# ViskaWei/VIT

Hardware: AMD Instinct MI355X
Metric: images/sec ViT-B/16 224^2 bf16 train step (higher is better)
Workload: dtype bf16

## Files before the change

include/vit_amd.h:

```cpp
#ifndef VIT_AMD_H_
#define VIT_AMD_H_

#include <stddef.h>
#include <stdint.h>

#ifdef __cplusplus
extern "C" {
#endif

#define VIT_AMD_VERSION 100

typedef struct vit_ctx* vit_handle;
typedef void* vit_stream;

typedef enum { VIT_OK = 0, VIT_ERR_ARG = -1, VIT_ERR_HIP = -2, VIT_ERR_UNSUPPORTED = -3, VIT_ERR_WORKSPACE = -4 } vit_status;
typedef enum { VIT_F32 = 0, VIT_BF16 = 1 } vit_dtype;
typedef enum { VIT_ACT_NONE = 0, VIT_ACT_GELU = 1, VIT_ACT_DGELU = 2, VIT_ACT_GELU_GRAD = 3, VIT_ACT_MUL_AUX = 4 } vit_act;
typedef enum { VIT_LOSS_MSE = 0, VIT_LOSS_L1 = 1, VIT_LOSS_CE = 2 } vit_loss;

int vit_version(void);
const char* vit_last_error(void);

int vit_create(vit_handle* out, int device);
int vit_destroy(vit_handle h);
int vit_set_workspace(vit_handle h, void* ws, size_t bytes);
size_t vit_workspace_needed(void);
int vit_set_option(const char* name, int value);
int vit_handle_set_option(vit_handle h, const char* name, int value);

int vit_step_state_bind(vit_handle h, void* state);
int vit_step_advance(vit_handle h, uint64_t base_seed, float beta1, float beta2, vit_stream stream);
int vit_adamw_step_dyn(vit_handle h, float* p, const float* g, float* m, float* v, void* p_bf16, int64_t n, float beta1,
                       float beta2, float eps, float weight_decay, const float* sqnorm, float max_norm, vit_stream stream);

typedef struct vit_gemm_desc {
  int M, N, K;
  int a_trans, b_trans;
  int ab_dtype;
  const void* A; int64_t lda;
  const void* B; int64_t ldb;
  void* C; int64_t ldc; int c_dtype;
  float alpha;
  const float* bias;
  int act;
  void* aux_out;
  const void* aux_in;
  int64_t ldaux;
  float dropout_p; uint64_t seed; uint64_t site;
  const float* residual; int64_t ldres;
  int rows_per_batch, out_batch_rows, out_row_offset;
  int split_k;
  int accumulate;
  float* colsum_out;
  const float* rope_cos; const float* rope_sin;
  int rope_T, rope_dh, rope_cols;
  int drop_row_stride;
} vit_gemm_desc;
int vit_gemm(vit_handle h, const vit_gemm_desc* d, vit_stream stream);
const char* vit_last_gemm_kernel(void);

int vit_linear_fwd(vit_handle h, const void* x, const void* W, const float* bias, void* y, int y_dtype, int M, int N,
                   int K, int act, void* aux_out, float dropout_p, uint64_t seed, uint64_t site,
                   const float* residual, vit_stream stream);
int vit_linear_bwd_dx(vit_handle h, const void* dy, const void* W, void* dx, int dx_dtype, int M, int N, int K,
                      const void* dgelu_aux_in, vit_stream stream);
int vit_linear_bwd_dw(vit_handle h, const void* dy, const void* x, float* dW, int M, int N, int K, int accumulate,
                      vit_stream stream);

int vit_linear_bwd_dw_rows(vit_handle h, const void* dy, int64_t ldy, const void* x, int64_t ldx, int dtype, float* dW,
                           int rows, int N, int K, int64_t row_stride, int64_t full_rows, vit_stream stream);
int vit_colsum_rows(vit_handle h, const void* a, int a_dtype, int64_t lda, float* out, int rows, int cols, int64_t row_stride,
                    int64_t full_rows, vit_stream stream);

int vit_layernorm_fwd(vit_handle h, const float* x, const float* gamma, const float* beta, void* y, int y_dtype,
                      float* mean, float* rstd, int rows, int D, float eps, vit_stream stream);
int vit_layernorm_fwd_residual(vit_handle h, const float* x, const void* delta, int delta_dtype, float* xsum,
                               const float* gamma, const float* beta, void* y, int y_dtype, float* mean, float* rstd,
                               int rows, int D, float eps, vit_stream stream);
int vit_layernorm_fwd_residual_rows(vit_handle h, const float* x, int64_t x_row_stride, const void* delta, int delta_dtype,
                                    float* xsum, const float* gamma, const float* beta, void* y, int y_dtype, float* mean,
                                    float* rstd, int rows, int D, float eps, vit_stream stream);
int vit_layernorm_bwd(vit_handle h, const void* dy, int dy_dtype, const float* x, const float* gamma,
                      const float* mean, const float* rstd, const float* dres, float* dx, float* dgamma,
                      float* dbeta, int rows, int D, vit_stream stream);

int vit_layernorm_bwd_fused(vit_handle h, const void* dy, int dy_dtype, const float* x, const float* gamma,
                            const float* mean, const float* rstd, const float* dres, float* dx, float* dgamma,
                            float* dbeta, int rows, int D, void* dyn, int dyn_dtype, float* dbias, float dropout_p,
                            uint64_t seed, uint64_t site, vit_stream stream);

int vit_layernorm_bwd_rows(vit_handle h, const void* dy, int dy_dtype, const float* x, const float* gamma, const float* mean,
                           const float* rstd, const float* dres, int64_t dres_row_stride, float* dx, float* dgamma,
                           float* dbeta, int rows, int D, void* dyn, int dyn_dtype, float* dbias, float dropout_p,
                           uint64_t seed, uint64_t site, int64_t row_stride, vit_stream stream);

int vit_attention_fwd(vit_handle h, const void* qkv, void* ctx, void* ctx_lo, float* lse, int io_dtype, int B, int H, int T,
                      int dh, float scale, float dropout_p, uint64_t seed, uint64_t site, vit_stream stream);
int vit_attention_bwd(vit_handle h, const void* qkv, const void* ctx, const void* ctx_lo, const void* dctx, const float* lse,
                      float* delta, void* dqkv, int io_dtype, int B, int H, int T, int dh, float scale, float dropout_p,
                      uint64_t seed, uint64_t site, float* dqkv_colsum, vit_stream stream);
int vit_attention_probs(vit_handle h, const void* qkv, float* probs, int io_dtype, int B, int H, int T, int dh,
                        float scale, vit_stream stream);

int vit_unfold_cast(vit_handle h, const float* x, void* patches, int out_dtype, int B, int L, int P, int S, int N,
                    vit_stream stream);
int vit_fold_add(vit_handle h, const float* dpatches, float* dx, int B, int L, int P, int S, int N, vit_stream stream);

int vit_add_noise(vit_handle h, const float* flux, const float* error, float* out, long n, float noise_level,
                  uint64_t seed, vit_stream stream);

int vit_rope_qk(vit_handle h, void* qkv, int dtype, const float* cos_half, const float* sin_half, long rows, int T,
                int H, int dh, long ld, int inverse, vit_stream stream);

int vit_embed_finish(vit_handle h, float* tokens, const float* cls, const float* pos, int B, int T, int D,
                     float dropout_p, uint64_t seed, uint64_t site, vit_stream stream);
int vit_embed_finish_bwd(vit_handle h, const float* dtokens, void* dpatch_out, int dpatch_dtype, float* dcls, float* dpos,
                         int B, int T, int D, float dropout_p, uint64_t seed, uint64_t site, int accumulate,
                         vit_stream stream);

int vit_dropout_bwd_cast(vit_handle h, const float* dx, void* dy, int dy_dtype, int rows, int cols, float dropout_p,
                         uint64_t seed, uint64_t site, vit_stream stream);
int vit_colsum(vit_handle h, const void* a, int a_dtype, int64_t lda, float* out, int rows, int cols, int accumulate,
               vit_stream stream);
int vit_cast_f32_bf16(vit_handle h, const float* src, void* dst, int64_t n, vit_stream stream);
int vit_cast_bf16_f32(vit_handle h, const void* src, float* dst, int64_t n, float scale, vit_stream stream);

int vit_head_loss_fwd(vit_handle h, const float* last_hidden, const float* W, const float* b, const void* labels,
                      float* logits, float* loss_out, int B, int T, int D, int C, int loss_kind, vit_stream stream);
int vit_head_loss_bwd(vit_handle h, const float* last_hidden, const float* W, const float* logits, const void* labels,
                      const float* dloss, float* dlast_hidden, float* dW, float* db, int B, int T, int D, int C,
                      int loss_kind, int accumulate, vit_stream stream);

int vit_grad_sqnorm(vit_handle h, const float* g, int64_t n, float* out, vit_stream stream);
int vit_grad_sqnorm_acc(vit_handle h, const float* g, int64_t n, float* out, vit_stream stream);
int vit_adamw_step(vit_handle h, float* p, const float* g, float* m, float* v, void* p_bf16, int64_t n, float lr,
                   float beta1, float beta2, float eps, float weight_decay, int step, const float* sqnorm,
                   float max_norm, vit_stream stream);

#ifdef __cplusplus
}
#endif

#include "vit_amd_cov.h"

#endif
```

vit_amd/_cabi.py:

```python
from __future__ import annotations

import ctypes as C
import os
import re
import threading

_HERE = os.path.dirname(os.path.abspath(__file__))
LIB_PATH = os.environ.get("VIT_AMD_LIB") or os.path.join(_HERE, "lib", "libvit_amd.so")
HEADER_PATH = os.path.join(os.path.dirname(_HERE), "include", "vit_amd.h")

VIT_OK, VIT_ERR_WORKSPACE = 0, -4
VIT_F32, VIT_BF16 = 0, 1
ACT_NONE, ACT_GELU, ACT_DGELU, ACT_GELU_GRAD, ACT_MUL_AUX = 0, 1, 2, 3, 4
LOSS_MSE, LOSS_L1, LOSS_CE = 0, 1, 2


class VitError(RuntimeError):
    pass


class GemmDesc(C.Structure):
    _fields_ = [
        ("M", C.c_int), ("N", C.c_int), ("K", C.c_int),
        ("a_trans", C.c_int), ("b_trans", C.c_int),
        ("ab_dtype", C.c_int),
        ("A", C.c_void_p), ("lda", C.c_int64),
        ("B", C.c_void_p), ("ldb", C.c_int64),
        ("C", C.c_void_p), ("ldc", C.c_int64), ("c_dtype", C.c_int),
        ("alpha", C.c_float),
        ("bias", C.c_void_p),
        ("act", C.c_int),
        ("aux_out", C.c_void_p),
        ("aux_in", C.c_void_p),
        ("ldaux", C.c_int64),
        ("dropout_p", C.c_float), ("seed", C.c_uint64), ("site", C.c_uint64),
        ("residual", C.c_void_p), ("ldres", C.c_int64),
        ("rows_per_batch", C.c_int), ("out_batch_rows", C.c_int), ("out_row_offset", C.c_int),
        ("split_k", C.c_int),
        ("accumulate", C.c_int),
        ("colsum_out", C.c_void_p),
        ("rope_cos", C.c_void_p), ("rope_sin", C.c_void_p),
        ("rope_T", C.c_int), ("rope_dh", C.c_int), ("rope_cols", C.c_int),
        ("drop_row_stride", C.c_int),
    ]


_P, _I, _F, _U64, _I64, _SZ = C.c_void_p, C.c_int, C.c_float, C.c_uint64, C.c_int64, C.c_size_t

_PROTOS = {
    "vit_version": [],
    "vit_last_error": [],
    "vit_create": [C.POINTER(_P), _I],
    "vit_destroy": [_P],
    "vit_set_workspace": [_P, _P, _SZ],
    "vit_workspace_needed": [],
    "vit_set_option": [C.c_char_p, _I],
    "vit_handle_set_option": [_P, C.c_char_p, _I],
    "vit_step_state_bind": [_P, _P],
    "vit_step_advance": [_P, _U64, _F, _F, _P],
    "vit_adamw_step_dyn": [_P, _P, _P, _P, _P, _P, _I64, _F, _F, _F, _F, _P, _F, _P],
    "vit_gemm": [_P, C.POINTER(GemmDesc), _P],
    "vit_last_gemm_kernel": [],
    "vit_linear_fwd": [_P, _P, _P, _P, _P, _I, _I, _I, _I, _I, _P, _F, _U64, _U64, _P, _P],
    "vit_linear_bwd_dx": [_P, _P, _P, _P, _I, _I, _I, _I, _P, _P],
    "vit_linear_bwd_dw": [_P, _P, _P, _P, _I, _I, _I, _I, _P],
    "vit_layernorm_fwd": [_P, _P, _P, _P, _P, _I, _P, _P, _I, _I, _F, _P],
    "vit_layernorm_fwd_residual": [_P, _P, _P, _I, _P, _P, _P, _P, _I, _P, _P, _I, _I, _F, _P],
    "vit_linear_bwd_dw_rows": [_P, _P, _I64, _P, _I64, _I, _P, _I, _I, _I, _I64, _I64, _P],
    "vit_colsum_rows": [_P, _P, _I, _I64, _P, _I, _I, _I64, _I64, _P],
    "vit_layernorm_fwd_residual_rows": [_P, _P, _I64, _P, _I, _P, _P, _P, _P, _I, _P, _P, _I, _I, _F, _P],
    "vit_layernorm_bwd_rows": [_P, _P, _I, _P, _P, _P, _P, _P, _I64, _P, _P, _P, _I, _I, _P, _I, _P, _F, _U64, _U64, _I64, _P],
    "vit_layernorm_bwd": [_P, _P, _I, _P, _P, _P, _P, _P, _P, _P, _P, _I, _I, _P],
    "vit_layernorm_bwd_fused": [_P, _P, _I, _P, _P, _P, _P, _P, _P, _P, _P, _I, _I, _P, _I, _P, _F, _U64, _U64, _P],
    "vit_attention_fwd": [_P, _P, _P, _P, _P, _I, _I, _I, _I, _I, _F, _F, _U64, _U64, _P],
    "vit_attention_bwd": [_P, _P, _P, _P, _P, _P, _P, _P, _I, _I, _I, _I, _I, _F, _F, _U64, _U64, _P, _P],
    "vit_attention_probs": [_P, _P, _P, _I, _I, _I, _I, _I, _F, _P],
    "vit_unfold_cast": [_P, _P, _P, _I, _I, _I, _I, _I, _I, _P],
    "vit_fold_add": [_P, _P, _P, _I, _I, _I, _I, _I, _P],
    "vit_add_noise": [_P, _P, _P, _P, C.c_long, _F, _U64, _P],
    "vit_rope_qk": [_P, _P, _I, _P, _P, C.c_long, _I, _I, _I, C.c_long, _I, _P],
    "vit_embed_finish": [_P, _P, _P, _P, _I, _I, _I, _F, _U64, _U64, _P],
    "vit_embed_finish_bwd": [_P, _P, _P, _I, _P, _P, _I, _I, _I, _F, _U64, _U64, _I, _P],
    "vit_dropout_bwd_cast": [_P, _P, _P, _I, _I, _I, _F, _U64, _U64, _P],
    "vit_colsum": [_P, _P, _I, _I64, _P, _I, _I, _I, _P],
    "vit_cov_accumulate": [_P, _P, _I64, _P, _P, _I, _I, _P],
    "vit_cov_finish": [_P, _P, _P, _I, _I64, _P],
    "vit_cov_mean_finish": [_P, _P, _I, _I64, _P],
    "vit_cast_f32_bf16": [_P, _P, _P, _I64, _P],
    "vit_cast_bf16_f32": [_P, _P, _P, _I64, _F, _P],
    "vit_head_loss_fwd": [_P, _P, _P, _P, _P, _P, _P, _I, _I, _I, _I, _I, _P],
    "vit_head_loss_bwd": [_P, _P, _P, _P, _P, _P, _P, _P, _P, _I, _I, _I, _I, _I, _I, _P],
    "vit_grad_sqnorm": [_P, _P, _I64, _P, _P],
    "vit_grad_sqnorm_acc": [_P, _P, _I64, _P, _P],
    "vit_adamw_step": [_P, _P, _P, _P, _P, _P, _I64, _F, _F, _F, _F, _F, _I, _P, _F, _P],
}
_RESTYPES = {"vit_last_error": C.c_char_p, "vit_last_gemm_kernel": C.c_char_p, "vit_workspace_needed": C.c_size_t}

_lib = None
_lock = threading.Lock()


def declared_symbols(header_path: str = HEADER_PATH):
    seen, names, todo = set(), set(), [os.path.abspath(header_path)]
    while todo:
        path = todo.pop()
        if path in seen:
            continue
        seen.add(path)
        text = re.sub(r"/\*.*?\*/", "", open(path).read(), flags=re.S)
        names.update(re.findall(r"\b(vit_[a-z0-9_]+)\s*\(", text))
        for inc in re.findall(r'#include\s+"([^"]+)"', text):
            sub = os.path.join(os.path.dirname(path), inc)
            if os.path.exists(sub):
                todo.append(sub)
    return sorted(names)


def load():
    global _lib
    if _lib is not None:
        return _lib
    with _lock:
        if _lib is not None:
            return _lib
        import torch

        if not os.path.exists(LIB_PATH):
            raise VitError(
                f"{LIB_PATH} is missing: run `python -m vit_amd.build` (or __graft_entry__.build()). "
                "vit_amd has no fallback path; the HIP library is required.")
        lib = C.CDLL(LIB_PATH)
        for name, argtypes in _PROTOS.items():
            fn = getattr(lib, name)
            fn.argtypes = argtypes
            fn.restype = _RESTYPES.get(name, C.c_int)
        _lib = lib
        for item in filter(None, os.environ.get("VIT_OPTIONS", "").split(",")):
            name, _, value = item.partition("=")
            rc = lib.vit_set_option(name.strip().encode(), int(value))
            if rc != VIT_OK:
                raise VitError(f"VIT_OPTIONS: vit_set_option({name!r}, {value}) failed: {lib.vit_last_error().decode()}")
        return lib


def set_option(name: str, value: int):
    check(load().vit_set_option(name.encode(), int(value)), f"vit_set_option({name})")


def check(rc: int, what: str = ""):
    if rc != VIT_OK:
        msg = load().vit_last_error()
        raise VitError(f"{what or 'vit call'} failed (status {rc}): {msg.decode() if msg else ''}")


class Handle:

    def __init__(self, device_index: int, workspace_bytes: int = 256 << 20):
        import torch

        self.lib = load()
        self.device_index = device_index
        h = C.c_void_p()
        check(self.lib.vit_create(C.byref(h), device_index), "vit_create")
        self.h = h
        self._ws = None
        self.set_workspace(workspace_bytes)

    def set_workspace(self, nbytes: int):
        import torch

        self._ws = torch.empty(nbytes, dtype=torch.uint8, device=f"cuda:{self.device_index}")
        check(self.lib.vit_set_workspace(self.h, self._ws.data_ptr(), nbytes), "vit_set_workspace")
        self.workspace_bytes = nbytes

    def set_option(self, name: str, value: int):
        check(self.lib.vit_handle_set_option(self.h, name.encode(), int(value)), f"vit_handle_set_option({name})")

    def ensure_workspace(self, nbytes: int):
        if nbytes > self.workspace_bytes:
            self.set_workspace(int(nbytes * 1.25))

    def call(self, name: str, *args):
        fn = getattr(self.lib, name)
        rc = fn(self.h, *args)
        if rc == VIT_ERR_WORKSPACE:
            self.ensure_workspace(self.lib.vit_workspace_needed())
            rc = fn(self.h, *args)
        check(rc, name)

    def __del__(self):
        try:
            if getattr(self, "h", None):
                self.lib.vit_destroy(self.h)
                self.h = None
        except Exception:
            pass


_handles = {}


def handle_for(device) -> Handle:
    import torch

    idx = device.index if device.index is not None else torch.cuda.current_device()
    if idx not in _handles:
        _handles[idx] = Handle(idx)
    return _handles[idx]
```

vit_amd/build.py:

```python
from __future__ import annotations

import hashlib
import os
import subprocess
import sys
from concurrent.futures import ThreadPoolExecutor

HERE = os.path.dirname(os.path.abspath(__file__))
ROOT = os.path.dirname(HERE)
CSRC = os.path.join(HERE, "csrc")
OBJ = os.path.join(CSRC, "_build")
LIBDIR = os.path.join(HERE, "lib")
LIB = os.path.join(LIBDIR, "libvit_amd.so")
ARCH = "gfx950"
SOURCES = ["api.hip", "gemm.hip", "gemm2.hip", "layernorm.hip", "attention.hip", "attention_tiled.hip", "attention_resident.hip",
           "attention_pipe.hip", "attention_f32.hip", "elementwise.hip", "covariance.hip"]
HEADERS = [os.path.join(CSRC, "common.h"), os.path.join(CSRC, "attention.h"), os.path.join(ROOT, "include", "vit_amd.h"),
           os.path.join(ROOT, "include", "vit_amd_cov.h")]


def _hipcc() -> str:
    for c in (os.environ.get("HIPCC"), "/opt/rocm/bin/hipcc", "hipcc"):
        if c and (os.path.isabs(c) and os.path.exists(c) or not os.path.isabs(c)):
            return c
    raise RuntimeError("hipcc not found")


def _stamp(paths) -> str:
    h = hashlib.sha256()
    for p in paths:
        with open(p, "rb") as f:
            h.update(f.read())
    return h.hexdigest()


def source_stamp() -> str:
    return _stamp([os.path.join(CSRC, s) for s in SOURCES] + HEADERS + [os.path.abspath(__file__)])


def _torch_libdir() -> str:
    import torch

    return os.path.join(os.path.dirname(torch.__file__), "lib")


def build(force: bool = False, verbose: bool = True) -> str:
    os.makedirs(OBJ, exist_ok=True)
    os.makedirs(LIBDIR, exist_ok=True)
    srcs = [os.path.join(CSRC, s) for s in SOURCES]
    stamp_file = os.path.join(OBJ, "stamp.txt")
    stamp = source_stamp()
    if not force and os.path.exists(LIB) and os.path.exists(stamp_file) and open(stamp_file).read() == stamp:
        return LIB
    hipcc = _hipcc()
    flags = [f"--offload-arch={ARCH}", "-O3", "-fPIC", "-std=c++17", "-Wno-comment", "-Wno-inline-asm", "-DNDEBUG"]

    def cc(src):
        obj = os.path.join(OBJ, os.path.basename(src).replace(".hip", ".o"))
        cmd = [hipcc, *flags, "-c", src, "-o", obj]
        r = subprocess.run(cmd, capture_output=True, text=True)
        if r.returncode != 0:
            raise RuntimeError(f"hipcc failed on {src}:\n{r.stdout}\n{r.stderr}")
        return obj

    with ThreadPoolExecutor(max_workers=min(len(srcs), os.cpu_count() or 4)) as ex:
        objs = list(ex.map(cc, srcs))
    tl = _torch_libdir()
    link = ["g++", "-shared", "-o", LIB, *objs, f"-L{tl}", "-lamdhip64", "-Wl,--no-undefined", "-lstdc++", "-lm",
            "-Wl,-rpath," + tl, "-Wl,-rpath,/opt/rocm/lib"]
    r = subprocess.run(link, capture_output=True, text=True)
    if r.returncode != 0:
        raise RuntimeError(f"link failed:\n{r.stdout}\n{r.stderr}")
    with open(stamp_file, "w") as f:
        f.write(stamp)
    if verbose:
        print(f"[vit_amd.build] built {LIB}")
    return LIB


if __name__ == "__main__":
    build(force="--force" in sys.argv)
```

vit_amd/csrc/common.h:

```cpp
#pragma once
#include <hip/hip_runtime.h>
#include <stdint.h>

#include "../../include/vit_amd.h"

namespace vit {

typedef __attribute__((ext_vector_type(8))) short bf16x8;
typedef __attribute__((ext_vector_type(4))) short bf16x4;
typedef __attribute__((ext_vector_type(4))) float f32x4;
typedef __attribute__((ext_vector_type(4))) int i32x4;
typedef __attribute__((ext_vector_type(2))) int i32x2;
typedef __attribute__((ext_vector_type(4))) unsigned u32x4;
typedef __attribute__((ext_vector_type(2))) unsigned u32x2;

#define LDS_AS __attribute__((address_space(3)))

void set_error(const char* fmt, ...);
extern thread_local char g_last_gemm[96];
#define VIT_CHECK(cond, code, ...)            \
  do {                                         \
    if (!(cond)) {                             \
      ::vit::set_error(__VA_ARGS__);           \
      return (code);                           \
    }                                          \
  } while (0)
#define VIT_HIP(expr)                                                                  \
  do {                                                                                 \
    hipError_t e_ = (expr);                                                            \
    if (e_ != hipSuccess) {                                                            \
      ::vit::set_error("%s failed: %s (%s:%d)", #expr, hipGetErrorString(e_), __FILE__, __LINE__); \
      return VIT_ERR_HIP;                                                              \
    }                                                                                  \
  } while (0)
#define VIT_LAUNCH_CHECK() VIT_HIP(hipGetLastError())

__device__ __forceinline__ float bf2f(short h) {
  return __builtin_bit_cast(float, ((unsigned)(unsigned short)h) << 16);
}
__device__ __forceinline__ short f2bf(float f) {
  return __builtin_bit_cast(short, (__bf16)f);
}
__device__ __forceinline__ unsigned pack2bf(float lo, float hi) {
  typedef __attribute__((ext_vector_type(2))) __bf16 bf2;
  typedef __attribute__((ext_vector_type(2))) float f2;
  f2 v = {lo, hi};
  bf2 r = __builtin_convertvector(v, bf2);
  return __builtin_bit_cast(unsigned, r);
}

__device__ __forceinline__ unsigned drop_hash(unsigned k0, unsigned k1, unsigned long long idx) {
  unsigned x = (unsigned)idx ^ k0 ^ ((unsigned)(idx >> 32) * 0x9E3779B9u);
  x ^= x >> 16; x *= 0x7feb352du; x += k1; x ^= x >> 15; x *= 0x846ca68bu; x ^= x >> 16;
  return x;
}
__device__ __forceinline__ unsigned drop_bits(unsigned rowkey, unsigned colpair) {
  unsigned x = (colpair ^ rowkey) * 0x2C1B3C6Du;
  x ^= x >> 15; x *= 0x297A2D39u; x ^= x >> 16;
  return x;
}
struct DropCfg {
  unsigned thr;
  float scale;
  unsigned k0, k1;
  const unsigned* dyn;
};
__device__ __forceinline__ void resolve_drop(DropCfg& d) {
  if (d.thr && d.dyn) {
    d.k0 ^= d.dyn[0];
    d.k1 ^= d.dyn[1];
  }
}
__host__ __device__ inline DropCfg make_drop(float p, uint64_t seed, uint64_t site) {
  DropCfg d;
  unsigned thr = (p <= 0.f) ? 0u : (unsigned)(p * 65536.0f + 0.5f);
  if (thr > 65535u) thr = 65535u;
  d.thr = thr;
  d.scale = 65536.0f / (float)(65536u - thr);
  uint64_t z = seed + 0x9E3779B97F4A7C15ull * (site + 1);
  z = (z ^ (z >> 30)) * 0xBF58476D1CE4E5B9ull;
  z = (z ^ (z >> 27)) * 0x94D049BB133111EBull;
  z ^= z >> 31;
  d.k0 = (unsigned)z;
  d.k1 = (unsigned)(z >> 32);
  d.dyn = nullptr;
  return d;
}
__device__ __forceinline__ unsigned drop_rowkey(const DropCfg& d, unsigned long long row) { return drop_hash(d.k0, d.k1, row); }
__device__ __forceinline__ void drop_pair(const DropCfg& d, unsigned long long row, unsigned col, float& m0, float& m1) {
  const unsigned h = drop_bits(drop_rowkey(d, row), col >> 1);
  m0 = ((h & 0xFFFFu) >= d.thr) ? d.scale : 0.f;
  m1 = ((h >> 16) >= d.thr) ? d.scale : 0.f;
}

__device__ __forceinline__ void phi_parts(float x, float& cdf, float& ex) {
  const float t = __builtin_amdgcn_rcpf(fmaf(0.3275911f * 0.70710678118654752440f, fabsf(x), 1.0f));
  ex = __builtin_amdgcn_exp2f(x * x * -0.72134752044448170368f);
  float poly = fmaf(0.5f * 1.061405429f, t, 0.5f * -1.453152027f);
  poly = fmaf(poly, t, 0.5f * 1.421413741f);
  poly = fmaf(poly, t, 0.5f * -0.284496736f);
  poly = fmaf(poly, t, 0.5f * 0.254829592f);
  const float half_erfc = poly * t * ex;
  cdf = x >= 0.f ? 1.0f - half_erfc : half_erfc;
}
__device__ __forceinline__ float gelu_erf(float x) {
  float cdf, ex;
  phi_parts(x, cdf, ex);
  return x * cdf;
}
__device__ __forceinline__ void gelu_both(float x, float& g, float& dg) {
  float cdf, ex;
  phi_parts(x, cdf, ex);
  g = x * cdf;
  dg = fmaf(x * 0.39894228040143267794f, ex, cdf);
}
typedef __attribute__((ext_vector_type(2))) float f32x2;
__device__ __forceinline__ void gelu_both2(f32x2 x, f32x2& g, f32x2& dg) {
  const f32x2 ax = {fabsf(x[0]), fabsf(x[1])};
  const f32x2 den = ax * (0.3275911f * 0.70710678118654752440f) + 1.0f;
  const f32x2 t = {__builtin_amdgcn_rcpf(den[0]), __builtin_amdgcn_rcpf(den[1])};
  const f32x2 e2 = (x * x) * -0.72134752044448170368f;
  const f32x2 ex = {__builtin_amdgcn_exp2f(e2[0]), __builtin_amdgcn_exp2f(e2[1])};
  f32x2 poly = t * (0.5f * 1.061405429f) + (0.5f * -1.453152027f);
  poly = poly * t + (0.5f * 1.421413741f);
  poly = poly * t + (0.5f * -0.284496736f);
  poly = poly * t + (0.5f * 0.254829592f);
  const f32x2 h = (poly * t) * ex;
  const f32x2 d = 0.5f - h;
  const f32x2 cdf = {0.5f + __builtin_copysignf(d[0], x[0]), 0.5f + __builtin_copysignf(d[1], x[1])};
  g = x * cdf;
  dg = (x * 0.39894228040143267794f) * ex + cdf;
}
__device__ __forceinline__ f32x2 gelu_erf2(f32x2 x) {
  f32x2 g, dg;
  gelu_both2(x, g, dg);
  return g;
}
__device__ __forceinline__ float dgelu_erf(float x) {
  float cdf, ex;
  phi_parts(x, cdf, ex);
  return fmaf(x * 0.39894228040143267794f, ex, cdf);
}

__device__ __forceinline__ float wave_sum(float v) {
#pragma unroll
  for (int o = 32; o > 0; o >>= 1) v += __shfl_xor(v, o, 64);
  return v;
}
__device__ __forceinline__ float wave_max(float v) {
#pragma unroll
  for (int o = 32; o > 0; o >>= 1) v = fmaxf(v, __shfl_xor(v, o, 64));
  return v;
}

__device__ __forceinline__ float dpp_add(float v, int ctrl_sel) {
  int m;
  const int iv = __builtin_bit_cast(int, v);
  switch (ctrl_sel) {
    case 0: m = __builtin_amdgcn_update_dpp(0, iv, 0x128, 0xF, 0xF, false); break;
    case 1: m = __builtin_amdgcn_update_dpp(0, iv, 0x124, 0xF, 0xF, false); break;
    case 2: m = __builtin_amdgcn_update_dpp(0, iv, 0x4E, 0xF, 0xF, false); break;
    default: m = __builtin_amdgcn_update_dpp(0, iv, 0xB1, 0xF, 0xF, false); break;
  }
  return v + __builtin_bit_cast(float, m);
}
template <int CPR>
__device__ __forceinline__ float sum_lanes_cpr(float x) {
  x = dpp_add(x, 3);
  x = dpp_add(x, 2);
  if (CPR == 8) {
    const int m = __builtin_amdgcn_update_dpp(0, __builtin_bit_cast(int, x), 0x141, 0xF, 0xF, false);
    x += __builtin_bit_cast(float, m);
  }
  return x;
}
__device__ __forceinline__ f32x4 rows16_sum(f32x4 v) {
#pragma unroll
  for (int c = 0; c < 4; ++c) {
    float x = v[c];
    x = dpp_add(x, 0); x = dpp_add(x, 1); x = dpp_add(x, 2); x = dpp_add(x, 3);
    v[c] = x;
  }
  return v;
}
__device__ __forceinline__ f32x4 bf_round4(u32x2 pk) {
  return (f32x4){__builtin_bit_cast(float, pk[0] << 16), __builtin_bit_cast(float, pk[0] & 0xFFFF0000u),
                 __builtin_bit_cast(float, pk[1] << 16), __builtin_bit_cast(float, pk[1] & 0xFFFF0000u)};
}

__device__ __forceinline__ int widen_pair(u32x2& a, u32x2& b, int lg) {
  auto r0 = __builtin_amdgcn_permlane16_swap(a[0], b[0], false, false);
  auto r1 = __builtin_amdgcn_permlane16_swap(a[1], b[1], false, false);
  a[0] = r0[0]; b[0] = r0[1];
  a[1] = r1[0]; b[1] = r1[1];
  return (lg & 1) ? 16 + 4 * (lg - 1) : 4 * lg;
}

__device__ __forceinline__ float grp4_max(float x) {
  x = fmaxf(x, __shfl_xor(x, 16, 64));
  return fmaxf(x, __shfl_xor(x, 32, 64));
}
__device__ __forceinline__ float grp4_sum(float x) {
  x += __shfl_xor(x, 16, 64);
  return x + __shfl_xor(x, 32, 64);
}
__device__ __forceinline__ float fast_exp2(float x) { return __builtin_amdgcn_exp2f(x); }

__device__ __forceinline__ __amdgpu_buffer_rsrc_t make_rsrc(const void* base, unsigned long long bytes) {
  unsigned n = bytes > 0x7FFFFFF0ull ? 0x7FFFFFF0u : (unsigned)bytes;
  return __builtin_amdgcn_make_buffer_rsrc(const_cast<void*>(base), 0, n, 0x00020000);
}
constexpr unsigned OOB = 0x80000000u;

__device__ __forceinline__ void lds_dma16(const void* gsrc, void* lds_dst ) {
  const unsigned a = __builtin_amdgcn_readfirstlane((unsigned)(uintptr_t)(__attribute__((address_space(3))) char*)lds_dst);
  asm volatile("s_mov_b32 m0, %1\n\ts_nop 0\n\tglobal_load_lds_dwordx4 %0, off" ::"v"(gsrc), "s"(a) : "memory", "m0");
}
__device__ __forceinline__ void lds_dma4(const void* gsrc, void* lds_dst ) {
  const unsigned a = __builtin_amdgcn_readfirstlane((unsigned)(uintptr_t)(__attribute__((address_space(3))) char*)lds_dst);
  asm volatile("s_mov_b32 m0, %1\n\ts_nop 0\n\tglobal_load_lds_dword %0, off" ::"v"(gsrc), "s"(a) : "memory", "m0");
}
__device__ __forceinline__ unsigned lds_addr_of(const void* p) { return (unsigned)(uintptr_t)(__attribute__((address_space(3))) const char*)p; }
__device__ __forceinline__ void lds_dma16_s(const void* sbase , unsigned voff, unsigned lds_addr ) {
  const unsigned a = __builtin_amdgcn_readfirstlane(lds_addr);
  asm volatile("s_mov_b32 m0, %2\n\ts_nop 0\n\tglobal_load_lds_dwordx4 %0, %1" ::"v"(voff), "s"(sbase), "s"(a) : "memory", "m0");
}
__device__ __forceinline__ void lds_dma4_s(const void* sbase , unsigned voff, unsigned lds_addr ) {
  const unsigned a = __builtin_amdgcn_readfirstlane(lds_addr);
  asm volatile("s_mov_b32 m0, %2\n\ts_nop 0\n\tglobal_load_lds_dword %0, %1" ::"v"(voff), "s"(sbase), "s"(a) : "memory", "m0");
}

struct StepState { unsigned key0, key1; float lr, bc1, rsqrt_bc2; unsigned step; };
const StepState* ctx_step_state(vit_handle h);
int ctx_num_cus(vit_handle h);
int ctx_grad_accumulate(vit_handle h);
void* ctx_claim(vit_handle h, size_t need_bytes, const char* who);
size_t colsum_ws_bytes(int rows, int cols);
static inline DropCfg make_drop_h(vit_handle h, float p, uint64_t seed, uint64_t site) {
  DropCfg d = make_drop(p, seed, site);
  const StepState* s = h ? ctx_step_state(h) : nullptr;
  d.dyn = s ? &s->key0 : nullptr;
  return d;
}

static inline int cdiv(long a, long b) { return (int)((a + b - 1) / b); }

int launch_reduce_partials(const float* part, int nblk, int width, float* out0, int split, float* out1, int accumulate,
                           hipStream_t st, int stride = 0 , int split2 = 0,
                           float* out2 = nullptr);

}
```

vit_amd/csrc/gemm.hip:

```cpp
#include <algorithm>
#include <stdio.h>

#include "common.h"

namespace vit {

constexpr int BM = 128, BN = 128, BK = 64, NTHR = 256;
constexpr int STAGE_BYTES = (BM * BK + BN * BK) * 2;
constexpr int A_BYTES = BM * BK * 2;

struct GemmArgs {
  const char* A; const char* B; char* C;
  long lda, ldb, ldc;
  long a_bs, b_bs, c_bs;
  int M, N, K;
  int tiles_m, tiles_n;
  int splits, k_per_split;
  float* slab;
  const float* bias;
  const short* aux_in; short* aux_out; long ldaux;
  const float* residual; long ldres;
  float alpha;
  int act, c_dtype;
  DropCfg drop;
  int rpb, orb, roff;
  int drs;
  int krs, krs_rows;
};

__device__ __forceinline__ int tr_swz(int k) { return ((k & 3) | (((k >> 3) & 1) << 2)) << 2; }

template <int AUX_F32>
__device__ __forceinline__ void generic_epilogue(f32x4 (&acc)[4][4], const GemmArgs& p, int m0, int n0, int wm, int wn,
                                                 int l15, int lg, int z, int batch) {
  if (p.splits > 1) {
    float* slab = p.slab + (long)z * p.M * p.N;
#pragma unroll
    for (int i = 0; i < 4; ++i) {
      const int m = m0 + wm * 64 + i * 16 + l15;
      if (m >= p.M) continue;
#pragma unroll
      for (int j = 0; j < 4; ++j) {
        const int n = n0 + wn * 64 + j * 16 + lg * 4;
        if (n < p.N) *(f32x4*)(slab + (long)m * p.N + n) = acc[i][j];
      }
    }
    return;
  }
  char* Cb = p.C + (long)batch * p.c_bs * (p.c_dtype == VIT_BF16 ? 2 : 4);
  const int N = p.N;
#pragma unroll
  for (int i = 0; i < 4; ++i) {
    const int m = m0 + wm * 64 + i * 16 + l15;
    if (m >= p.M) continue;
    long orow = m;
    if (p.rpb > 0) {
      const int b = m / p.rpb;
      orow = (long)b * p.orb + (m - b * p.rpb) + p.roff;
    }
#pragma unroll
    for (int j = 0; j < 4; ++j) {
      const int n = n0 + wn * 64 + j * 16 + lg * 4;
      if (n >= N) continue;
      f32x4 v = acc[i][j] * p.alpha;
      if (p.bias) v += *(const f32x4*)(p.bias + n);
      if (p.act == VIT_ACT_GELU || p.act == VIT_ACT_GELU_GRAD) {
        f32x4 sv = v;
        if (p.act == VIT_ACT_GELU_GRAD) {
#pragma unroll
          for (int r = 0; r < 4; ++r) {
            float g_, d_;
            gelu_both(v[r], g_, d_);
            v[r] = g_;
            sv[r] = d_;
          }
        } else {
#pragma unroll
          for (int r = 0; r < 4; ++r) v[r] = gelu_erf(v[r]);
        }
        if (p.aux_out) {
          if (AUX_F32) {
            *(f32x4*)((float*)p.aux_out + orow * p.ldaux + n) = sv;
          } else {
            u32x2 pk = {pack2bf(sv[0], sv[1]), pack2bf(sv[2], sv[3])};
            *(u32x2*)(p.aux_out + orow * p.ldaux + n) = pk;
          }
        }
      } else if (p.act == VIT_ACT_DGELU || p.act == VIT_ACT_MUL_AUX) {
        f32x4 u;
        if (AUX_F32) {
          u = *(const f32x4*)((const float*)p.aux_in + orow * p.ldaux + n);
        } else {
          const bf16x4 ub = *(const bf16x4*)(p.aux_in + orow * p.ldaux + n);
          u = (f32x4){bf2f(ub[0]), bf2f(ub[1]), bf2f(ub[2]), bf2f(ub[3])};
        }
        if (p.act == VIT_ACT_DGELU) {
#pragma unroll
          for (int r = 0; r < 4; ++r) u[r] = dgelu_erf(u[r]);
        }
        v *= u;
      }
      if (p.drop.thr) {
        float k0, k1, k2, k3;
        const unsigned long long krow = (unsigned long long)orow * (unsigned)p.drs;
        drop_pair(p.drop, krow, (unsigned)n, k0, k1);
        drop_pair(p.drop, krow, (unsigned)n + 2, k2, k3);
        v[0] *= k0; v[1] *= k1; v[2] *= k2; v[3] *= k3;
      }
      if (p.residual) v += *(const f32x4*)(p.residual + orow * p.ldres + n);
      if (p.c_dtype == VIT_BF16) {
        u32x2 pk = {pack2bf(v[0], v[1]), pack2bf(v[2], v[3])};
        *(u32x2*)(Cb + (orow * p.ldc + n) * 2) = pk;
      } else {
        *(f32x4*)(Cb + (orow * p.ldc + n) * 4) = v;
      }
    }
  }
}

template <int TRANS>
struct Loader {
  unsigned voff[4];
  unsigned lds_off[4];
  bool col_ok[4];
  int kchunk[4];
  __device__ __forceinline__ void init(int tid, long ld, int rows_total_minus_r0, int kdummy) {
#pragma unroll
    for (int i = 0; i < 4; ++i) {
      int q = tid + NTHR * i;
      if (TRANS == 0) {
        int r = q >> 3, c = q & 7;
        voff[i] = (unsigned)(r * ld * 2 + c * 16);
        lds_off[i] = r * 128 + ((c ^ ((r >> 1) & 7)) << 4);
        kchunk[i] = c * 8;
        col_ok[i] = true;
      } else {
        int kr = q >> 4, c16 = q & 15;
        voff[i] = (unsigned)(kr * ld * 2 + c16 * 16);
        lds_off[i] = kr * 256 + (((2 * c16) ^ tr_swz(kr)) << 3);
        kchunk[i] = 0;
        col_ok[i] = (c16 * 8) < rows_total_minus_r0;
      }
    }
  }
};

template <int A_T, int B_T>
__global__ __launch_bounds__(NTHR, 2) void gemm_bf16_kernel(GemmArgs p) {
  resolve_drop(p.drop);
  __shared__ __attribute__((aligned(16))) char smem[2 * STAGE_BYTES];
  const int tid = threadIdx.x, lane = tid & 63, wave = tid >> 6;
  const int wm = wave >> 1, wn = wave & 1;
  const int l15 = lane & 15, lg = lane >> 4;

  const int ntile = p.tiles_m * p.tiles_n;
  int bid = blockIdx.x;
  {
    const int q = ntile >> 3, r = ntile & 7, xcd = bid & 7, within = bid >> 3;
    bid = (xcd < r ? xcd * (q + 1) : r * (q + 1) + (xcd - r) * q) + within;
  }
  const int tm = bid / p.tiles_n, tn = bid - tm * p.tiles_n;
  const int m0 = tm * BM, n0 = tn * BN;
  const int z = blockIdx.y;
  const int batch = z / p.splits, split = z - batch * p.splits;
  const int k_begin = split * p.k_per_split;
  const int k_end = min(p.K, k_begin + p.k_per_split);
  const int nk = (k_end - k_begin + BK - 1) / BK;

  const char* Ab;
  const char* Bb;
  unsigned long long a_bytes, b_bytes;
  if (A_T == 0) {
    Ab = p.A + ((long)batch * p.a_bs + (long)m0 * p.lda + k_begin) * 2;
    a_bytes = (unsigned long long)(p.M - m0) * p.lda * 2;
  } else {
    Ab = p.A + ((long)batch * p.a_bs + (long)k_begin * p.lda + m0) * 2;
    a_bytes = (unsigned long long)(k_end - k_begin) * p.lda * 2;
  }
  if (B_T == 0) {
    Bb = p.B + ((long)batch * p.b_bs + (long)n0 * p.ldb + k_begin) * 2;
    b_bytes = (unsigned long long)(p.N - n0) * p.ldb * 2;
  } else {
    Bb = p.B + ((long)batch * p.b_bs + (long)k_begin * p.ldb + n0) * 2;
    b_bytes = (unsigned long long)(k_end - k_begin) * p.ldb * 2;
  }
  const __amdgpu_buffer_rsrc_t ra = make_rsrc(Ab, a_bytes);
  const __amdgpu_buffer_rsrc_t rb = make_rsrc(Bb, b_bytes);

  Loader<A_T> la;
  Loader<B_T> lb;
  la.init(tid, p.lda, p.M - m0, 0);
  lb.init(tid, p.ldb, p.N - n0, 0);
  const unsigned a_step = (A_T == 0) ? BK * 2 : (unsigned)(BK * p.lda * 2);
  const unsigned b_step = (B_T == 0) ? BK * 2 : (unsigned)(BK * p.ldb * 2);
  const int klen = k_end - k_begin;

  i32x4 sa[4], sb[4];
  auto issue = [&](int kt) {
#pragma unroll
    for (int i = 0; i < 4; ++i) {
      bool ok = (A_T == 0) ? (kt * BK + la.kchunk[i] < klen) : la.col_ok[i];
      unsigned vo = ok ? la.voff[i] + (unsigned)kt * a_step : OOB;
      sa[i] = __builtin_amdgcn_raw_buffer_load_b128(ra, vo, 0, 0);
    }
#pragma unroll
    for (int i = 0; i < 4; ++i) {
      bool ok = (B_T == 0) ? (kt * BK + lb.kchunk[i] < klen) : lb.col_ok[i];
      unsigned vo = ok ? lb.voff[i] + (unsigned)kt * b_step : OOB;
      sb[i] = __builtin_amdgcn_raw_buffer_load_b128(rb, vo, 0, 0);
    }
  };
  auto commit = [&](int stage) {
    char* As = smem + stage * STAGE_BYTES;
    char* Bs = As + A_BYTES;
#pragma unroll
    for (int i = 0; i < 4; ++i) *(i32x4*)(As + la.lds_off[i]) = sa[i];
#pragma unroll
    for (int i = 0; i < 4; ++i) *(i32x4*)(Bs + lb.lds_off[i]) = sb[i];
  };

  const int kc_row = l15 * 128;
  const int kc_c0 = ((lg ^ (l15 >> 1)) << 4);
  const int kc_c1 = (((4 + lg) ^ (l15 >> 1)) << 4);
  const int tq = l15 >> 2, tp = l15 & 3;
  const int tr_f = (tq | ((lg & 1) << 2)) << 2;
  const int tr_k0 = (lg * 8 + tq) * 256;

  f32x4 acc[4][4];
#pragma unroll
  for (int i = 0; i < 4; ++i)
#pragma unroll
    for (int j = 0; j < 4; ++j) acc[i][j] = (f32x4){0.f, 0.f, 0.f, 0.f};

  auto read_frag = [&](const char* img, int trans, int base16, int s) -> bf16x8 {
    if (!trans) {
      const char* pa = img + (base16 * 128 + kc_row) + (s ? kc_c1 : kc_c0);
      return *(const bf16x8*)pa;
    } else {
      const int ch = (((base16 >> 2) + tp) ^ tr_f) << 3;
      const char* pa = img + tr_k0 + s * (32 * 256) + ch;
      bf16x4 lo = __builtin_amdgcn_ds_read_tr16_b64_v4i16((LDS_AS bf16x4*)pa);
      bf16x4 hi = __builtin_amdgcn_ds_read_tr16_b64_v4i16((LDS_AS bf16x4*)(pa + 4 * 256));
      return (bf16x8){lo[0], lo[1], lo[2], lo[3], hi[0], hi[1], hi[2], hi[3]};
    }
  };

  if (nk > 0) {
    issue(0);
    commit(0);
  }
  __syncthreads();
  for (int kt = 0; kt < nk; ++kt) {
    const int cur = kt & 1;
    if (kt + 1 < nk) issue(kt + 1);
    const char* As = smem + cur * STAGE_BYTES;
    const char* Bs = As + A_BYTES;
#pragma unroll
    for (int s = 0; s < 2; ++s) {
      bf16x8 af[4], bf[4];
#pragma unroll
      for (int i = 0; i < 4; ++i) af[i] = read_frag(As, A_T, wm * 64 + i * 16, s);
#pragma unroll
      for (int j = 0; j < 4; ++j) bf[j] = read_frag(Bs, B_T, wn * 64 + j * 16, s);
#pragma unroll
      for (int i = 0; i < 4; ++i)
#pragma unroll
        for (int j = 0; j < 4; ++j)
          acc[i][j] = __builtin_amdgcn_mfma_f32_16x16x32_bf16(bf[j], af[i], acc[i][j], 0, 0, 0);
    }
    if (kt + 1 < nk) commit(cur ^ 1);
    __syncthreads();
  }

  generic_epilogue<0>(acc, p, m0, n0, wm, wn, l15, lg, z, batch);
}

constexpr int XBK = 32;
constexpr int XIMG = 128 * XBK * 2;
constexpr int XSTAGE = 4 * XIMG;

__device__ __forceinline__ void split8(const i32x4& v0, const i32x4& v1, i32x4& out_hi, i32x4& out_lo) {
  const f32x4 a = __builtin_bit_cast(f32x4, v0), b = __builtin_bit_cast(f32x4, v1);
  const unsigned h0 = pack2bf(a[0], a[1]), h1 = pack2bf(a[2], a[3]), h2 = pack2bf(b[0], b[1]), h3 = pack2bf(b[2], b[3]);
  const f32x4 ra = {a[0] - __builtin_bit_cast(float, h0 << 16), a[1] - __builtin_bit_cast(float, h0 & 0xFFFF0000u),
                    a[2] - __builtin_bit_cast(float, h1 << 16), a[3] - __builtin_bit_cast(float, h1 & 0xFFFF0000u)};
  const f32x4 rb = {b[0] - __builtin_bit_cast(float, h2 << 16), b[1] - __builtin_bit_cast(float, h2 & 0xFFFF0000u),
                    b[2] - __builtin_bit_cast(float, h3 << 16), b[3] - __builtin_bit_cast(float, h3 & 0xFFFF0000u)};
  out_hi = (i32x4){(int)h0, (int)h1, (int)h2, (int)h3};
  out_lo = (i32x4){(int)pack2bf(ra[0], ra[1]), (int)pack2bf(ra[2], ra[3]), (int)pack2bf(rb[0], rb[1]),
                   (int)pack2bf(rb[2], rb[3])};
}

template <int A_T, int B_T>
__global__ __launch_bounds__(NTHR, 2) void gemm_f32x3_kernel(GemmArgs p) {
  resolve_drop(p.drop);
  __shared__ __attribute__((aligned(16))) char smem[2 * XSTAGE];
  const int tid = threadIdx.x, lane = tid & 63, wave = tid >> 6;
  const int wm = wave >> 1, wn = wave & 1;
  const int l15 = lane & 15, lg = lane >> 4;
  const int tm = blockIdx.x / p.tiles_n, tn = blockIdx.x - tm * p.tiles_n;
  const int m0 = tm * BM, n0 = tn * BN;
  const int z = blockIdx.y;
  const int batch = z / p.splits, split = z - batch * p.splits;
  const int k_begin = split * p.k_per_split;
  const int k_end = min(p.K, k_begin + p.k_per_split);
  const int klen = k_end - k_begin;
  const int nk = (klen + XBK - 1) / XBK;

  const char* Ab;
  const char* Bb;
  unsigned long long a_bytes, b_bytes;
  const bool strided = A_T == 1 && B_T == 1 && p.krs > 1;
  if (A_T == 0) { Ab = p.A + ((long)batch * p.a_bs + (long)m0 * p.lda + k_begin) * 4; a_bytes = (unsigned long long)(p.M - m0) * p.lda * 4; }
  else if (strided) { Ab = p.A; a_bytes = (unsigned long long)p.krs_rows * p.lda * 4; }
  else { Ab = p.A + ((long)batch * p.a_bs + (long)k_begin * p.lda + m0) * 4; a_bytes = (unsigned long long)klen * p.lda * 4; }
  if (B_T == 0) { Bb = p.B + ((long)batch * p.b_bs + (long)n0 * p.ldb + k_begin) * 4; b_bytes = (unsigned long long)(p.N - n0) * p.ldb * 4; }
  else if (strided) { Bb = p.B; b_bytes = (unsigned long long)p.krs_rows * p.ldb * 4; }
  else { Bb = p.B + ((long)batch * p.b_bs + (long)k_begin * p.ldb + n0) * 4; b_bytes = (unsigned long long)klen * p.ldb * 4; }
  const __amdgpu_buffer_rsrc_t ra = make_rsrc(Ab, a_bytes);
  const __amdgpu_buffer_rsrc_t rb = make_rsrc(Bb, b_bytes);

  unsigned voffA[2], voffB[2], ldsA[2], ldsB[2];
  bool okA[2], okB[2];
  int kcA[2], kcB[2];
#pragma unroll
  for (int i = 0; i < 2; ++i) {
    const int q = tid + NTHR * i;
    if (A_T == 0) { const int r = q >> 2, c = q & 3; voffA[i] = (unsigned)(r * p.lda * 4 + c * 32); ldsA[i] = r * 64 + ((c ^ ((-(r >> 2)) & 3)) << 4); kcA[i] = c * 8; okA[i] = true; }
    else { const int kr = q >> 4, c16 = q & 15; voffA[i] = (unsigned)(kr * p.lda * 4 + c16 * 32); ldsA[i] = kr * 256 + (((2 * c16) ^ tr_swz(kr)) << 3); kcA[i] = 0; okA[i] = (c16 * 8) < (p.M - m0); }
    if (B_T == 0) { const int r = q >> 2, c = q & 3; voffB[i] = (unsigned)(r * p.ldb * 4 + c * 32); ldsB[i] = r * 64 + ((c ^ ((-(r >> 2)) & 3)) << 4); kcB[i] = c * 8; okB[i] = true; }
    else { const int kr = q >> 4, c16 = q & 15; voffB[i] = (unsigned)(kr * p.ldb * 4 + c16 * 32); ldsB[i] = kr * 256 + (((2 * c16) ^ tr_swz(kr)) << 3); kcB[i] = 0; okB[i] = (c16 * 8) < (p.N - n0); }
  }
  const unsigned a_step = (A_T == 0) ? XBK * 4 : (unsigned)(XBK * p.lda * 4);
  const unsigned b_step = (B_T == 0) ? XBK * 4 : (unsigned)(XBK * p.ldb * 4);

  i32x4 sa[2][2], sb[2][2];
  auto issue = [&](int kt) {
#pragma unroll
    for (int i = 0; i < 2; ++i) {
      bool ok = (A_T == 0) ? (kt * XBK + kcA[i] < klen) : okA[i];
      unsigned vo = ok ? voffA[i] + (unsigned)kt * a_step : OOB;
      bool okb = (B_T == 0) ? (kt * XBK + kcB[i] < klen) : okB[i];
      unsigned vb = okb ? voffB[i] + (unsigned)kt * b_step : OOB;
      if (strided) {
        const int q = tid + NTHR * i, c16 = q & 15;
        const int k = k_begin + kt * XBK + (q >> 4);
        const int ph = k / p.krs;
        const bool here = k < k_end && ph * p.krs == k && ph < p.krs_rows;
        ok = ok && here;
        okb = okb && here;
        vo = ok ? (unsigned)ph * (unsigned)(p.lda * 4) + (unsigned)((m0 + c16 * 8) * 4) : OOB;
        vb = okb ? (unsigned)ph * (unsigned)(p.ldb * 4) + (unsigned)((n0 + c16 * 8) * 4) : OOB;
      }
      sa[i][0] = __builtin_amdgcn_raw_buffer_load_b128(ra, vo, 0, 0);
      sa[i][1] = __builtin_amdgcn_raw_buffer_load_b128(ra, ok ? vo + 16 : OOB, 0, 0);
      sb[i][0] = __builtin_amdgcn_raw_buffer_load_b128(rb, vb, 0, 0);
      sb[i][1] = __builtin_amdgcn_raw_buffer_load_b128(rb, okb ? vb + 16 : OOB, 0, 0);
    }
  };
  auto commit = [&](int stage) {
    char* st = smem + stage * XSTAGE;
#pragma unroll
    for (int i = 0; i < 2; ++i) {
      i32x4 h, l;
      split8(sa[i][0], sa[i][1], h, l);
      *(i32x4*)(st + ldsA[i]) = h;
      *(i32x4*)(st + XIMG + ldsA[i]) = l;
      split8(sb[i][0], sb[i][1], h, l);
      *(i32x4*)(st + 2 * XIMG + ldsB[i]) = h;
      *(i32x4*)(st + 3 * XIMG + ldsB[i]) = l;
    }
  };

  const int kc_off = l15 * 64 + ((lg ^ ((-(l15 >> 2)) & 3)) << 4);
  const int tq = l15 >> 2, tp = l15 & 3;
  const int tr_f = (tq | ((lg & 1) << 2)) << 2;
  auto read_frag = [&](const char* img, int trans, int base16) -> bf16x8 {
    if (!trans) {
      return *(const bf16x8*)(img + base16 * 64 + kc_off);
    } else {
      const char* pa = img + (lg * 8 + tq) * 256 + ((((base16 >> 2) + tp) ^ tr_f) << 3);
      bf16x4 lo = __builtin_amdgcn_ds_read_tr16_b64_v4i16((LDS_AS bf16x4*)pa);
      bf16x4 hi = __builtin_amdgcn_ds_read_tr16_b64_v4i16((LDS_AS bf16x4*)(pa + 4 * 256));
      return (bf16x8){lo[0], lo[1], lo[2], lo[3], hi[0], hi[1], hi[2], hi[3]};
    }
  };

  f32x4 acc[4][4];
#pragma unroll
  for (int i = 0; i < 4; ++i)
#pragma unroll
    for (int j = 0; j < 4; ++j) acc[i][j] = (f32x4){0.f, 0.f, 0.f, 0.f};

  if (nk > 0) {
    issue(0);
    commit(0);
  }
  __syncthreads();
  for (int kt = 0; kt < nk; ++kt) {
    const int cur = kt & 1;
    if (kt + 1 < nk) issue(kt + 1);
    const char* st = smem + cur * XSTAGE;
    bf16x8 ah[4], al[4];
#pragma unroll
    for (int i = 0; i < 4; ++i) {
      ah[i] = read_frag(st, A_T, wm * 64 + i * 16);
      al[i] = read_frag(st + XIMG, A_T, wm * 64 + i * 16);
    }
#pragma unroll
    for (int j = 0; j < 4; ++j) {
      const bf16x8 bh = read_frag(st + 2 * XIMG, B_T, wn * 64 + j * 16);
      const bf16x8 bl = read_frag(st + 3 * XIMG, B_T, wn * 64 + j * 16);
#pragma unroll
      for (int i = 0; i < 4; ++i) {
        acc[i][j] = __builtin_amdgcn_mfma_f32_16x16x32_bf16(bl, ah[i], acc[i][j], 0, 0, 0);
        acc[i][j] = __builtin_amdgcn_mfma_f32_16x16x32_bf16(bh, al[i], acc[i][j], 0, 0, 0);
        acc[i][j] = __builtin_amdgcn_mfma_f32_16x16x32_bf16(bh, ah[i], acc[i][j], 0, 0, 0);
      }
    }
    if (kt + 1 < nk) commit(cur ^ 1);
    __syncthreads();
  }
  generic_epilogue<1>(acc, p, m0, n0, wm, wn, l15, lg, z, batch);
}

__global__ void splitk_reduce_kernel(const float* __restrict__ slab, float* __restrict__ C, long ldc, int M, int N,
                                     int splits, float alpha, int accumulate) {
  const long nvec = (long)M * (N >> 2);
  const long stride = (long)M * N;
  for (long i = blockIdx.x * (long)blockDim.x + threadIdx.x; i < nvec; i += (long)gridDim.x * blockDim.x) {
    const long m = i / (N >> 2);
    const int n = (int)(i - m * (N >> 2)) << 2;
    const float* s = slab + m * N + n;
    f32x4 a = *(const f32x4*)s;
    for (int k = 1; k < splits; ++k) a += *(const f32x4*)(s + k * stride);
    a *= alpha;
    float* c = C + m * ldc + n;
    if (accumulate) a += *(const f32x4*)c;
    *(f32x4*)c = a;
  }
}

__global__ void add_into_kernel(float* __restrict__ C, long ldc, const float* __restrict__ src, int M, int N) {
  const long nvec = (long)M * (N >> 2);
  for (long i = blockIdx.x * (long)blockDim.x + threadIdx.x; i < nvec; i += (long)gridDim.x * blockDim.x) {
    const long m = i / (N >> 2);
    const int n = (int)(i - m * (N >> 2)) << 2;
    float* c = C + m * ldc + n;
    *(f32x4*)c = *(const f32x4*)c + *(const f32x4*)(src + m * N + n);
  }
}

void* ctx_reserve_tail(vit_handle h, size_t bytes);
void ctx_release_tail(vit_handle h);
int gemm2_try_launch(vit_handle h, const vit_gemm_desc* d, hipStream_t st, int* rc);
bool gemm2_ws_bytes(vit_handle h, const vit_gemm_desc* d, size_t* bytes);

int launch_splitk_reduce(const float* slab, float* C, long ldc, int M, int N, int splits, float alpha, int accumulate,
                         hipStream_t st) {
  const long nvec = (long)M * (N / 4);
  const int blocks = (int)std::min<long>((nvec + 255) / 256, 2048);
  hipLaunchKernelGGL(splitk_reduce_kernel, dim3(blocks), dim3(256), 0, st, slab, C, ldc, M, N, splits, alpha, accumulate);
  VIT_LAUNCH_CHECK();
  return VIT_OK;
}

static bool al16(const void* p) { return ((uintptr_t)p & 15) == 0; }

thread_local int g_colsum_fused = 0;
thread_local int g_rope_fused = 0;
struct KRows { int stride, rows; };
int gemm_launch(vit_handle h, const vit_gemm_desc* d, hipStream_t st, int k_row_stride = 0, int k_rows = 0);
static int gemm_launch_core(vit_handle h, const vit_gemm_desc* d, hipStream_t st, KRows kr = {0, 0});

static size_t round256(size_t bytes) { return (bytes + 255) & ~(size_t)255; }

static size_t accum_scratch_bytes(const vit_gemm_desc* d) { return round256((size_t)d->M * d->N * sizeof(float)); }
static int gemm_accumulate_with_colsum(vit_handle h, const vit_gemm_desc* d, hipStream_t st) {
  float* scr = (float*)ctx_reserve_tail(h, accum_scratch_bytes(d));
  VIT_CHECK(scr, VIT_ERR_WORKSPACE, "vit_gemm: the workspace's tail is already lent out");
  vit_gemm_desc t = *d;
  t.C = scr; t.ldc = d->N; t.accumulate = 0; t.colsum_out = nullptr;
  int rc = gemm_launch_core(h, &t, st);
  if (rc == VIT_OK) rc = vit_colsum(h, scr, VIT_F32, d->N, d->colsum_out, d->M, d->N, 1, (vit_stream)st);
  ctx_release_tail(h);
  if (rc != VIT_OK) return rc;
  const long nvec = (long)d->M * (d->N / 4);
  hipLaunchKernelGGL(add_into_kernel, dim3((int)std::min<long>((nvec + 255) / 256, 2048)), dim3(256), 0, st, (float*)d->C,
                     (long)d->ldc, scr, d->M, d->N);
  VIT_LAUNCH_CHECK();
  return VIT_OK;
}

static void split_plan(const vit_gemm_desc* d, int bk, int* splits_out, int* kps_out) {
  const int ktiles = cdiv(d->K, bk);
  int splits = d->split_k;
  if (splits < 0) {
    const int tiles = cdiv(d->M, BM) * cdiv(d->N, BN);
    splits = 1;
    if (tiles < 256) splits = std::min(std::max(1, 512 / tiles), std::max(1, ktiles / 4));
  }
  if (splits < 1) splits = 1;
  if (splits > ktiles) splits = ktiles;
  const int kps = cdiv(ktiles, splits) * bk;
  *splits_out = cdiv(d->K, kps);
  *kps_out = kps;
}

static size_t gemm_ws_bytes(vit_handle h, const vit_gemm_desc* d) {
  size_t need = 0;
  const bool f32in = d->ab_dtype == VIT_F32;
  if (f32in || !gemm2_ws_bytes(h, d, &need)) {
    int splits, kps;
    split_plan(d, f32in ? XBK : BK, &splits, &kps);
    if (splits > 1) need = (size_t)splits * d->M * d->N * sizeof(float);
  }
  if (d->colsum_out) need = std::max(need, colsum_ws_bytes(d->M, d->N));
  return need;
}

static int gemm_check_args(const vit_gemm_desc* d, KRows kr) {
  VIT_CHECK(d && d->A && d->B && d->C, VIT_ERR_ARG, "vit_gemm: null operand");
  VIT_CHECK(d->M > 0 && d->N > 0 && d->K > 0, VIT_ERR_ARG, "vit_gemm: empty problem M=%d N=%d K=%d", d->M, d->N, d->K);
  VIT_CHECK(d->ab_dtype == VIT_BF16 || d->ab_dtype == VIT_F32, VIT_ERR_ARG, "vit_gemm: bad ab_dtype");
  const bool f32in = d->ab_dtype == VIT_F32;
  VIT_CHECK(d->c_dtype == VIT_BF16 || d->c_dtype == VIT_F32, VIT_ERR_ARG, "vit_gemm: bad c_dtype");
  VIT_CHECK((d->lda % 8) == 0 && (d->ldb % 8) == 0 && (d->ldc % 4) == 0 && (d->N % 4) == 0, VIT_ERR_ARG,
            "vit_gemm: lda, ldb must be multiples of 8, ldc and N of 4 (N=%d lda=%ld ldb=%ld ldc=%ld)", d->N,
            (long)d->lda, (long)d->ldb, (long)d->ldc);
  VIT_CHECK(d->a_trans ? (d->M % 8) == 0 : (d->K % 8) == 0, VIT_ERR_ARG,
            "vit_gemm: A needs %s %% 8 == 0 (M=%d K=%d)", d->a_trans ? "M" : "K", d->M, d->K);
  VIT_CHECK(d->b_trans ? (d->N % 8) == 0 : (d->K % 8) == 0, VIT_ERR_ARG,
            "vit_gemm: B needs %s %% 8 == 0 (N=%d K=%d)", d->b_trans ? "N" : "K", d->N, d->K);
  VIT_CHECK(al16(d->A) && al16(d->B) && al16(d->C), VIT_ERR_ARG, "vit_gemm: operands must be 16-byte aligned");
  VIT_CHECK(d->lda >= (d->a_trans ? d->M : d->K) && d->ldb >= (d->b_trans ? d->N : d->K) && d->ldc >= d->N,
            VIT_ERR_ARG, "vit_gemm: leading dimension smaller than the row length");
  if (d->bias) VIT_CHECK(al16(d->bias), VIT_ERR_ARG, "vit_gemm: bias must be 16-byte aligned");
  if (d->residual) VIT_CHECK(al16(d->residual) && (d->ldres % 4) == 0, VIT_ERR_ARG, "vit_gemm: residual alignment");
  VIT_CHECK(d->act >= VIT_ACT_NONE && d->act <= VIT_ACT_MUL_AUX, VIT_ERR_ARG, "vit_gemm: bad act %d", d->act);
  if (d->act == VIT_ACT_DGELU || d->act == VIT_ACT_MUL_AUX)
    VIT_CHECK(d->aux_in && (d->ldaux % 4) == 0, VIT_ERR_ARG, "vit_gemm: ACT_DGELU / ACT_MUL_AUX need aux_in");
  if (d->act == VIT_ACT_GELU_GRAD) VIT_CHECK(d->aux_out, VIT_ERR_ARG, "vit_gemm: ACT_GELU_GRAD needs aux_out");
  if (d->aux_out) VIT_CHECK((d->ldaux % 4) == 0 && d->ldaux >= d->N, VIT_ERR_ARG, "vit_gemm: bad ldaux");
  VIT_CHECK(d->dropout_p >= 0.f && d->dropout_p < 1.f, VIT_ERR_ARG, "vit_gemm: dropout_p out of [0,1)");
  VIT_CHECK(d->drop_row_stride >= 0, VIT_ERR_ARG, "vit_gemm: drop_row_stride=%d", d->drop_row_stride);

  if (d->dropout_p > 0.f) VIT_CHECK((d->N % 2) == 0, VIT_ERR_ARG, "vit_gemm: dropout needs an even N");
  if (kr.stride > 1)
    VIT_CHECK(f32in && d->a_trans && d->b_trans && kr.rows > 0 &&
                  (unsigned long long)kr.rows * (unsigned long long)std::max(d->lda, d->ldb) * 4 < 0x7FFFFFF0ull,
              VIT_ERR_ARG, "vit_gemm: compact K rows need f32 operands, both transposed, below 2 GiB");
  return VIT_OK;
}

int gemm_launch(vit_handle h, const vit_gemm_desc* d, hipStream_t st, int k_row_stride, int k_rows) {
  g_colsum_fused = 0;
  g_rope_fused = 0;
  const KRows kr = {k_row_stride, k_rows};
  int rc = gemm_check_args(d, kr);
  if (rc != VIT_OK) return rc;
  const int accum = ctx_grad_accumulate(h);
  vit_gemm_desc dd;
  if (accum && d->a_trans && d->c_dtype == VIT_F32 && !d->accumulate) {
    dd = *d;
    dd.accumulate = 1;
    d = &dd;
  }
  const bool scratch = accum && d->accumulate && d->colsum_out;
  if (scratch)
    VIT_CHECK(d->c_dtype == VIT_F32 && d->rows_per_batch == 0 && !d->rope_cos && !d->residual, VIT_ERR_ARG,
              "vit_gemm: accumulate with colsum_out needs an f32 C and no row map, rope or residual");
  if (d->colsum_out) VIT_CHECK(d->rows_per_batch == 0, VIT_ERR_ARG, "vit_gemm: colsum_out with a row map is not supported");
  if (d->rope_cos) {
    VIT_CHECK(d->rope_sin && d->rope_T > 0 && d->rope_dh >= 8 && (d->rope_dh % 8) == 0 && d->rope_cols > 0 &&
                  (d->rope_cols % (2 * d->rope_dh)) == 0 && d->rope_cols <= d->N && d->rows_per_batch == 0 && !d->colsum_out &&
                  d->act == VIT_ACT_NONE && !d->residual && d->split_k <= 1 && d->dropout_p == 0.f,
              VIT_ERR_ARG, "vit_gemm: rope needs sin, T > 0, head_dim %% 8 == 0, rope_cols = 2 x heads x head_dim <= N, and a "
                           "projection (a bias is fine) without dropout, row map, column sums, residual or split-K: the pass "
                           "behind a dropped-out product would rotate AFTER the dropout, which is not the reference's order");
  }
  size_t need = gemm_ws_bytes(h, d);
  if (scratch) need = round256(need) + accum_scratch_bytes(d);
  if (need && !ctx_claim(h, need, "vit_gemm")) return VIT_ERR_WORKSPACE;
  if (scratch) return gemm_accumulate_with_colsum(h, d, st);
  rc = gemm_launch_core(h, d, st, kr);
  if (rc == VIT_OK && d->rope_cos && !g_rope_fused)
    rc = vit_rope_qk(h, d->C, d->c_dtype, d->rope_cos, d->rope_sin, d->M, d->rope_T, d->rope_cols / (2 * d->rope_dh), d->rope_dh,
                     d->ldc, 0, (vit_stream)st);
  if (rc != VIT_OK || !d->colsum_out || g_colsum_fused) return rc;
  return vit_colsum(h, d->C, d->c_dtype, d->ldc, d->colsum_out, d->M, d->N, accum, (vit_stream)st);
}

static int gemm_launch_core(vit_handle h, const vit_gemm_desc* d, hipStream_t st, KRows kr) {
  const bool f32in = d->ab_dtype == VIT_F32;
  if (!f32in) {
    int rc2 = VIT_OK;
    if (gemm2_try_launch(h, d, st, &rc2)) return rc2;
  }

  GemmArgs a;
  a.A = (const char*)d->A; a.B = (const char*)d->B; a.C = (char*)d->C;
  a.lda = d->lda; a.ldb = d->ldb; a.ldc = d->ldc;
  a.a_bs = a.b_bs = a.c_bs = 0;
  a.M = d->M; a.N = d->N; a.K = d->K;
  a.tiles_m = cdiv(d->M, BM); a.tiles_n = cdiv(d->N, BN);
  int splits, kps;
  split_plan(d, f32in ? XBK : BK, &splits, &kps);
  a.splits = splits; a.k_per_split = kps;
  a.slab = nullptr;
  if (splits > 1) {
    VIT_CHECK(d->c_dtype == VIT_F32 && !d->bias && d->act == VIT_ACT_NONE && d->dropout_p == 0.f && !d->residual &&
                  d->rows_per_batch == 0,
              VIT_ERR_ARG, "vit_gemm: split_k supports only alpha and an f32 C");
    if (!(a.slab = (float*)ctx_claim(h, (size_t)splits * d->M * d->N * sizeof(float), "vit_gemm: split-K"))) return VIT_ERR_WORKSPACE;
  }
  a.bias = d->bias;
  a.aux_in = (const short*)d->aux_in; a.aux_out = (short*)d->aux_out; a.ldaux = d->ldaux;
  a.residual = d->residual; a.ldres = d->ldres;
  if (d->accumulate && splits == 1) {
    VIT_CHECK(d->c_dtype == VIT_F32 && !d->residual && d->rows_per_batch == 0, VIT_ERR_ARG,
              "vit_gemm: accumulate needs an f32 C and no residual");
    a.residual = (const float*)d->C; a.ldres = d->ldc;
  }
  a.alpha = d->alpha;
  a.act = d->act; a.c_dtype = d->c_dtype;
  a.drop = make_drop_h(h, d->dropout_p, d->seed, d->site);
  a.rpb = d->rows_per_batch; a.orb = d->out_batch_rows; a.roff = d->out_row_offset;
  a.drs = (a.drop.thr && d->drop_row_stride > 1) ? d->drop_row_stride : 1;
  a.krs = a.krs_rows = 0;
  if (kr.stride > 1) {
    a.krs = kr.stride;
    a.krs_rows = kr.rows;
  }

  dim3 grid(a.tiles_m * a.tiles_n, splits), block(NTHR);
  const int v = d->a_trans * 2 + d->b_trans;
  snprintf(g_last_gemm, sizeof(g_last_gemm), "%s<%d, %d>", f32in ? "gemm_f32x3_kernel" : "gemm_bf16_kernel", d->a_trans,
           d->b_trans);
  if (f32in) {
    switch (v) {
      case 0: hipLaunchKernelGGL((gemm_f32x3_kernel<0, 0>), grid, block, 0, st, a); break;
      case 1: hipLaunchKernelGGL((gemm_f32x3_kernel<0, 1>), grid, block, 0, st, a); break;
      case 2: hipLaunchKernelGGL((gemm_f32x3_kernel<1, 0>), grid, block, 0, st, a); break;
      default: hipLaunchKernelGGL((gemm_f32x3_kernel<1, 1>), grid, block, 0, st, a); break;
    }
  } else
  switch (v) {
    case 0: hipLaunchKernelGGL((gemm_bf16_kernel<0, 0>), grid, block, 0, st, a); break;
    case 1: hipLaunchKernelGGL((gemm_bf16_kernel<0, 1>), grid, block, 0, st, a); break;
    case 2: hipLaunchKernelGGL((gemm_bf16_kernel<1, 0>), grid, block, 0, st, a); break;
    default: hipLaunchKernelGGL((gemm_bf16_kernel<1, 1>), grid, block, 0, st, a); break;
  }
  VIT_LAUNCH_CHECK();
  if (splits > 1)
    return launch_splitk_reduce(a.slab, (float*)d->C, (long)d->ldc, d->M, d->N, splits, d->alpha, d->accumulate, st);
  return VIT_OK;
}

}

extern "C" {

int vit_gemm(vit_handle h, const vit_gemm_desc* d, vit_stream stream) {
  return vit::gemm_launch(h, d, (hipStream_t)stream);
}

int vit_linear_fwd(vit_handle h, const void* x, const void* W, const float* bias, void* y, int y_dtype, int M, int N,
                   int K, int act, void* aux_out, float dropout_p, uint64_t seed, uint64_t site,
                   const float* residual, vit_stream stream) {
  vit_gemm_desc d = {};
  d.M = M; d.N = N; d.K = K; d.ab_dtype = VIT_BF16;
  d.A = x; d.lda = K; d.B = W; d.ldb = K; d.C = y; d.ldc = N; d.c_dtype = y_dtype;
  d.alpha = 1.f; d.bias = bias; d.act = act; d.aux_out = aux_out; d.ldaux = N;
  d.dropout_p = dropout_p; d.seed = seed; d.site = site; d.residual = residual; d.ldres = N;
  return vit::gemm_launch(h, &d, (hipStream_t)stream);
}

int vit_linear_bwd_dx(vit_handle h, const void* dy, const void* W, void* dx, int dx_dtype, int M, int N, int K,
                      const void* dgelu_aux_in, vit_stream stream) {
  vit_gemm_desc d = {};
  d.M = M; d.N = K; d.K = N; d.ab_dtype = VIT_BF16;
  d.A = dy; d.lda = N; d.B = W; d.ldb = K; d.b_trans = 1; d.C = dx; d.ldc = K; d.c_dtype = dx_dtype;
  d.alpha = 1.f;
  if (dgelu_aux_in) { d.act = VIT_ACT_DGELU; d.aux_in = dgelu_aux_in; d.ldaux = K; }
  return vit::gemm_launch(h, &d, (hipStream_t)stream);
}

int vit_linear_bwd_dw(vit_handle h, const void* dy, const void* x, float* dW, int M, int N, int K, int accumulate,
                      vit_stream stream) {
  vit_gemm_desc d = {};
  d.M = N; d.N = K; d.K = M; d.ab_dtype = VIT_BF16;
  d.A = dy; d.lda = N; d.a_trans = 1; d.B = x; d.ldb = K; d.b_trans = 1; d.C = dW; d.ldc = K; d.c_dtype = VIT_F32;
  d.alpha = 1.f; d.split_k = -1; d.accumulate = accumulate;
  return vit::gemm_launch(h, &d, (hipStream_t)stream);
}

}
```

vit_amd/csrc/gemm2.hip:

```cpp
#include <algorithm>
#include <stdio.h>

#include "common.h"

namespace vit {

#define GLB_AS __attribute__((address_space(1)))

struct Gemm2Args {
  const char* A; const char* B; char* C;
  long lda, ldb, ldc;
  int M, N, K;
  int tiles_m, tiles_n, nblk;
  int splits, k_per_split;
  float* slab;
  const float* bias;
  const short* aux_in; short* aux_out; long ldaux;
  const float* residual; long ldres;
  float alpha;
  int act, c_dtype;
  DropCfg drop;
  int rpb, orb, roff;
  int drs;
  int lin_split;
  float* colsum_part;
  int grp2;
  const float* rope_cos; const float* rope_sin;
  int rope_T, rope_dh, rope_cols;
};

__device__ __forceinline__ int tr_swz2(int k) { return ((k & 3) | (((k >> 3) & 1) << 2)) << 2; }

template <int WM, int WN, int CW, int EPI>
__device__ __forceinline__ void tile_epilogue(f32x4 (&acc)[WM][WN], char* scr, const Gemm2Args& p, int m0, int n0,
                                              int split, int lane) {
  const int l15 = lane & 15, lg = lane >> 4;
  constexpr int CPR = CW / 4;
  constexpr int RPI = 64 / CPR;
  float* slab = p.splits > 1 ? p.slab + (long)split * p.M * p.N : nullptr;
#pragma unroll
  for (int i = 0; i < WM; ++i) {
#pragma unroll
    for (int jc = 0; jc < (WN * 16) / CW; ++jc) {
#pragma unroll
      for (int jj = 0; jj < CW / 16; ++jj) {
        const int c16 = jj * 4 + lg;
        *(f32x4*)(scr + l15 * (CW * 4) + ((c16 ^ (l15 & (CPR - 1))) << 4)) = acc[i][jc * (CW / 16) + jj];
        acc[i][jc * (CW / 16) + jj] = (f32x4){0.f, 0.f, 0.f, 0.f};
      }
#pragma unroll
      for (int rr = 0; rr < 16 / RPI; ++rr) {
        const int row = rr * RPI + lane / CPR, c16 = lane % CPR;
        f32x4 v = *(const f32x4*)(scr + row * (CW * 4) + ((c16 ^ (row & (CPR - 1))) << 4));
        const int m = m0 + i * 16 + row, n = n0 + jc * CW + c16 * 4;
        if (slab) {
          *(f32x4*)(slab + (long)m * p.N + n) = v;
          continue;
        }
        long orow = m;
        if (p.rpb > 0) {
          const int b = m / p.rpb;
          orow = (long)b * p.orb + (m - b * p.rpb) + p.roff;
        }
        v *= p.alpha;
        if (p.bias) v += *(const f32x4*)(p.bias + n);
        if (EPI == 1) {
          f32x4 sv = v;
          if (p.act == VIT_ACT_GELU_GRAD) {
#pragma unroll
            for (int r = 0; r < 4; ++r) {
              float g_, d_;
              gelu_both(v[r], g_, d_);
              v[r] = g_;
              sv[r] = d_;
            }
          } else {
#pragma unroll
            for (int r = 0; r < 4; ++r) v[r] = gelu_erf(v[r]);
          }
          if (p.aux_out) {
            u32x2 pk = {pack2bf(sv[0], sv[1]), pack2bf(sv[2], sv[3])};
            *(u32x2*)(p.aux_out + orow * p.ldaux + n) = pk;
          }
        } else if (EPI == 2) {
          bf16x4 u = *(const bf16x4*)(p.aux_in + orow * p.ldaux + n);
          if (p.act == VIT_ACT_MUL_AUX) {
#pragma unroll
            for (int r = 0; r < 4; ++r) v[r] *= bf2f(u[r]);
          } else {
#pragma unroll
            for (int r = 0; r < 4; ++r) v[r] *= dgelu_erf(bf2f(u[r]));
          }
        }
        if (p.drop.thr) {
          float k0, k1, k2, k3;
          const unsigned long long krow = (unsigned long long)orow * (unsigned)p.drs;
          drop_pair(p.drop, krow, (unsigned)n, k0, k1);
          drop_pair(p.drop, krow, (unsigned)n + 2, k2, k3);
          v[0] *= k0; v[1] *= k1; v[2] *= k2; v[3] *= k3;
        }
        if (p.residual) v += *(const f32x4*)(p.residual + orow * p.ldres + n);
        if (p.c_dtype == VIT_BF16) {
          u32x2 pk = {pack2bf(v[0], v[1]), pack2bf(v[2], v[3])};
          *(u32x2*)(p.C + (orow * p.ldc + n) * 2) = pk;
        } else {
          *(f32x4*)(p.C + (orow * p.ldc + n) * 4) = v;
        }
      }
    }
  }
}

int launch_splitk_reduce(const float* slab, float* C, long ldc, int M, int N, int splits, float alpha, int accumulate,
                         hipStream_t st);

template <int FAST, int NI>
__device__ __forceinline__ void pp_epilogue(f32x4 (&acc)[NI][4], char* scr, const Gemm2Args& p, int m0, int n0, int split,
                                            int lane) {
  const int l15 = lane & 15, lg = lane >> 4;
  if (FAST == 7) {
    float* cf = p.splits > 1 ? p.slab + (long)split * p.M * p.N : (float*)p.C;
    const long ldc = p.splits > 1 ? (long)p.N : p.ldc;
    const int n = n0 + l15 * 4;
#pragma unroll
    for (int i = 0; i < NI; ++i) {
#pragma unroll
      for (int j = 0; j < 4; ++j) {
        *(f32x4*)(scr + l15 * 256 + (((j * 4 + lg) ^ l15) << 4)) = acc[i][j];
        acc[i][j] = (f32x4){0.f, 0.f, 0.f, 0.f};
      }
#pragma unroll
      for (int rr = 0; rr < 4; ++rr) {
        const int row = rr * 4 + lg;
        *(f32x4*)(cf + (long)(m0 + i * 16 + row) * ldc + n) = *(const f32x4*)(scr + row * 256 + ((l15 ^ row) << 4));
      }
    }
    return;
  }
  const int cg = lane & 7, rsub = lane >> 3;
  const int n = n0 + cg * 8;
  const __amdgpu_buffer_rsrc_t rc_ = make_rsrc(p.C, (unsigned long long)p.M * p.ldc * 2);
  const __amdgpu_buffer_rsrc_t ra_ = make_rsrc(p.aux_out ? (const void*)p.aux_out : (const void*)p.C, (unsigned long long)p.M * p.ldaux * 2);
#define EPI_STORE_C(M_, PK) __builtin_amdgcn_raw_buffer_store_b128(PK, rc_, (unsigned)(((M_) * p.ldc + n) * 2), 0, 16)
#define EPI_STORE_AUX(M_, PK) __builtin_amdgcn_raw_buffer_store_b128(PK, ra_, (unsigned)(((M_) * p.ldaux + n) * 2), 0, 16)
  f32x4 bv0 = (f32x4){0.f, 0.f, 0.f, 0.f}, bv1 = bv0;
  if ((FAST == 3 || FAST == 4 || FAST == 8) && p.bias) {
    bv0 = *(const f32x4*)(p.bias + n);
    bv1 = *(const f32x4*)(p.bias + n + 4);
  }
  float cs[8] = {0.f, 0.f, 0.f, 0.f, 0.f, 0.f, 0.f, 0.f};
  const bool want_cs = p.colsum_part != nullptr;
  u32x4 au[4][2];
  f32x4 rc0, rc1, rs0, rs1, k8c0, k8c1, k8s0, k8s1;
  int rt = 0;
  const int rope_peer = (lane ^ (p.rope_dh >> 4)) << 2;
  if (FAST == 8 && n0 < p.rope_cols) {
    const int hl_ = p.rope_dh >> 4, hd = p.rope_dh >> 1, io = (cg & (hl_ - 1)) * 8;
    rt = (m0 + rsub) % p.rope_T;
    const long to = (long)rt * hd + io, t8 = 8L * hd + io;
    rc0 = *(const f32x4*)(p.rope_cos + to); rc1 = *(const f32x4*)(p.rope_cos + to + 4);
    rs0 = *(const f32x4*)(p.rope_sin + to); rs1 = *(const f32x4*)(p.rope_sin + to + 4);
    k8c0 = *(const f32x4*)(p.rope_cos + t8); k8c1 = *(const f32x4*)(p.rope_cos + t8 + 4);
    k8s0 = *(const f32x4*)(p.rope_sin + t8); k8s1 = *(const f32x4*)(p.rope_sin + t8 + 4);
  }
  const __amdgpu_buffer_rsrc_t rx_ = make_rsrc(p.aux_in ? (const void*)p.aux_in : (const void*)p.C, (unsigned long long)p.M * p.ldaux * 2);
#pragma unroll
  for (int i = 0; i < NI; ++i) {
    if (FAST == 5 && (i & 3) == 0) {
#pragma unroll
      for (int ii = 0; ii < 4; ++ii)
#pragma unroll
        for (int rr = 0; rr < 2; ++rr)
          au[ii][rr] = __builtin_amdgcn_raw_buffer_load_b128(rx_, (unsigned)(((long)(m0 + (i + ii) * 16 + rr * 8 + rsub) * p.ldaux + n) * 2), 0, 18);
    }
    f32x4 v[2][2];
#pragma unroll
    for (int j = 0; j < 4; ++j) {
      *(f32x4*)(scr + l15 * 256 + (((j * 4 + lg) ^ l15) << 4)) = acc[i][j];
      acc[i][j] = (f32x4){0.f, 0.f, 0.f, 0.f};
    }
#pragma unroll
    for (int rr = 0; rr < 2; ++rr) {
      const int row = rr * 8 + rsub;
      v[rr][0] = *(const f32x4*)(scr + row * 256 + (((2 * cg) ^ row) << 4));
      v[rr][1] = *(const f32x4*)(scr + row * 256 + (((2 * cg + 1) ^ row) << 4));
    }
#pragma unroll
    for (int rr = 0; rr < 2; ++rr) {
      const long m = m0 + i * 16 + rr * 8 + rsub;
      float o[8];
#pragma unroll
      for (int r = 0; r < 4; ++r) {
        o[r] = v[rr][0][r] + bv0[r];
        o[4 + r] = v[rr][1][r] + bv1[r];
      }
      if (FAST == 4) {
        float sv[8];
        if (p.act == VIT_ACT_GELU_GRAD) {
#pragma unroll
          for (int r = 0; r < 8; r += 2) {
            f32x2 g_, d_;
            gelu_both2((f32x2){o[r], o[r + 1]}, g_, d_);
            o[r] = g_[0]; o[r + 1] = g_[1];
            sv[r] = d_[0]; sv[r + 1] = d_[1];
          }
        } else {
#pragma unroll
          for (int r = 0; r < 8; r += 2) {
            sv[r] = o[r]; sv[r + 1] = o[r + 1];
            const f32x2 g_ = gelu_erf2((f32x2){o[r], o[r + 1]});
            o[r] = g_[0]; o[r + 1] = g_[1];
          }
        }
        if (p.aux_out) {
          u32x4 pk = {pack2bf(sv[0], sv[1]), pack2bf(sv[2], sv[3]), pack2bf(sv[4], sv[5]), pack2bf(sv[6], sv[7])};
          EPI_STORE_AUX(m, pk);
        }
      }
      if (FAST == 5) {
        const u32x4 u = au[i & 3][rr];
        if (p.act == VIT_ACT_MUL_AUX) {
#pragma unroll
          for (int r = 0; r < 4; ++r) {
            o[2 * r] *= __builtin_bit_cast(float, u[r] << 16);
            o[2 * r + 1] *= __builtin_bit_cast(float, u[r] & 0xFFFF0000u);
          }
        } else {
#pragma unroll
          for (int r = 0; r < 4; ++r) {
            o[2 * r] *= dgelu_erf(__builtin_bit_cast(float, u[r] << 16));
            o[2 * r + 1] *= dgelu_erf(__builtin_bit_cast(float, u[r] & 0xFFFF0000u));
          }
        }
      }
      if (FAST == 8 && n0 < p.rope_cols) {
        const int hl = p.rope_dh >> 4;
        const float sg = (cg & hl) ? 1.f : -1.f;
        const f32x4 c0 = rc0, c1 = rc1, s0 = rs0, s1 = rs1;
        float px[8];
#pragma unroll
        for (int r = 0; r < 8; ++r)
          px[r] = __builtin_bit_cast(float, __builtin_amdgcn_ds_bpermute(rope_peer, __builtin_bit_cast(int, o[r])));
#pragma unroll
        for (int r = 0; r < 4; ++r) {
          o[r] = fmaf(o[r], c0[r], sg * px[r] * s0[r]);
          o[4 + r] = fmaf(o[4 + r], c1[r], sg * px[4 + r] * s1[r]);
        }
        rt += 8;
        const bool wrapped = rt >= p.rope_T;
        if (wrapped) rt -= p.rope_T;
        {
          const f32x4 nc0 = rc0 * k8c0 - rs0 * k8s0, ns0 = rs0 * k8c0 + rc0 * k8s0;
          const f32x4 nc1 = rc1 * k8c1 - rs1 * k8s1, ns1 = rs1 * k8c1 + rc1 * k8s1;
          rc0 = nc0; rs0 = ns0; rc1 = nc1; rs1 = ns1;
        }
        if (__builtin_amdgcn_ballot_w64(wrapped)) {
          const long to = (long)rt * (p.rope_dh >> 1) + (cg & (hl - 1)) * 8;
          rc0 = *(const f32x4*)(p.rope_cos + to); rc1 = *(const f32x4*)(p.rope_cos + to + 4);
          rs0 = *(const f32x4*)(p.rope_sin + to); rs1 = *(const f32x4*)(p.rope_sin + to + 4);
        }
      }
      if (FAST == 3 && p.drop.thr) {
#pragma unroll
        for (int r = 0; r < 4; ++r) {
          float k0, k1;
          drop_pair(p.drop, (unsigned long long)m, (unsigned)n + 2 * r, k0, k1);
          o[2 * r] *= k0;
          o[2 * r + 1] *= k1;
        }
      }
      u32x4 pk = {pack2bf(o[0], o[1]), pack2bf(o[2], o[3]), pack2bf(o[4], o[5]), pack2bf(o[6], o[7])};
      EPI_STORE_C(m, pk);
      if (want_cs) {
#pragma unroll
        for (int r = 0; r < 4; ++r) {
          cs[2 * r] += __builtin_bit_cast(float, pk[r] << 16);
          cs[2 * r + 1] += __builtin_bit_cast(float, pk[r] & 0xFFFF0000u);
        }
      }
    }
  }
  if (p.colsum_part) {
#pragma unroll
    for (int r = 0; r < 8; ++r) {
      float v = cs[r];
      v += __shfl_xor(v, 8, 64);
      v += __shfl_xor(v, 16, 64);
      v += __shfl_xor(v, 32, 64);
      cs[r] = v;
    }
    if (lane < 8) {
      float* dst = p.colsum_part + (long)(m0 >> 7) * p.N + n;
      *(f32x4*)dst = (f32x4){cs[0], cs[1], cs[2], cs[3]};
      *(f32x4*)(dst + 4) = (f32x4){cs[4], cs[5], cs[6], cs[7]};
    }
  }
#undef EPI_STORE_C
#undef EPI_STORE_AUX
}

template <int A_T, int B_T, int EPI, int NSLOT>
__global__ __launch_bounds__(512, 2) void gemm3_kernel(Gemm2Args p) {
  resolve_drop(p.drop);
  constexpr int BM = 256, BN = 256, BK = 64;
  constexpr int HALF = 128 * BK * 2;
  static_assert(NSLOT == 8, "the ring arithmetic below is for 8 slots (two K-tiles of four half-tiles)");
  constexpr int DEPTH = NSLOT - 3, INFL = 2 * (DEPTH - 1);
  constexpr int SCR = 4096, CW = 64;
  constexpr int XA0 = 0, XB0 = 1, XB1 = 2, XA1 = 3;
  constexpr int RELAX = INFL + (((EPI >= 3 && EPI <= 6) || EPI == 8) ? 16 : 32);
  extern __shared__ __attribute__((aligned(16))) char smem[];

  const int tid = threadIdx.x, lane = tid & 63;
  const int wave = __builtin_amdgcn_readfirstlane(tid >> 6);
  const int wr = wave >> 2, wc = wave & 3, grp = wr;
  const int l15 = lane & 15, lg = lane >> 4;

  const int ntile = p.tiles_m * p.tiles_n;
  int split = blockIdx.y, bx = blockIdx.x;
  if (p.lin_split) {
    const int total = ntile * p.splits, lin = blockIdx.x;
    const int q = total >> 3, r = total & 7, xcd = lin & 7, within = lin >> 3;
    const int pos = (xcd < r ? xcd * (q + 1) : r * (q + 1) + (xcd - r) * q) + within;
    split = pos / ntile;
    bx = pos - split * ntile;
  }
  const int k_begin = split * p.k_per_split;
  const int k_end = min(p.K, k_begin + p.k_per_split);
  const int nk = (k_end - k_begin) / BK;
  const int nblk = p.nblk;
  const int my_tiles = (ntile - bx + nblk - 1) / nblk;
  const int T = my_tiles * nk;

  int offA[2], offB[2];
#pragma unroll
  for (int i = 0; i < 2; ++i) {
    if (A_T == 0) {
      const int rimg = i * 64 + wave * 8 + (lane >> 3);
      offA[i] = (i * 128 + wave * 8 + (lane >> 3)) * (int)p.lda + (((lane & 7) ^ ((rimg >> 1) & 7)) << 3);
    } else {
      const int k = i * 32 + wave * 4 + (lane >> 4);
      const int c16 = (lane & 15) ^ (tr_swz2(k) >> 1);
      offA[i] = k * (int)p.lda + (c16 >> 3) * 128 + ((c16 & 7) << 3);
    }
    if (B_T == 0) {
      const int rimg = i * 64 + wave * 8 + (lane >> 3);
      offB[i] = ((rimg >> 5) * 64 + (rimg & 31)) * (int)p.ldb + (((lane & 7) ^ ((rimg >> 1) & 7)) << 3);
    } else {
      const int k = i * 32 + wave * 4 + (lane >> 4);
      const int c16 = (lane & 15) ^ (tr_swz2(k) >> 1);
      offB[i] = k * (int)p.ldb + (c16 >> 2) * 64 + ((c16 & 3) << 3);
    }
  }
  const long halfA = (A_T == 0) ? 64 * p.lda : 64, halfB = (B_T == 0) ? 32 * p.ldb : 32;

  auto tile_coords = [&](int j, int& tm, int& tn) {
    const int round0 = j * nblk;
    const int n_here = min(nblk, ntile - round0);
    const int q = n_here >> 3, r = n_here & 7, xcd = bx & 7, within = bx >> 3;
    const int pos = (xcd < r ? xcd * (q + 1) : r * (q + 1) + (xcd - r) * q) + within;
    if (p.grp2) {
      const int hgrp = n_here >> 1, hn = p.tiles_n >> 1;
      const int g = pos >= hgrp;
      const int u = (round0 >> 1) + (g ? pos - hgrp : pos);
      tm = u / hn;
      tn = g * hn + (u - tm * hn);
      return;
    }
    const int t = p.lin_split ? bx : round0 + pos;
    tm = t / p.tiles_n;
    tn = t - tm * p.tiles_n;
  };
  const long dA = (A_T == 0) ? (long)BK * 2 : (long)BK * p.lda * 2;
  const long dB = (B_T == 0) ? (long)BK * 2 : (long)BK * p.ldb * 2;
  int cj = 0, ckt = 0;
  const char *ca, *cb;
  auto tile_bases = [&](int j) {
    int tm, tn;
    tile_coords(j, tm, tn);
    ca = (A_T == 0) ? p.A + ((long)tm * BM * p.lda + k_begin) * 2 : p.A + ((long)k_begin * p.lda + (long)tm * BM) * 2;
    cb = (B_T == 0) ? p.B + ((long)tn * BN * p.ldb + k_begin) * 2 : p.B + ((long)k_begin * p.ldb + (long)tn * BN) * 2;
  };
  tile_bases(0);
  auto cursor_next = [&](const char*& ab, const char*& bb) {
    ab = ca;
    bb = cb;
    if (++ckt == nk) {
      if (cj + 1 < my_tiles) {
        ++cj;
        ckt = 0;
        tile_bases(cj);
      } else {
        ckt = nk - 1;
      }
    } else {
      ca += dA;
      cb += dB;
    }
  };
  unsigned dofs = 0;
  const unsigned smem_a = lds_addr_of(smem) + wave * 1024;
  auto issue_half = [&](const char* base, long half_off, const int (&off)[2]) {
    const unsigned dst = smem_a + dofs;
    dofs = (dofs + HALF) & (NSLOT * HALF - 1);
    const char* sb = base + half_off * 2;
    lds_dma16_s(sb, (unsigned)off[0] * 2u, dst);
    lds_dma16_s(sb, (unsigned)off[1] * 2u, dst + 8192);
  };

  const int tq = l15 >> 2, tp = l15 & 3;
  const int tr_f = (tq | ((lg & 1) << 2)) << 2;
  int kc_off[2];
#pragma unroll
  for (int s = 0; s < 2; ++s) kc_off[s] = l15 * 128 + (((s * 4 + lg) ^ (l15 >> 1)) << 4);
  auto read_frag = [&](const char* img, int trans, int base16, int s) -> bf16x8 {
    if (!trans) {
      return *(const bf16x8*)(img + base16 * (BK * 2) + kc_off[s]);
    } else {
      const char* pa = img + (s * 32 + lg * 8 + tq) * 256 + ((((base16 >> 2) + tp) ^ tr_f) << 3);
      bf16x4 lo = __builtin_amdgcn_ds_read_tr16_b64_v4i16((LDS_AS bf16x4*)pa);
      bf16x4 hi = __builtin_amdgcn_ds_read_tr16_b64_v4i16((LDS_AS bf16x4*)(pa + 4 * 256));
      return (bf16x8){lo[0], lo[1], lo[2], lo[3], hi[0], hi[1], hi[2], hi[3]};
    }
  };

  f32x4 acc[8][4];
#pragma unroll
  for (int i = 0; i < 8; ++i)
#pragma unroll
    for (int j = 0; j < 4; ++j) acc[i][j] = (f32x4){0.f, 0.f, 0.f, 0.f};
  bf16x8 af[4][2], b0[2][2], b1[2][2];

#define PP_READ_A(IMG)                                                                           \
  _Pragma("unroll") for (int i_ = 0; i_ < 4; ++i_) _Pragma("unroll") for (int s_ = 0; s_ < 2; ++s_) \
      af[i_][s_] = read_frag(IMG, A_T, wr * 64 + i_ * 16, s_);
#define PP_READ_B(BF, IMG)                                                                       \
  _Pragma("unroll") for (int j_ = 0; j_ < 2; ++j_) _Pragma("unroll") for (int s_ = 0; s_ < 2; ++s_) \
      BF[j_][s_] = read_frag(IMG, B_T, wc * 32 + j_ * 16, s_);
#define PP_MFMA(HA, HB, BF)                                                                      \
  __builtin_amdgcn_sched_barrier(0);                                                             \
  __builtin_amdgcn_s_barrier();                                                                  \
  asm volatile("s_waitcnt lgkmcnt(0)" ::: "memory");                                             \
  __builtin_amdgcn_sched_barrier(0);                                                             \
  __builtin_amdgcn_s_setprio(1);                                                                 \
  _Pragma("unroll") for (int s_ = 0; s_ < 2; ++s_) _Pragma("unroll") for (int i_ = 0; i_ < 4; ++i_) \
      _Pragma("unroll") for (int j_ = 0; j_ < 2; ++j_)                                            \
          acc[HA * 4 + i_][HB * 2 + j_] =                                                        \
              __builtin_amdgcn_mfma_f32_16x16x32_bf16(BF[j_][s_], af[i_][s_], acc[HA * 4 + i_][HB * 2 + j_], 0, 0, 0); \
  __builtin_amdgcn_s_setprio(0);                                                                 \
  __builtin_amdgcn_sched_barrier(0);                                                             \
  __builtin_amdgcn_s_barrier();
#define PP_STAGE(BASE, HOFF, OFF)                                                                \
  {                                                                                              \
  issue_half(BASE, HOFF, OFF);                                                                   \
  asm volatile("s_cmp_lg_u32 %0, 0\n\t"                                                          \
               "s_cbranch_scc1 .Lpp_relaxed_%=\n\t"                                              \
               "s_waitcnt vmcnt(%1)\n\t"                                                         \
               "s_branch .Lpp_waited_%=\n"                                                       \
               ".Lpp_relaxed_%=:\n\t"                                                            \
               "s_waitcnt vmcnt(%2)\n"                                                           \
               ".Lpp_waited_%=:" ::"s"(relaxed), "n"(INFL), "n"(RELAX) : "scc", "memory");        \
  }
#define PP_KTILE4                                                                                \
  PP_READ_B(b0, sp + XB0 * HALF)                                                                 \
  PP_READ_A(sp + XA0 * HALF)                                                                     \
  PP_STAGE(bb1, halfB, offB)                                                                     \
  PP_MFMA(0, 0, b0)                                                                              \
  PP_READ_B(b1, sp + XB1 * HALF)                                                                 \
  PP_STAGE(a1, halfA, offA)                                                                      \
  PP_MFMA(0, 1, b1)                                                                              \
  PP_READ_A(sp + XA1 * HALF)                                                                     \
  PP_STAGE(a2, 0, offA)                                                                          \
  PP_MFMA(1, 1, b1)                                                                              \
  PP_STAGE(bb2, 0, offB)                                                                         \
  PP_MFMA(1, 0, b0)
#define PP_LOADED(RX)                                                                            \
  asm volatile("s_cmp_lg_u32 %0, 0\n\t"                                                          \
               "s_cbranch_scc1 .Lpp_relaxed_%=\n\t"                                              \
               "s_waitcnt vmcnt(%1)\n\t"                                                         \
               "s_branch .Lpp_waited_%=\n"                                                       \
               ".Lpp_relaxed_%=:\n\t"                                                            \
               "s_waitcnt vmcnt(%2)\n"                                                           \
               ".Lpp_waited_%=:\n\t"                                                             \
               "s_waitcnt lgkmcnt(0)" ::"s"(relaxed), "n"(INFL), "n"(RX) : "scc", "memory");
#define PP_MFMA2(HA, BFA, HBA, BFB, HBB)                                                         \
  __builtin_amdgcn_sched_barrier(0);                                                             \
  __builtin_amdgcn_s_barrier();                                                                  \
  __builtin_amdgcn_sched_barrier(0);                                                             \
  __builtin_amdgcn_s_setprio(1);                                                                 \
  _Pragma("unroll") for (int s_ = 0; s_ < 2; ++s_) _Pragma("unroll") for (int i_ = 0; i_ < 4; ++i_) \
      _Pragma("unroll") for (int j_ = 0; j_ < 2; ++j_)                                            \
          acc[HA * 4 + i_][HBA * 2 + j_] =                                                       \
              __builtin_amdgcn_mfma_f32_16x16x32_bf16(BFA[j_][s_], af[i_][s_], acc[HA * 4 + i_][HBA * 2 + j_], 0, 0, 0); \
  _Pragma("unroll") for (int s_ = 0; s_ < 2; ++s_) _Pragma("unroll") for (int i_ = 0; i_ < 4; ++i_) \
      _Pragma("unroll") for (int j_ = 0; j_ < 2; ++j_)                                            \
          acc[HA * 4 + i_][HBB * 2 + j_] =                                                       \
              __builtin_amdgcn_mfma_f32_16x16x32_bf16(BFB[j_][s_], af[i_][s_], acc[HA * 4 + i_][HBB * 2 + j_], 0, 0, 0); \
  __builtin_amdgcn_s_setprio(0);                                                                 \
  __builtin_amdgcn_sched_barrier(0);                                                             \
  __builtin_amdgcn_s_barrier();
#define PP_KTILE2                                                                                \
  PP_READ_B(b0, sp + XB0 * HALF)                                                                 \
  PP_READ_A(sp + XA0 * HALF)                                                                     \
  PP_READ_B(b1, sp + XB1 * HALF)                                                                 \
  issue_half(a1, halfA, offA);                                                                   \
  PP_LOADED(RELAX)                                                                               \
  PP_MFMA2(0, b0, 0, b1, 1)                                                                      \
  PP_READ_A(sp + XA1 * HALF)                                                                     \
  issue_half(a2, 0, offA);                                                                       \
  issue_half(bb2, 0, offB);                                                                      \
  issue_half(bb2, halfB, offB);                                                                  \
  PP_LOADED(RELAX)                                                                               \
  PP_MFMA2(1, b1, 1, b0, 0)
  constexpr bool MERGED = A_T || B_T;

  static_assert(DEPTH == 5, "stage schedule written out for the 8-slot ring");
  const char *a1, *bb1, *a2, *bb2;
  {
    const char *a0, *bb0;
    cursor_next(a0, bb0);
    issue_half(a0, 0, offA);
    issue_half(bb0, 0, offB);
    issue_half(bb0, halfB, offB);
    issue_half(a0, halfA, offA);
    cursor_next(a1, bb1);
    issue_half(a1, 0, offA);
    issue_half(bb1, 0, offB);
    if constexpr (MERGED) issue_half(bb1, halfB, offB);
    asm volatile("s_waitcnt vmcnt(%0)" ::"n"(INFL) : "memory");
    cursor_next(a2, bb2);
  }
  __builtin_amdgcn_s_barrier();
  if (grp == 1) __builtin_amdgcn_s_barrier();

  unsigned kb = 0;
  int relaxed = 0;
  for (int jt = 0; jt < my_tiles; ++jt) {
    for (int kt = 0; kt < nk; ++kt) {
      const char* sp = smem + kb;
      if constexpr (MERGED) {
        PP_KTILE2
      } else {
        PP_KTILE4
      }
      relaxed = 0;
      a1 = a2;
      bb1 = bb2;
      cursor_next(a2, bb2);
      kb ^= 4 * HALF;
    }
    {
      int tm, tn;
      tile_coords(jt, tm, tn);
      if (grp == 0) __builtin_amdgcn_s_barrier();
      char* scr = smem + 8 * HALF + wave * SCR;
      if constexpr (EPI >= 3) pp_epilogue<EPI, 8>(acc, scr, p, tm * BM + wr * 128, tn * BN + wc * 64, split, lane);
      else tile_epilogue<8, 4, CW, EPI>(acc, scr, p, tm * BM + wr * 128, tn * BN + wc * 64, split, lane);
      if (grp == 1) __builtin_amdgcn_s_barrier();
      relaxed = 1;
    }
  }
  if (grp == 0) __builtin_amdgcn_s_barrier();
#undef PP_READ_A
#undef PP_READ_B
#undef PP_MFMA
#undef PP_STAGE
#undef PP_KTILE2
#undef PP_KTILE4
#undef PP_LOADED
#undef PP_MFMA2
  asm volatile("s_waitcnt vmcnt(0)" ::: "memory");
}

template <int AT, int BT, int EPI>
static int launch_stag(const Gemm2Args& a, dim3 grid, hipStream_t st) {
  constexpr int smem = 160 * 1024;
  static bool attr_done = false;
  auto fn = gemm3_kernel<AT, BT, EPI, 8>;
  if (!attr_done) {
    VIT_HIP(hipFuncSetAttribute((const void*)fn, hipFuncAttributeMaxDynamicSharedMemorySize, smem));
    attr_done = true;
  }
  hipLaunchKernelGGL(fn, grid, dim3(512), smem, st, a);
  VIT_LAUNCH_CHECK();
  return VIT_OK;
}
static int launch_stag_cfg(const Gemm2Args& a, int at, int bt, int epi, dim3 grid, hipStream_t st) {
  if (epi == 1) return launch_stag<0, 0, 1>(a, grid, st);
  if (epi == 2) return launch_stag<0, 1, 2>(a, grid, st);
  if (epi == 3) return launch_stag<0, 0, 3>(a, grid, st);
  if (epi == 4) return launch_stag<0, 0, 4>(a, grid, st);
  if (epi == 5) return launch_stag<0, 1, 5>(a, grid, st);
  if (epi == 6) return launch_stag<0, 1, 6>(a, grid, st);
  if (epi == 8) return launch_stag<0, 0, 8>(a, grid, st);
  if (epi == 7) return launch_stag<1, 1, 7>(a, grid, st);
  if (!at && !bt) return launch_stag<0, 0, 0>(a, grid, st);
  if (!at && bt) return launch_stag<0, 1, 0>(a, grid, st);
  if (at && !bt) return launch_stag<1, 0, 0>(a, grid, st);
  return launch_stag<1, 1, 0>(a, grid, st);
}

extern thread_local int g_colsum_fused, g_rope_fused;
int g_gemm2_mode = 1;

static void pp_split_plan(int slots, int ntile, int K, int split_k, int* splits_out, int* kps_out) {
  const int ktiles = K / 64;
  int splits = split_k;
  if (splits < 0) {
    splits = 1;
    if (ntile < slots) splits = std::min(std::max(1, slots / ntile), std::max(1, ktiles / 8));
  }
  if (splits < 1) splits = 1;
  if (splits > ktiles) splits = ktiles;
  const int kps = cdiv(ktiles, splits) * 64;
  *splits_out = cdiv(K, kps);
  *kps_out = kps;
}

static bool pp_shape_ok(long M, long N, long K, long lda, long ldb) {
  if (g_gemm2_mode == 0) return false;
  if (M % 256 || N % 256 || K % 64) return false;
  if (lda * 256 >= (1L << 30) || ldb * 256 >= (1L << 30)) return false;
  return true;
}

static bool pp_plan(vit_handle h, const vit_gemm_desc* d, int* epi_out, int* splits_out, int* kps_out) {
  if (!pp_shape_ok(d->M, d->N, d->K, d->lda, d->ldb)) return false;
  int epi = 0;
  if (d->act == VIT_ACT_GELU || d->act == VIT_ACT_GELU_GRAD) {
    if (d->a_trans || d->b_trans) return false;
    epi = 1;
  } else if (d->act == VIT_ACT_DGELU || d->act == VIT_ACT_MUL_AUX) {
    if (d->a_trans || !d->b_trans) return false;
    epi = 2;
  }
  int splits, kps;
  pp_split_plan(ctx_num_cus(h), (d->M / 256) * (d->N / 256), d->K, d->split_k, &splits, &kps);
  if (splits > 1 && !(d->c_dtype == VIT_F32 && !d->bias && d->act == VIT_ACT_NONE && d->dropout_p == 0.f && !d->residual &&
                      d->rows_per_batch == 0)) return false;
  if (d->accumulate && splits == 1 && !(d->c_dtype == VIT_F32 && !d->residual && d->rows_per_batch == 0)) return false;
  *epi_out = epi; *splits_out = splits; *kps_out = kps;
  return true;
}
static size_t pp_colsum_bytes(const vit_gemm_desc* d) { return (size_t)(d->M / 256) * 2 * d->N * sizeof(float); }

bool gemm2_ws_bytes(vit_handle h, const vit_gemm_desc* d, size_t* bytes) {
  int epi, splits, kps;
  if (!pp_plan(h, d, &epi, &splits, &kps)) return false;
  *bytes = splits > 1 ? (size_t)splits * d->M * d->N * sizeof(float) : 0;
  if (d->colsum_out) *bytes = std::max(*bytes, pp_colsum_bytes(d));
  return true;
}

int gemm2_try_launch(vit_handle h, const vit_gemm_desc* d, hipStream_t st, int* rc) {
  int epi, splits, kps;
  if (!pp_plan(h, d, &epi, &splits, &kps)) return 0;
  const int slots = ctx_num_cus(h);

  Gemm2Args a;
  a.A = (const char*)d->A; a.B = (const char*)d->B; a.C = (char*)d->C;
  a.lda = d->lda; a.ldb = d->ldb; a.ldc = d->ldc;
  a.M = d->M; a.N = d->N; a.K = d->K;
  a.tiles_m = d->M / 256; a.tiles_n = d->N / 256;
  const int ntile = a.tiles_m * a.tiles_n;
  a.splits = splits; a.k_per_split = kps;
  a.slab = nullptr;
  *rc = VIT_ERR_WORKSPACE;
  if (splits > 1 && !(a.slab = (float*)ctx_claim(h, (size_t)splits * d->M * d->N * sizeof(float), "vit_gemm: split-K"))) return 1;
  a.nblk = std::min(ntile, slots);
  a.bias = d->bias;
  a.aux_in = (const short*)d->aux_in; a.aux_out = (short*)d->aux_out; a.ldaux = d->ldaux;
  a.residual = d->residual; a.ldres = d->ldres;
  if (d->accumulate && splits == 1) { a.residual = (const float*)d->C; a.ldres = d->ldc; }
  a.alpha = d->alpha;
  a.rope_cos = d->rope_cos; a.rope_sin = d->rope_sin; a.rope_T = d->rope_T; a.rope_dh = d->rope_dh; a.rope_cols = d->rope_cols;
  a.act = d->act; a.c_dtype = d->c_dtype;
  a.drop = make_drop_h(h, d->dropout_p, d->seed, d->site);
  a.rpb = d->rows_per_batch; a.orb = d->out_batch_rows; a.roff = d->out_row_offset;
  a.drs = (a.drop.thr && d->drop_row_stride > 1) ? d->drop_row_stride : 1;

  dim3 grid(a.nblk, splits);
  a.lin_split = 0;
  a.colsum_part = nullptr;
  if (splits > 1 && a.nblk == ntile) {
    a.lin_split = 1;
    grid = dim3(ntile * splits, 1);
  }
  int epi5 = epi;
  const bool plain = !a.residual && a.rpb == 0 && a.drs == 1 && d->alpha == 1.0f;
  if (epi == 1 && plain && a.bias && d->c_dtype == VIT_BF16 && !a.drop.thr && splits == 1) epi5 = 4;
  else if (epi == 2 && plain && !a.bias && d->c_dtype == VIT_BF16 && !a.drop.thr && splits == 1) epi5 = 5;
  else if (epi == 0 && plain && d->c_dtype == VIT_BF16 && !d->a_trans && !d->b_trans && splits == 1) epi5 = 3;
  else if (epi == 0 && plain && !a.bias && !a.drop.thr && d->c_dtype == VIT_BF16 && !d->a_trans && d->b_trans &&
           splits == 1) epi5 = 6;
  else if (epi == 0 && plain && !a.bias && !a.drop.thr && d->c_dtype == VIT_F32 && d->a_trans && d->b_trans) epi5 = 7;
  if (d->rope_cos) {
    if (epi5 == 3 && !a.drop.thr && (d->rope_dh == 16 || d->rope_dh == 32 || d->rope_dh == 64) && (d->rope_cols % 64) == 0 &&
        d->rope_T >= 9)
      epi5 = 8;
  }
  if (((epi5 >= 3 && epi5 <= 6) || epi5 == 8) &&
      ((unsigned long long)d->M * d->ldc * 2 >= 0x7FFFFFF0ull ||
       ((d->aux_out || d->aux_in) && (unsigned long long)d->M * d->ldaux * 2 >= 0x7FFFFFF0ull)))
    epi5 = epi;
  if (splits == 1 && ntile > slots) {
    a.nblk = cdiv(ntile, cdiv(ntile, slots));
    grid = dim3(a.nblk, splits);
  }
  a.grp2 = 0;
  if (splits == 1 && (a.tiles_n % 2) == 0 && (size_t)d->N * d->K * 2 > (size_t)4 << 20 && ntile > slots && (ntile % 2) == 0) {
    a.grp2 = 1;
    if (a.nblk & 1) {
      a.nblk += 1;
      grid = dim3(a.nblk, splits);
    }
  }
  if (d->colsum_out && (epi5 == 3 || epi5 == 5 || epi5 == 6) &&
      !(a.colsum_part = (float*)ctx_claim(h, pp_colsum_bytes(d), "vit_gemm: column sums"))) return 1;
  {
    const int at = epi ? 0 : d->a_trans, bt = epi == 1 ? 0 : (epi == 2 ? 1 : d->b_trans);
    snprintf(g_last_gemm, sizeof(g_last_gemm), "gemm3_kernel<%d, %d, %d, %d>", at, bt, epi5, 8);
  }
  if (epi5 == 8) g_rope_fused = 1;
  int r = launch_stag_cfg(a, d->a_trans, d->b_trans, epi5, grid, st);
  if (r == VIT_OK && a.colsum_part) {
    r = launch_reduce_partials(a.colsum_part, a.tiles_m * 2, d->N, d->colsum_out, d->N, d->colsum_out, ctx_grad_accumulate(h), st);
    g_colsum_fused = 1;
  }
  if (r == VIT_OK && splits > 1)
    r = launch_splitk_reduce(a.slab, (float*)d->C, (long)d->ldc, d->M, d->N, splits, d->alpha, d->accumulate, st);
  *rc = r;
  return 1;
}


__global__ __launch_bounds__(256) void dw_rows_kernel(const short* __restrict__ dy, long ldy, const short* __restrict__ x,
                                                      long ldx, float* __restrict__ dW, long ldw, int B, int s, int kps,
                                                      int splits, int accumulate) {
  constexpr int R = 128;
  __shared__ __attribute__((aligned(16))) short ys[R][64];
  __shared__ __attribute__((aligned(16))) short xs[R][64];
  const int t = threadIdx.x, lane = t & 63, wave = t >> 6, l15 = lane & 15, lg = lane >> 4;
  const int wn = (wave >> 1) * 32, wk = (wave & 1) * 32;
  const int n0 = blockIdx.x * 64, k0 = blockIdx.y * 64;
  f32x4 acc[2][2], tot[2][2];
#pragma unroll
  for (int i = 0; i < 2; ++i)
#pragma unroll
    for (int j = 0; j < 2; ++j) acc[i][j] = tot[i][j] = (f32x4){0.f, 0.f, 0.f, 0.f};
  int sp = 0;
  int bend = (int)min((long)B, ((long)(sp + 1) * kps + s - 1) / s);
  auto flush = [&]() {
#pragma unroll
    for (int i = 0; i < 2; ++i)
#pragma unroll
      for (int j = 0; j < 2; ++j) {
        tot[i][j] = sp == 0 ? acc[i][j] : tot[i][j] + acc[i][j];
        acc[i][j] = (f32x4){0.f, 0.f, 0.f, 0.f};
      }
    ++sp;
    bend = sp >= splits - 1 ? B : (int)min((long)B, ((long)(sp + 1) * kps + s - 1) / s);
  };
  if (splits == 1) bend = B;
  const int lr = t >> 3, lc = (t & 7) * 8;
  for (int b0 = 0; b0 < B; b0 += R) {
    __syncthreads();
    {
      u32x4 vy[R / 32], vx[R / 32];
#pragma unroll
      for (int q = 0; q < R / 32; ++q) {
        const int b = b0 + lr + 32 * q;
        vy[q] = vx[q] = (u32x4){0u, 0u, 0u, 0u};
        if (b < B) {
          vy[q] = *(const u32x4*)(dy + (long)b * ldy + n0 + lc);
          vx[q] = *(const u32x4*)(x + (long)b * ldx + k0 + lc);
        }
      }
#pragma unroll
      for (int q = 0; q < R / 32; ++q) {
        *(u32x4*)&ys[lr + 32 * q][lc] = vy[q];
        *(u32x4*)&xs[lr + 32 * q][lc] = vx[q];
      }
    }
    __syncthreads();
    const int nb = min(R, B - b0);
    int bb = 0;
    while (bb < nb) {
      while (b0 + bb >= bend) flush();
      const int seg = min(nb, bend - b0);
#pragma unroll 4
      for (; bb < seg; ++bb) {
        bf16x8 yf[2], xf[2];
#pragma unroll
        for (int i = 0; i < 2; ++i) {
          yf[i] = (bf16x8){0, 0, 0, 0, 0, 0, 0, 0};
          xf[i] = (bf16x8){0, 0, 0, 0, 0, 0, 0, 0};
          if (lg == 0) {
            yf[i][0] = ys[bb][wn + i * 16 + l15];
            xf[i][0] = xs[bb][wk + i * 16 + l15];
          }
        }
#pragma unroll
        for (int i = 0; i < 2; ++i)
#pragma unroll
          for (int j = 0; j < 2; ++j) acc[i][j] = __builtin_amdgcn_mfma_f32_16x16x32_bf16(yf[i], xf[j], acc[i][j], 0, 0, 0);
      }
    }
  }
  while (sp < splits) flush();
#pragma unroll
  for (int i = 0; i < 2; ++i)
#pragma unroll
    for (int j = 0; j < 2; ++j)
#pragma unroll
      for (int r = 0; r < 4; ++r) {
        float* o = dW + (long)(n0 + wn + i * 16 + 4 * lg + r) * ldw + k0 + wk + j * 16 + l15;
        *o = accumulate ? *o + tot[i][j][r] : tot[i][j][r];
      }
}

__global__ void colsum_rows_part_kernel(const short* __restrict__ a, long lda, float* __restrict__ part, int nblk, int N,
                                        int B, int s) {
  const long i = blockIdx.x * (long)blockDim.x + threadIdx.x;
  if (i >= (long)nblk * N) return;
  const int p = (int)(i / N), n = (int)(i - (long)p * N);
  const int b0 = (int)(((long)p * 128 + s - 1) / s), b1 = (int)min((long)B, ((long)(p + 1) * 128 + s - 1) / s);
  float v = 0.f;
  for (int b = b0; b < b1; ++b) v += bf2f(a[(long)b * lda + n]);
  part[i] = v;
}

int gemm_launch(vit_handle h, const vit_gemm_desc* d, hipStream_t st, int k_row_stride = 0, int k_rows = 0);
int colsum_strided(vit_handle h, const void* a, int a_dtype, int64_t lda, float* out, int rows, int cols, int64_t row_stride,
                   int held, int accumulate, hipStream_t st);

}

extern "C" {

int vit_linear_bwd_dw_rows(vit_handle h, const void* dy, int64_t ldy, const void* x, int64_t ldx, int dtype, float* dW,
                           int rows, int N, int K, int64_t row_stride, int64_t full_rows, vit_stream stream) {
  using namespace vit;
  VIT_CHECK(dy && x && dW, VIT_ERR_ARG, "vit_linear_bwd_dw_rows: null pointer");
  VIT_CHECK(rows > 0 && N > 0 && K > 0 && row_stride >= 1 && full_rows >= (int64_t)(rows - 1) * row_stride + 1 &&
                full_rows <= 0x7FFFFFFF && ldy >= N && ldx >= K,
            VIT_ERR_ARG, "vit_linear_bwd_dw_rows: rows=%d N=%d K=%d row_stride=%lld full_rows=%lld", rows, N, K,
            (long long)row_stride, (long long)full_rows);
  hipStream_t st = (hipStream_t)stream;
  if (dtype == VIT_BF16 && pp_shape_ok(N, K, full_rows, N, K) && (ldy % 8) == 0 && (ldx % 8) == 0 &&
      ((uintptr_t)dy % 16) == 0 && ((uintptr_t)x % 16) == 0 && ((uintptr_t)dW % 16) == 0) {
    int splits, kps;
    pp_split_plan(ctx_num_cus(h), (N / 256) * (K / 256), (int)full_rows, -1, &splits, &kps);
    hipLaunchKernelGGL(dw_rows_kernel, dim3(N / 64, K / 64), dim3(256), 0, st, (const short*)dy, (long)ldy, (const short*)x,
                       (long)ldx, dW, (long)K, rows, (int)row_stride, kps, splits, ctx_grad_accumulate(h));
    VIT_LAUNCH_CHECK();
    return VIT_OK;
  }
  if (dtype == VIT_F32 && row_stride > 1 &&
      (unsigned long long)rows * (unsigned long long)std::max(ldy, ldx) * 4 < 0x7FFFFFF0ull) {
    vit_gemm_desc d = {};
    d.M = N; d.N = K; d.K = (int)full_rows; d.ab_dtype = VIT_F32; d.a_trans = 1; d.b_trans = 1;
    d.A = dy; d.lda = ldy; d.B = x; d.ldb = ldx; d.C = dW; d.ldc = K; d.c_dtype = VIT_F32; d.alpha = 1.f; d.split_k = -1;
    return gemm_launch(h, &d, st, (int)row_stride, rows);
  }
  vit_gemm_desc d = {};
  d.M = N; d.N = K; d.K = rows; d.ab_dtype = dtype; d.a_trans = 1; d.b_trans = 1;
  d.A = dy; d.lda = ldy; d.B = x; d.ldb = ldx; d.C = dW; d.ldc = K; d.c_dtype = VIT_F32; d.alpha = 1.f; d.split_k = 1;
  return gemm_launch(h, &d, st);
}

int vit_colsum_rows(vit_handle h, const void* a, int a_dtype, int64_t lda, float* out, int rows, int cols, int64_t row_stride,
                    int64_t full_rows, vit_stream stream) {
  using namespace vit;
  VIT_CHECK(a && out, VIT_ERR_ARG, "vit_colsum_rows: null pointer");
  VIT_CHECK(rows > 0 && cols > 0 && lda >= cols && row_stride >= 1 && full_rows >= (int64_t)(rows - 1) * row_stride + 1 &&
                full_rows <= 0x7FFFFFFF,
            VIT_ERR_ARG, "vit_colsum_rows: rows=%d cols=%d row_stride=%lld full_rows=%lld", rows, cols, (long long)row_stride,
            (long long)full_rows);
  hipStream_t st = (hipStream_t)stream;
  if (a_dtype == VIT_BF16 && pp_shape_ok(full_rows, cols, 64, 64, 64)) {
    const int nblk = (int)(full_rows / 128);
    float* part = (float*)ctx_claim(h, (size_t)nblk * cols * sizeof(float), "vit_colsum_rows");
    if (!part) return VIT_ERR_WORKSPACE;
    hipLaunchKernelGGL(colsum_rows_part_kernel, dim3((unsigned)cdiv((long)nblk * cols, 256)), dim3(256), 0, st,
                       (const short*)a, (long)lda, part, nblk, cols, rows, (int)row_stride);
    VIT_LAUNCH_CHECK();
    return launch_reduce_partials(part, nblk, cols, out, cols, out, ctx_grad_accumulate(h), st);
  }
  if (a_dtype == VIT_F32 && row_stride > 1)
    return colsum_strided(h, a, a_dtype, lda, out, (int)full_rows, cols, row_stride, rows, ctx_grad_accumulate(h), st);
  return vit_colsum(h, a, a_dtype, lda, out, rows, cols, ctx_grad_accumulate(h), stream);
}

}
```

vit_amd/engine.py:

```python
from __future__ import annotations

import math
import os
from typing import Callable, Dict, List, Optional, Tuple

import torch

from . import functional as vf
from ._cabi import ACT_GELU, LOSS_CE, LOSS_L1, LOSS_MSE, VitError
from .config import ViTConfig

ALIGN = 8


def resolved_loss(task_type: str, loss_name: str) -> Tuple[str, int]:
    if task_type == "cls":
        return "ce", LOSS_CE
    if task_type == "reg":
        ln = loss_name or "l2"
        return ln, (LOSS_L1 if "l1" in ln.lower() else LOSS_MSE)
    raise ValueError(f"Unsupported task_type '{task_type}'")


class ParamLayout:

    def __init__(self, cfg: ViTConfig):
        D, P, Fd, T = cfg.hidden_size, cfg.patch_size, cfg.intermediate_size, cfg.seq_len
        self.entries: Dict[str, Tuple[int, Tuple[int, ...]]] = {}
        self.layer_ranges: List[Tuple[int, int]] = []
        off = 0

        def add(name, shape):
            nonlocal off
            n = 1
            for s in shape:
                n *= s
            self.entries[name] = (off, tuple(shape))
            off += (n + ALIGN - 1) // ALIGN * ALIGN

        e = "vit.embeddings."
        self.embed_start = off
        add(e + "cls_token", (1, 1, D))
        if cfg.pos_encoding_type == "learned":
            add(e + "position_embeddings", (1, T, D))
        add(e + "patch_embeddings.projection.weight", (D, P) if cfg.proj_fn == "SW" else (D, 1, P))
        add(e + "patch_embeddings.projection.bias", (D,))
        self.embed_end = off
        for i in range(cfg.num_hidden_layers):
            p = f"vit.encoder.layer.{i}."
            start = off
            for n in ("query", "key", "value"):
                add(p + f"attention.attention.{n}.weight", (D, D))
            for n in ("query", "key", "value"):
                add(p + f"attention.attention.{n}.bias", (D,))
            add(p + "attention.output.dense.weight", (D, D))
            add(p + "attention.output.dense.bias", (D,))
            add(p + "intermediate.dense.weight", (Fd, D))
            add(p + "intermediate.dense.bias", (Fd,))
            add(p + "output.dense.weight", (D, Fd))
            add(p + "output.dense.bias", (D,))
            add(p + "layernorm_before.weight", (D,))
            add(p + "layernorm_before.bias", (D,))
            add(p + "layernorm_after.weight", (D,))
            add(p + "layernorm_after.bias", (D,))
            self.layer_ranges.append((start, off))
        self.tail_start = off
        add("vit.layernorm.weight", (D,))
        add("vit.layernorm.bias", (D,))
        head = "classifier" if cfg.task_type == "cls" else "regressor"
        self.head = head
        add(head + ".weight", (cfg.num_labels, D))
        add(head + ".bias", (cfg.num_labels,))
        self.n_trainable = off
        add("vit.pooler.dense.weight", (D, D))
        add("vit.pooler.dense.bias", (D,))
        self.n_total = off
        order = [e + "cls_token"]
        if cfg.pos_encoding_type == "learned":
            order.append(e + "position_embeddings")
        order += [e + "patch_embeddings.projection.weight", e + "patch_embeddings.projection.bias"]
        for i in range(cfg.num_hidden_layers):
            p = f"vit.encoder.layer.{i}."
            for n in ("query", "key", "value"):
                order += [p + f"attention.attention.{n}.weight", p + f"attention.attention.{n}.bias"]
            for n in ("attention.output.dense", "intermediate.dense", "output.dense", "layernorm_before", "layernorm_after"):
                order += [p + n + ".weight", p + n + ".bias"]
        order += ["vit.layernorm.weight", "vit.layernorm.bias", "vit.pooler.dense.weight", "vit.pooler.dense.bias",
                  head + ".weight", head + ".bias"]
        assert sorted(order) == sorted(self.entries)
        self.state_order = order

    def view(self, flat: torch.Tensor, name: str) -> torch.Tensor:
        off, shape = self.entries[name]
        n = 1
        for s in shape:
            n *= s
        return flat[off:off + n].view(shape)

    def numel(self, name: str) -> int:
        n = 1
        for s in self.entries[name][1]:
            n *= s
        return n

    def buckets(self) -> List[Tuple[int, int]]:
        return [(self.tail_start, self.n_trainable)] + list(reversed(self.layer_ranges)) + \
               [(self.embed_start, self.embed_end)]


class ViTEngine:
    def __init__(self, cfg: ViTConfig, loss_name: str = ""):
        if cfg.pos_encoding_type == "rope" and (cfg.head_dim % 8) != 0:
            raise ValueError(f"pos_encoding_type='rope' needs head_dim % 8 == 0 here (got {cfg.head_dim}); "
                             f"the reference needs it even (rope.py:28-29)")
        if cfg.pos_encoding_type not in (None, "none", "learned", "rope"):
            raise ValueError(f"Unsupported pos_encoding_type '{cfg.pos_encoding_type}'. "
                             f"Choose from: 'rope', 'learned', 'none', or None")
        if cfg.proj_fn not in ("SW", "C1D", "CNN"):
            raise ValueError(f"Unsupported proj_fn '{cfg.proj_fn}'")
        if cfg.hidden_size % cfg.num_attention_heads:
            raise ValueError(f"The hidden size {cfg.hidden_size} is not a multiple of the number of attention heads "
                             f"{cfg.num_attention_heads}.")
        if cfg.head_dim % 4 or cfg.head_dim > 128 or cfg.hidden_size % 8 or cfg.patch_size % 8:
            raise ValueError(f"vit_amd kernels need head_dim % 4 == 0 and <= 128, hidden_size % 8 == 0, patch_size % 8 == 0 "
                             f"(got head_dim {cfg.head_dim}, hidden_size {cfg.hidden_size}, patch_size {cfg.patch_size})")
        self.cfg = cfg
        self.loss_name, self.loss_kind = resolved_loss(cfg.task_type, loss_name)
        self.layout = ParamLayout(cfg)
        self.flat = torch.zeros(self.layout.n_total, dtype=torch.float32)
        self.shadow: Optional[torch.Tensor] = None
        self.grads: Optional[torch.Tensor] = None
        self._shadow_version = -1
        self._arena_key = None
        self._arenas: Dict[bool, tuple] = {}
        self.act: Dict[str, object] = {}
        self.tmp: Dict[str, torch.Tensor] = {}
        self.precision = "f32"
        self.base_seed = int(torch.initial_seed()) & 0x7FFFFFFFFFFFFFFF
        self.step_counter = 0
        self._last = None
        self.side_stream: Optional[torch.cuda.Stream] = None
        self._side_handle = None
        self._main_handle = None
        self.reserve_cus = -1
        self._side_reads: Dict[str, object] = {}
        self.overlap_dw = "auto"
        self.cls_tail = os.environ.get("VIT_CLS_TAIL", "1") != "0"
        self._accum = False
        self._gen = 0
        self.grad_ready_cb: Optional[Callable[[int, int], None]] = None
        self.version_fn: Callable[[], int] = lambda: self.flat._version

    def set_precision(self, precision) -> str:
        ps = str(precision).lower()
        if ps in ("32", "32-true", "fp32", "f32", "float32"):
            mode = "f32"
        elif ps in ("bf16-mixed", "bf16", "bf16-true", "bfloat16"):
            mode = "bf16"
        elif ps in ("16-mixed", "16", "16-true", "fp16"):
            raise ValueError(f"precision '{precision}': fp16 arithmetic is not implemented on this path (it would need loss "
                             f"scaling); use '32' or 'bf16-mixed'")
        else:
            raise ValueError(f"Unsupported precision '{precision}'")
        if mode == "f32" and self.cfg.seq_len > 4096:
            raise ValueError(f"precision '{precision}': the fp32 attention kernels keep a score row in the LDS and take at most "
                             f"4096 tokens (this model has {self.cfg.seq_len}); use 'bf16-mixed'")
        if mode != self.precision:
            self.precision = mode
            self._drop_arenas()
        return mode

    @property
    def adt(self):
        return torch.bfloat16 if self.precision == "bf16" else torch.float32

    @property
    def device(self):
        return self.flat.device

    def rebind(self, new_flat: torch.Tensor):
        if new_flat.dtype != torch.float32:
            raise VitError("vit_amd keeps master parameters in fp32 (precision '32' / 'bf16-mixed' semantics); "
                           "casting the module to another dtype is not supported")
        self.flat = new_flat.contiguous()
        self.shadow = None
        self.grads = None
        self._shadow_version = -1
        self._drop_arenas()

    def p(self, name: str) -> torch.Tensor:
        return self.layout.view(self.flat, name)

    def _ensure_device_state(self):
        if not self.flat.is_cuda:
            raise VitError("vit_amd runs on an MI355X only: move the model to the GPU first (model.to('cuda')); "
                           "there is no CPU fallback path")
        if self.grads is None:
            self.grads = torch.zeros(self.layout.n_total, dtype=torch.float32, device=self.flat.device)
        if self.precision != "bf16":
            return
        if self.shadow is None:
            self.shadow = torch.empty(self.layout.n_total, dtype=torch.bfloat16, device=self.flat.device)
            self._shadow_version = -1
        ver = self.version_fn()
        if self._shadow_version != ver:
            vf.cast_f32_bf16(self.flat, self.shadow)
            self._shadow_version = ver

    def handle(self):
        from . import _cabi

        dev = self.flat.device
        if self._main_handle is None or self._main_handle.device_index != (dev.index if dev.index is not None else torch.cuda.current_device()):
            self._main_handle = _cabi.Handle(dev.index if dev.index is not None else torch.cuda.current_device())
            self._main_handle.set_option("reserve_cus", self.reserve_cus)
        return self._main_handle

    def set_reserve_cus(self, n: int):
        self.reserve_cus = int(n)
        for h in (self._main_handle, self._side_handle):
            if h is not None:
                h.set_option("reserve_cus", self.reserve_cus)

    def mark_shadow_fresh(self):
        self._shadow_version = self.version_fn()

    def w16(self, name: str) -> torch.Tensor:
        return self.layout.view(self.shadow if self.precision == "bf16" else self.flat, name)

    def g(self, name: str) -> torch.Tensor:
        return self.layout.view(self.grads, name)

    def _qkv16(self, i: int):
        off, _ = self.layout.entries[f"vit.encoder.layer.{i}.attention.attention.query.weight"]
        D = self.cfg.hidden_size
        src = self.shadow if self.precision == "bf16" else self.flat
        return src[off:off + 3 * D * D].view(3 * D, D)

    def _qkv_bias(self, i: int, buf: torch.Tensor):
        off, _ = self.layout.entries[f"vit.encoder.layer.{i}.attention.attention.query.bias"]
        D = self.cfg.hidden_size
        return buf[off:off + 3 * D]

    def _qkv_wgrad(self, i: int):
        off, _ = self.layout.entries[f"vit.encoder.layer.{i}.attention.attention.query.weight"]
        D = self.cfg.hidden_size
        return self.grads[off:off + 3 * D * D].view(3 * D, D)

    def _ensure_arena(self, B: int, train: bool):
        key = (B, train, self.precision)
        if self._arena_key == key:
            return
        slot = self._arenas.get(train)
        if slot is not None and slot[0] == key:
            self._arena_key, self.act, self.tmp, self._Mp = key, slot[1], slot[2], slot[3]
            return
        self.act, self.tmp = {}, {}
        self._arenas.pop(train, None)
        c = self.cfg
        dev = self.flat.device
        T, D, Fd, H, L, N, P = c.seq_len, c.hidden_size, c.intermediate_size, c.num_attention_heads, \
            c.num_hidden_layers, c.num_patches, c.patch_size
        M = B * T
        Mp = -(-M // 256) * 256 if (D % 256 == 0 and Fd % 256 == 0) else M
        self._Mp = Mp
        nl = L if train else 1
        f32, b16 = torch.float32, self.adt

        def E(shape, dt):
            return torch.empty(shape, dtype=dt, device=dev)

        def G(cols, dt):
            return torch.zeros((Mp, cols), dtype=dt, device=dev)[:M]

        self.act = dict(
            patches=E((B * N, P), b16),
            x=[E((B, T, D), f32) for _ in range(L + 1)],
            h1=[G(D, b16) for _ in range(nl)], qkv=[G(3 * D, b16) for _ in range(nl)],
            ctx=[G(D, b16) for _ in range(nl)], lse=[E((B * H, T), f32) for _ in range(nl)],
            ctx_lo=[E((M, D), b16) if (train and self.precision == "bf16") else None for _ in range(nl)],
            x1=[E((M, D), f32) for _ in range(nl)], h2=[G(D, b16) for _ in range(nl)],
            u=[G(Fd, b16) for _ in range(nl)], g=[G(Fd, b16) for _ in range(nl)],
            mean1=[E((M,), f32) for _ in range(nl)], rstd1=[E((M,), f32) for _ in range(nl)],
            mean2=[E((M,), f32) for _ in range(nl)], rstd2=[E((M,), f32) for _ in range(nl)],
            last=E((B, T, D), f32), meanF=E((M,), f32), rstdF=E((M,), f32),
            y=G(D, b16),
            c_y=E((B, D), b16), c_x1=E((B, D), f32), c_h2=E((B, D), b16), c_u=E((B, Fd), b16), c_g=E((B, Fd), b16),
            c_mean2=E((B,), f32), c_rstd2=E((B,), f32), c_xL=E((B, D), f32), c_last=E((B, 1, D), f32),
            c_meanF=E((B,), f32), c_rstdF=E((B,), f32),
        )
        self.tmp = {}
        if train:
            self.tmp = dict(
                dxa=E((M, D), f32), dxb=E((M, D), f32), dy=G(D, b16), dy2=G(D, b16), dU=G(Fd, b16), dh=G(D, b16),
                dqkv=G(3 * D, b16), dctx=G(D, b16), delta=E((B * H, T), f32), dpatch=E((B * N, D), b16),
                dlast=E((B, T, D), f32),
                c_dxa=E((B, D), f32), c_dxb=E((B, D), f32), c_dy=E((B, D), b16), c_dy2=E((B, D), b16), c_dU=E((B, Fd), b16),
                c_dh=E((B, D), b16), c_dlast=E((B, 1, D), f32),
                dctx_cls=G(D, b16),
            )
        self._arena_key = key
        self._arenas[train] = (key, self.act, self.tmp, Mp)

    def _drop_arenas(self):
        self._arena_key = None
        self._arenas = {}
        self.act, self.tmp = {}, {}

    def _rope_tables(self, T: int):
        c = self.cfg
        key = (T, c.head_dim, float(c.rope_base), self.flat.device)
        if getattr(self, "_rope_key", None) != key:
            dim = c.head_dim
            inv_freq = 1.0 / (c.rope_base ** (torch.arange(0, dim, 2).float() / dim))
            freqs = torch.outer(torch.arange(T).type_as(inv_freq), inv_freq)
            self._rope = (freqs.cos().contiguous().to(self.flat.device), freqs.sin().contiguous().to(self.flat.device))
            self._rope_key = key
        return self._rope

    def _site(self, layer: int, which: int) -> int:
        return 1 + 4 * layer + which

    def forward(self, x: torch.Tensor, labels: Optional[torch.Tensor], training: bool, need_grad: bool,
                output_hidden_states: bool = False, output_attentions: bool = False, capture_ctx: Optional[list] = None):
        self._ensure_device_state()
        with vf.use_handle(self.handle()):
            return self._forward(x, labels, training, need_grad, output_hidden_states, output_attentions, capture_ctx)

    def _forward(self, x, labels, training, need_grad, output_hidden_states, output_attentions, capture_ctx):
        c = self.cfg
        if x.dim() != 2 or x.shape[1] != c.image_size:
            raise ValueError(f"pixel_values must be [batch, {c.image_size}], got {tuple(x.shape)}")
        if not x.is_cuda:
            raise VitError("pixel_values must live on the GPU")
        if self.precision == "f32" and c.seq_len > 4096:
            raise ValueError(f"precision '32': the fp32 attention kernels take at most 4096 tokens (this model has "
                             f"{c.seq_len}); use train.precision 'bf16-mixed'")
        x = x.contiguous().to(torch.float32)
        B = x.shape[0]
        self._gen += 1
        T, D, Fd, H, L, N, P, S = c.seq_len, c.hidden_size, c.intermediate_size, c.num_attention_heads, \
            c.num_hidden_layers, c.num_patches, c.patch_size, c.stride
        dh, M = c.head_dim, B * T
        self._ensure_arena(B, need_grad)
        Mp = self._Mp
        a = self.act
        ph = c.hidden_dropout_prob if training else 0.0
        pa = c.attention_probs_dropout_prob if training else 0.0
        if training:
            self.step_counter += 1
        seed = (self.base_seed + 0x9E3779B97F4A7C15 * self.step_counter) & 0xFFFFFFFFFFFFFFFF
        scale = dh ** -0.5
        eps = c.layer_norm_eps
        e = "vit.embeddings."

        vf.unfold_cast(x, P, S, N, out=a["patches"])
        wp = self.w16(e + "patch_embeddings.projection.weight").view(D, P)
        x0 = a["x"][0]
        vf.gemm(a["patches"], wp, M=B * N, N=D, K=P, out=x0.view(M, D), bias=self.p(e + "patch_embeddings.projection.bias"),
                row_map=(N, T, 1))
        pos = self.p(e + "position_embeddings").view(T, D) if c.pos_encoding_type == "learned" else None
        vf.embed_finish(x0, self.p(e + "cls_token").view(D), pos, dropout=(ph, seed, 0))

        atts = [] if output_attentions else None
        rope = self._rope_tables(T) if c.pos_encoding_type == "rope" else None
        y = a["y"]
        tail = bool(self.cls_tail) and L > 0 and not output_hidden_states
        for i in range(L):
            j = i if need_grad else 0
            pre = f"vit.encoder.layer.{i}."
            xin = a["x"][i].view(M, D)
            if i == 0:
                self._ln(xin, pre + "layernorm_before", a["h1"][j], a["mean1"][j], a["rstd1"][j])
            else:
                self._ln_res(a["x1"][jprev], y, xin, pre + "layernorm_before", a["h1"][j], a["mean1"][j], a["rstd1"][j])
            vf.gemm(a["h1"][j], self._qkv16(i), M=Mp, N=3 * D, K=D, out=a["qkv"][j], bias=self._qkv_bias(i, self.flat),
                    rope=None if rope is None else (rope[0], rope[1], T, dh, 2 * D))
            vf.attention_fwd(a["qkv"][j], B, H, T, dh, scale, dropout=(pa, seed, self._site(i, 0)), ctx=a["ctx"][j],
                             lse=a["lse"][j], ctx_lo=a["ctx_lo"][j])
            if output_attentions:
                atts.append(vf.attention_probs(a["qkv"][j], B, H, T, dh, scale))
            if capture_ctx is not None:
                capture_ctx.append(a["ctx"][j].view(B, T, D).clone())
            if tail and i == L - 1:
                break
            vf.gemm(a["ctx"][j], self.w16(pre + "attention.output.dense.weight"), M=Mp, N=D, K=D, out=y,
                    bias=self.p(pre + "attention.output.dense.bias"), dropout=(ph, seed, self._site(i, 1)))
            self._ln_res(xin, y, a["x1"][j], pre + "layernorm_after", a["h2"][j], a["mean2"][j], a["rstd2"][j])
            vf.gemm(a["h2"][j], self.w16(pre + "intermediate.dense.weight"), M=Mp, N=Fd, K=D, out=a["g"][j],
                    bias=self.p(pre + "intermediate.dense.bias"), act=vf.ACT_GELU_GRAD if need_grad else ACT_GELU,
                    aux_out=a["u"][j] if need_grad else None)
            vf.gemm(a["g"][j], self.w16(pre + "output.dense.weight"), M=Mp, N=D, K=Fd, out=y,
                    bias=self.p(pre + "output.dense.bias"), dropout=(ph, seed, self._site(i, 2)))
            jprev = j
        last = a["last"]
        if tail:
            i, pre = L - 1, f"vit.encoder.layer.{L - 1}."
            j = i if need_grad else 0
            cy, last = a["c_y"], a["c_last"]
            vf.gemm(a["ctx"][j], self.w16(pre + "attention.output.dense.weight"), M=B, N=D, K=D, lda=T * D, out=cy,
                    bias=self.p(pre + "attention.output.dense.bias"), dropout=(ph, seed, self._site(i, 1)), drop_row_stride=T)
            self._ln_res(a["x"][i].view(M, D), cy, a["c_x1"], pre + "layernorm_after", a["c_h2"], a["c_mean2"], a["c_rstd2"],
                         x_row_stride=T)
            vf.gemm(a["c_h2"], self.w16(pre + "intermediate.dense.weight"), M=B, N=Fd, K=D, out=a["c_g"],
                    bias=self.p(pre + "intermediate.dense.bias"), act=vf.ACT_GELU_GRAD if need_grad else ACT_GELU,
                    aux_out=a["c_u"] if need_grad else None)
            vf.gemm(a["c_g"], self.w16(pre + "output.dense.weight"), M=B, N=D, K=Fd, out=cy,
                    bias=self.p(pre + "output.dense.bias"), dropout=(ph, seed, self._site(i, 2)), drop_row_stride=T)
            self._ln_res(a["c_x1"], cy, a["c_xL"], "vit.layernorm", last.view(B, D), a["c_meanF"], a["c_rstdF"])
        elif L > 0:
            self._ln_res(a["x1"][jprev], y, a["x"][L].view(M, D), "vit.layernorm", a["last"].view(M, D), a["meanF"],
                         a["rstdF"])
        else:
            self._ln(a["x"][L].view(M, D), "vit.layernorm", a["last"].view(M, D), a["meanF"], a["rstdF"])
        hn = self.layout.head
        if labels is not None:
            labels = labels.to(self.flat.device)
            labels = labels.contiguous().to(torch.int64 if self.loss_kind == LOSS_CE else torch.float32)
            n_expected = B if self.loss_kind == LOSS_CE else B * c.num_labels
            if labels.numel() != n_expected:
                raise ValueError(f"labels has {labels.numel()} elements, expected {n_expected}")
        logits, loss = vf.head_loss_fwd(last, self.p(hn + ".weight"), self.p(hn + ".bias"), labels, self.loss_kind)
        self._last = dict(B=B, seed=seed, ph=ph, pa=pa, labels=labels, logits=logits, gen=self._gen, grad=need_grad,
                          tail=tail)
        hs = [t.clone() for t in a["x"]] if output_hidden_states else None
        return loss, logits, hs, atts

    def saved_attentions(self):
        st, c = self._last, self.cfg
        if st is None or not st["grad"] or st["gen"] != self._gen:
            raise VitError("saved_attentions(): the last forward did not keep per-layer activations")
        with vf.use_handle(self.handle()):
            return [vf.attention_probs(self.act["qkv"][i], st["B"], c.num_attention_heads, c.seq_len, c.head_dim,
                                       c.head_dim ** -0.5) for i in range(c.num_hidden_layers)]

    def _ln(self, x, name, out, mean, rstd):
        vf.layernorm_fwd(x, self.p(name + ".weight"), self.p(name + ".bias"), self.cfg.layer_norm_eps, out=out,
                         mean=mean, rstd=rstd)

    def _ln_res(self, x, delta, xsum, name, out, mean, rstd, x_row_stride=1):
        vf.layernorm_fwd_residual(x, delta, xsum, self.p(name + ".weight"), self.p(name + ".bias"),
                                  self.cfg.layer_norm_eps, out=out, mean=mean, rstd=rstd, x_row_stride=x_row_stride)

    def _dw(self, *args, reads=(), **kw):
        if self.side_stream is None:
            return vf.gemm(*args, **kw)
        main = torch.cuda.current_stream(self.flat.device)
        self.side_stream.wait_stream(main)
        with torch.cuda.stream(self.side_stream), vf.use_handle(self._side_handle):
            out = vf.gemm(*args, **kw)
            if reads:
                ev = torch.cuda.Event()
                ev.record(self.side_stream)
                for name in reads:
                    self._side_reads[name] = ev
        return out

    def _dw_rows(self, dy, x, out, **kw):
        if self.side_stream is None:
            return vf.linear_bwd_dw_rows(dy, x, out, **kw)
        self.side_stream.wait_stream(torch.cuda.current_stream(self.flat.device))
        with torch.cuda.stream(self.side_stream), vf.use_handle(self._side_handle):
            return vf.linear_bwd_dw_rows(dy, x, out, **kw)

    def _before_write(self, *names):
        if self.side_stream is None:
            return
        main = torch.cuda.current_stream(self.flat.device)
        for name in names:
            ev = self._side_reads.pop(name, None)
            if ev is not None:
                main.wait_event(ev)

    def _join_side(self):
        if self.side_stream is not None:
            torch.cuda.current_stream(self.flat.device).wait_stream(self.side_stream)
            self._side_reads.clear()

    def _notify(self, lo: int, hi: int):
        cb = self.grad_ready_cb
        if cb is None:
            return
        if self.side_stream is None:
            return cb(lo, hi)
        self.side_stream.wait_stream(torch.cuda.current_stream(self.flat.device))
        with torch.cuda.stream(self.side_stream):
            cb(lo, hi)

    def _want_side(self) -> bool:
        if self.overlap_dw != "auto":
            return bool(self.overlap_dw)
        D = self.cfg.hidden_size
        Mp = getattr(self, "_Mp", 0)
        if D % 256 or not Mp or Mp % 256:
            return True
        cus = max(1, torch.cuda.get_device_properties(self.flat.device).multi_processor_count - max(0, self.reserve_cus))
        tiles = (Mp // 256) * (D // 256)
        rounds = -(-tiles // cus)
        return -(-tiles // rounds) <= 0.7 * cus

    def _setup_side(self):
        from . import _cabi

        on = self.precision == "bf16" and self._want_side()
        if on and self.side_stream is None:
            import os

            self.side_stream = torch.cuda.Stream(device=self.flat.device, priority=int(os.environ.get("VIT_SIDE_STREAM_PRIORITY", "0")))
            if self._side_handle is None:
                self._side_handle = _cabi.Handle(self.flat.device.index if self.flat.device.index is not None
                                                 else torch.cuda.current_device())
                self._side_handle.set_option("reserve_cus", self.reserve_cus)
        elif not on:
            self.side_stream = None
        if self._accum and self._side_handle is not None:
            self._side_handle.set_option("grad_accumulate", 1)

    def _backward_cls_tail(self, i: int, cdx: torch.Tensor, ph: float, seed: int) -> torch.Tensor:
        c, a, t = self.cfg, self.act, self.tmp
        T, D, Fd = c.seq_len, c.hidden_size, c.intermediate_size
        B = cdx.shape[0]
        pre = f"vit.encoder.layer.{i}."
        other = t["c_dxb"] if cdx is t["c_dxa"] else t["c_dxa"]
        Mp = self._Mp
        self._dw_rows(t["c_dy"], a["c_g"], self.g(pre + "output.dense.weight"), row_stride=T, full_rows=Mp)
        vf.gemm(t["c_dy"], self.w16(pre + "output.dense.weight"), M=B, N=Fd, K=D, b_trans=True, out=t["c_dU"],
                act=vf.ACT_MUL_AUX, aux_in=a["c_u"])
        vf.colsum_rows(t["c_dU"], self.g(pre + "intermediate.dense.bias"), row_stride=T, full_rows=Mp)
        self._dw_rows(t["c_dU"], a["c_h2"], self.g(pre + "intermediate.dense.weight"), row_stride=T, full_rows=Mp)
        vf.gemm(t["c_dU"], self.w16(pre + "intermediate.dense.weight"), M=B, N=D, K=Fd, b_trans=True, out=t["c_dh"])
        vf.layernorm_bwd_rows(t["c_dh"], a["c_x1"], self.p(pre + "layernorm_after.weight"), a["c_mean2"], a["c_rstd2"], cdx,
                              other, self.g(pre + "layernorm_after.weight"), self.g(pre + "layernorm_after.bias"),
                              dyn=t["c_dy2"], dbias=self.g(pre + "attention.output.dense.bias"),
                              dropout=(ph, seed, self._site(i, 1)), row_stride=T, full_rows=B * T)
        self._dw_rows(t["c_dy2"], a["ctx"][i], self.g(pre + "attention.output.dense.weight"), row_stride=T, full_rows=Mp,
                      ldx=T * D)
        vf.gemm(t["c_dy2"], self.w16(pre + "attention.output.dense.weight"), M=B, N=D, K=D, b_trans=True,
                out=t["dctx_cls"], ldc=T * D)
        return other

    def _set_accumulate(self, on: bool):
        for h in (self._main_handle, self._side_handle):
            if h is not None:
                h.set_option("grad_accumulate", int(on))

    def backward(self, dloss: torch.Tensor, need_dx: bool = False, gen: Optional[int] = None, accumulate: bool = False):
        with vf.use_handle(self.handle()):
            if not accumulate:
                return self._backward(dloss, need_dx, gen)
            self._accum = True
            try:
                self._set_accumulate(True)
                return self._backward(dloss, need_dx, gen)
            finally:
                self._accum = False
                self._set_accumulate(False)

    def _backward(self, dloss: torch.Tensor, need_dx: bool = False, gen: Optional[int] = None):
        st = self._last
        if st is None or st["labels"] is None:
            raise VitError("backward without a preceding forward(labels=...)")
        if not st["grad"] or (gen is not None and gen != st["gen"]) or st["gen"] != self._gen:
            raise VitError("backward: the activations of that forward are gone -- another forward ran on this model in "
                           "between (the engine keeps the activations of ONE forward; run backward before the next forward)")
        c = self.cfg
        a, t = self.act, self.tmp
        B, seed, ph, pa = st["B"], st["seed"], st["ph"], st["pa"]
        T, D, Fd, H, L, N, P = c.seq_len, c.hidden_size, c.intermediate_size, c.num_attention_heads, \
            c.num_hidden_layers, c.num_patches, c.patch_size
        dh, M = c.head_dim, B * T
        Mp = self._Mp
        scale = dh ** -0.5
        rope = self._rope_tables(T) if c.pos_encoding_type == "rope" else None
        hn = self.layout.head
        dloss = dloss.reshape(1).to(torch.float32).contiguous()

        tail = st["tail"]
        vf.head_loss_bwd(a["c_last"] if tail else a["last"], self.p(hn + ".weight"), st["logits"], st["labels"], dloss,
                         self.loss_kind, dlast=t["c_dlast"] if tail else t["dlast"], dW=self.g(hn + ".weight"),
                         db=self.g(hn + ".bias"))
        self._setup_side()
        dx, dx_other = t["dxa"], t["dxb"]
        cdx = None
        if tail:
            last_pre = f"vit.encoder.layer.{L - 1}."
            cdx = t["c_dxa"]
            vf.layernorm_bwd_rows(t["c_dlast"].view(B, D), a["c_xL"], self.p("vit.layernorm.weight"), a["c_meanF"],
                                  a["c_rstdF"], None, cdx, self.g("vit.layernorm.weight"), self.g("vit.layernorm.bias"),
                                  dyn=t["c_dy"], dbias=self.g(last_pre + "output.dense.bias"),
                                  dropout=(ph, seed, self._site(L - 1, 2)), row_stride=T, full_rows=M)
        elif L == 0:
            vf.layernorm_bwd(t["dlast"].view(M, D), a["x"][0].view(M, D), self.p("vit.layernorm.weight"), a["meanF"],
                             a["rstdF"], dres=None, dx=dx, dgamma=self.g("vit.layernorm.weight"),
                             dbeta=self.g("vit.layernorm.bias"))
        else:
            last_pre = f"vit.encoder.layer.{L - 1}."
            vf.layernorm_bwd_fused(t["dlast"].view(M, D), a["x"][L].view(M, D), self.p("vit.layernorm.weight"), a["meanF"],
                                   a["rstdF"], None, dx, self.g("vit.layernorm.weight"), self.g("vit.layernorm.bias"),
                                   t["dy"], self.g(last_pre + "output.dense.bias"), (ph, seed, self._site(L - 1, 2)))
        self._notify(self.layout.tail_start, self.layout.n_trainable)
        for i in reversed(range(L)):
            pre = f"vit.encoder.layer.{i}."
            if cdx is not None:
                cdx, dctx = self._backward_cls_tail(i, cdx, ph, seed), t["dctx_cls"]
            else:
                self._dw(t["dy"], a["g"][i], M=D, N=Fd, K=Mp, a_trans=True, b_trans=True,
                         out=self.g(pre + "output.dense.weight"), split_k=-1, reads=("dy",))
                self._before_write("dU")
                vf.gemm(t["dy"], self.w16(pre + "output.dense.weight"), M=Mp, N=Fd, K=D, b_trans=True, out=t["dU"],
                        act=vf.ACT_MUL_AUX, aux_in=a["u"][i], colsum_out=self.g(pre + "intermediate.dense.bias"))
                self._dw(t["dU"], a["h2"][i], M=Fd, N=D, K=Mp, a_trans=True, b_trans=True,
                         out=self.g(pre + "intermediate.dense.weight"), split_k=-1, reads=("dU",))
                vf.gemm(t["dU"], self.w16(pre + "intermediate.dense.weight"), M=Mp, N=D, K=Fd, b_trans=True, out=t["dh"])
                self._before_write("dy2")
                vf.layernorm_bwd_fused(t["dh"], a["x1"][i], self.p(pre + "layernorm_after.weight"), a["mean2"][i],
                                       a["rstd2"][i], dx, dx_other, self.g(pre + "layernorm_after.weight"),
                                       self.g(pre + "layernorm_after.bias"), t["dy2"],
                                       self.g(pre + "attention.output.dense.bias"), (ph, seed, self._site(i, 1)))
                dx, dx_other = dx_other, dx
                self._dw(t["dy2"], a["ctx"][i], M=D, N=D, K=Mp, a_trans=True, b_trans=True,
                         out=self.g(pre + "attention.output.dense.weight"), split_k=-1, reads=("dy2",))
                vf.gemm(t["dy2"], self.w16(pre + "attention.output.dense.weight"), M=Mp, N=D, K=D, b_trans=True,
                        out=t["dctx"])
                dctx = t["dctx"]
            self._before_write("dqkv")
            vf.attention_bwd(a["qkv"][i], a["ctx"][i], dctx, a["lse"][i], B, H, T, dh, scale,
                             dropout=(pa, seed, self._site(i, 0)), dqkv=t["dqkv"], delta=t["delta"],
                             colsum_out=None if rope is not None else self._qkv_bias(i, self.grads), ctx_lo=a["ctx_lo"][i])
            if rope is not None:
                vf.rope_qk(t["dqkv"], rope[0], rope[1], T, H, dh, inverse=True)
                vf.colsum(t["dqkv"], out=self._qkv_bias(i, self.grads), accumulate=self._accum)
            self._dw(t["dqkv"], a["h1"][i], M=3 * D, N=D, K=Mp, a_trans=True, b_trans=True, out=self._qkv_wgrad(i),
                     split_k=-1, reads=("dqkv",))
            vf.gemm(t["dqkv"], self._qkv16(i), M=Mp, N=D, K=3 * D, b_trans=True, out=t["dh"])
            self._before_write("dy")
            if cdx is not None:
                prev = f"vit.encoder.layer.{i - 1}."
                vf.layernorm_bwd_rows(t["dh"], a["x"][i].view(M, D), self.p(pre + "layernorm_before.weight"), a["mean1"][i],
                                      a["rstd1"][i], cdx, dx_other, self.g(pre + "layernorm_before.weight"),
                                      self.g(pre + "layernorm_before.bias"), dyn=t["dy"] if i > 0 else None,
                                      dbias=self.g(prev + "output.dense.bias") if i > 0 else None,
                                      dropout=(ph, seed, self._site(i - 1, 2)) if i > 0 else vf.NO_DROP, dres_row_stride=T)
                cdx = None
            elif i > 0:
                prev = f"vit.encoder.layer.{i - 1}."
                vf.layernorm_bwd_fused(t["dh"], a["x"][i].view(M, D), self.p(pre + "layernorm_before.weight"),
                                       a["mean1"][i], a["rstd1"][i], dx, dx_other,
                                       self.g(pre + "layernorm_before.weight"), self.g(pre + "layernorm_before.bias"),
                                       t["dy"], self.g(prev + "output.dense.bias"), (ph, seed, self._site(i - 1, 2)))
            else:
                vf.layernorm_bwd(t["dh"], a["x"][i].view(M, D), self.p(pre + "layernorm_before.weight"), a["mean1"][i],
                                 a["rstd1"][i], dres=dx, dx=dx_other, dgamma=self.g(pre + "layernorm_before.weight"),
                                 dbeta=self.g(pre + "layernorm_before.bias"))
            dx, dx_other = dx_other, dx
            self._notify(*self.layout.layer_ranges[i])
        e = "vit.embeddings."
        dpos = self.g(e + "position_embeddings").view(T, D) if c.pos_encoding_type == "learned" else None
        vf.embed_finish_bwd(dx.view(B, T, D), self.g(e + "cls_token").view(D), dpos, dropout=(ph, seed, 0),
                            dpatch=t["dpatch"])
        vf.colsum(t["dpatch"], out=self.g(e + "patch_embeddings.projection.bias"), accumulate=self._accum)
        vf.gemm(t["dpatch"], a["patches"], M=D, N=P, K=B * N, a_trans=True, b_trans=True,
                out=self.g(e + "patch_embeddings.projection.weight").view(D, P), split_k=-1)
        self._join_side()
        self._notify(self.layout.embed_start, self.layout.embed_end)
        if need_dx:
            S = c.stride
            wp = self.w16(e + "patch_embeddings.projection.weight").view(D, P)
            dpat = vf.gemm(t["dpatch"], wp, M=B * N, N=P, K=D, b_trans=True, out_dtype=torch.float32)
            return vf.fold_add(dpat, B, c.image_size, P, S, N)
        return None
```

vit_amd/functional.py:

```python
from __future__ import annotations

import ctypes as C
from typing import Optional, Tuple

import torch

from . import _cabi
from ._cabi import ACT_DGELU, ACT_GELU, ACT_GELU_GRAD, ACT_MUL_AUX, ACT_NONE, LOSS_CE, LOSS_L1, LOSS_MSE, VIT_BF16, VIT_F32, GemmDesc

_DT = {torch.float32: VIT_F32, torch.bfloat16: VIT_BF16}


def _stream(t: torch.Tensor) -> int:
    return torch.cuda.current_stream(t.device).cuda_stream


_HANDLE_OVERRIDE: Optional[_cabi.Handle] = None


def _h(t: torch.Tensor) -> _cabi.Handle:
    if not t.is_cuda:
        raise _cabi.VitError("vit_amd kernels need tensors on an MI355X (cuda/hip device); there is no CPU path")
    return _HANDLE_OVERRIDE if _HANDLE_OVERRIDE is not None else _cabi.handle_for(t.device)


class use_handle:

    def __init__(self, handle: _cabi.Handle):
        self.handle = handle

    def __enter__(self):
        global _HANDLE_OVERRIDE
        self.prev, _HANDLE_OVERRIDE = _HANDLE_OVERRIDE, self.handle
        return self.handle

    def __exit__(self, *exc):
        global _HANDLE_OVERRIDE
        _HANDLE_OVERRIDE = self.prev
        return False


def _ptr(t: Optional[torch.Tensor]) -> Optional[int]:
    return None if t is None else t.data_ptr()


def _chk(t: torch.Tensor, dtype, name: str):
    if t.dtype != dtype:
        raise _cabi.VitError(f"{name}: expected {dtype}, got {t.dtype}")
    if not t.is_contiguous():
        raise _cabi.VitError(f"{name}: tensor must be contiguous")


Dropout = Tuple[float, int, int]
NO_DROP: Dropout = (0.0, 0, 0)


def gemm(a: torch.Tensor, b: torch.Tensor, *, M: int, N: int, K: int, a_trans: bool = False, b_trans: bool = False,
         lda: Optional[int] = None, ldb: Optional[int] = None, out: Optional[torch.Tensor] = None,
         out_dtype=torch.bfloat16, ldc: Optional[int] = None, alpha: float = 1.0, bias: Optional[torch.Tensor] = None,
         act: int = ACT_NONE, aux_out: Optional[torch.Tensor] = None, aux_in: Optional[torch.Tensor] = None,
         dropout: Dropout = NO_DROP, residual: Optional[torch.Tensor] = None, row_map: Tuple[int, int, int] = (0, 0, 0),
         out_rows: Optional[int] = None, split_k: int = 0, accumulate: bool = False,
         colsum_out: Optional[torch.Tensor] = None,
         rope: Optional[Tuple[torch.Tensor, torch.Tensor, int, int, int]] = None, drop_row_stride: int = 0) -> torch.Tensor:
    h = _h(a)
    if a.dtype != b.dtype or a.dtype not in _DT:
        raise _cabi.VitError(f"gemm: operands must both be bf16 or both f32 (got {a.dtype}, {b.dtype})")
    if out is None:
        out = torch.empty((out_rows if out_rows is not None else M, N), dtype=out_dtype, device=a.device)
    d = GemmDesc()
    d.M, d.N, d.K = M, N, K
    d.a_trans, d.b_trans = int(a_trans), int(b_trans)
    d.ab_dtype = _DT[a.dtype]
    d.A, d.lda = a.data_ptr(), lda if lda is not None else (M if a_trans else K)
    d.B, d.ldb = b.data_ptr(), ldb if ldb is not None else (N if b_trans else K)
    d.C, d.ldc, d.c_dtype = out.data_ptr(), ldc if ldc is not None else N, _DT[out.dtype]
    d.alpha = alpha
    d.bias = _ptr(bias)
    d.act = act
    d.aux_out, d.aux_in, d.ldaux = _ptr(aux_out), _ptr(aux_in), N
    d.dropout_p, d.seed, d.site = dropout
    d.drop_row_stride = int(drop_row_stride)
    d.residual, d.ldres = _ptr(residual), N
    d.rows_per_batch, d.out_batch_rows, d.out_row_offset = row_map
    d.split_k = split_k
    d.accumulate = int(accumulate)
    if colsum_out is not None:
        _chk(colsum_out, torch.float32, "gemm colsum_out")
        if colsum_out.numel() != N:
            raise _cabi.VitError(f"gemm: colsum_out must have N={N} elements")
        d.colsum_out = colsum_out.data_ptr()
    if rope is not None:
        cos, sin, rT, rdh, rcols = rope
        _chk(cos, torch.float32, "gemm rope cos")
        _chk(sin, torch.float32, "gemm rope sin")
        if cos.numel() != rT * (rdh // 2) or sin.numel() != cos.numel():
            raise _cabi.VitError(f"gemm: rope tables must be [T={rT}, head_dim/2={rdh // 2}]")
        d.rope_cos, d.rope_sin, d.rope_T, d.rope_dh, d.rope_cols = cos.data_ptr(), sin.data_ptr(), int(rT), int(rdh), int(rcols)
    h.call("vit_gemm", C.byref(d), _stream(a))
    return out


def linear_fwd(x, W, bias=None, *, out_dtype=torch.bfloat16, act=ACT_NONE, aux_out=None, dropout: Dropout = NO_DROP,
               residual=None, out=None):
    M, K = x.shape
    N = W.shape[0]
    return gemm(x, W, M=M, N=N, K=K, out=out, out_dtype=out_dtype, bias=bias, act=act, aux_out=aux_out, dropout=dropout,
                residual=residual)


def linear_bwd_dx(dy, W, *, out_dtype=torch.bfloat16, dgelu_aux=None, out=None):
    M, N = dy.shape
    K = W.shape[1]
    return gemm(dy, W, M=M, N=K, K=N, b_trans=True, out=out, out_dtype=out_dtype,
                act=ACT_DGELU if dgelu_aux is not None else ACT_NONE, aux_in=dgelu_aux)


def linear_bwd_dw(dy, x, *, out=None, accumulate=False):
    M, N = dy.shape
    K = x.shape[1]
    return gemm(dy, x, M=N, N=K, K=M, a_trans=True, b_trans=True, out=out, out_dtype=torch.float32, split_k=-1,
                accumulate=accumulate)


def layernorm_fwd(x, gamma, beta, eps: float, out_dtype=torch.bfloat16, out=None, mean=None, rstd=None):
    _chk(x, torch.float32, "layernorm_fwd x")
    h = _h(x)
    D = x.shape[-1]
    rows = x.numel() // D
    y = out if out is not None else torch.empty(x.shape, dtype=out_dtype, device=x.device)
    mean = mean if mean is not None else torch.empty(rows, dtype=torch.float32, device=x.device)
    rstd = rstd if rstd is not None else torch.empty(rows, dtype=torch.float32, device=x.device)
    h.call("vit_layernorm_fwd", x.data_ptr(), gamma.data_ptr(), beta.data_ptr(), y.data_ptr(), _DT[y.dtype], _ptr(mean),
           _ptr(rstd), rows, D, eps, _stream(x))
    return y, mean, rstd


def layernorm_fwd_residual(x, delta, xsum, gamma, beta, eps: float, out_dtype=torch.bfloat16, out=None, mean=None,
                           rstd=None, x_row_stride: int = 1):
    _chk(x, torch.float32, "layernorm_fwd_residual x")
    _chk(xsum, torch.float32, "layernorm_fwd_residual xsum")
    h = _h(x)
    D = x.shape[-1]
    rows = xsum.numel() // D
    if x_row_stride < 1 or (rows - 1) * x_row_stride * D + D > x.numel() or (x_row_stride == 1 and x.numel() != xsum.numel()):
        raise _cabi.VitError("layernorm_fwd_residual: x does not hold the rows that xsum and x_row_stride name")
    if delta.dtype not in _DT or not delta.is_contiguous() or delta.numel() != xsum.numel():
        raise _cabi.VitError("layernorm_fwd_residual: delta must be a contiguous bf16/f32 tensor of xsum's shape")
    y = out if out is not None else torch.empty(xsum.shape, dtype=out_dtype, device=x.device)
    mean = mean if mean is not None else torch.empty(rows, dtype=torch.float32, device=x.device)
    rstd = rstd if rstd is not None else torch.empty(rows, dtype=torch.float32, device=x.device)
    if y.numel() != xsum.numel() or mean.numel() < rows or rstd.numel() < rows:
        raise _cabi.VitError("layernorm_fwd_residual: out / mean / rstd do not hold xsum's rows")
    if x_row_stride != 1:
        h.call("vit_layernorm_fwd_residual_rows", x.data_ptr(), x_row_stride, delta.data_ptr(), _DT[delta.dtype],
               xsum.data_ptr(), gamma.data_ptr(), beta.data_ptr(), y.data_ptr(), _DT[y.dtype], _ptr(mean), _ptr(rstd), rows,
               D, eps, _stream(x))
        return y, mean, rstd
    h.call("vit_layernorm_fwd_residual", x.data_ptr(), delta.data_ptr(), _DT[delta.dtype], xsum.data_ptr(),
           gamma.data_ptr(), beta.data_ptr(), y.data_ptr(), _DT[y.dtype], _ptr(mean), _ptr(rstd), rows, D, eps, _stream(x))
    return y, mean, rstd


def layernorm_bwd(dy, x, gamma, mean, rstd, dres=None, dx=None, dgamma=None, dbeta=None):
    _chk(x, torch.float32, "layernorm_bwd x")
    h = _h(x)
    D = x.shape[-1]
    rows = x.numel() // D
    dx = dx if dx is not None else torch.empty_like(x)
    dgamma = dgamma if dgamma is not None else torch.empty(D, dtype=torch.float32, device=x.device)
    dbeta = dbeta if dbeta is not None else torch.empty(D, dtype=torch.float32, device=x.device)
    h.call("vit_layernorm_bwd", dy.data_ptr(), _DT[dy.dtype], x.data_ptr(), gamma.data_ptr(), mean.data_ptr(),
           rstd.data_ptr(), _ptr(dres), dx.data_ptr(), dgamma.data_ptr(), dbeta.data_ptr(), rows, D, _stream(x))
    return dx, dgamma, dbeta


def layernorm_bwd_fused(dy, x, gamma, mean, rstd, dres, dx, dgamma, dbeta, dyn, dbias, dropout: Dropout = NO_DROP):
    _chk(x, torch.float32, "layernorm_bwd_fused x")
    h = _h(x)
    D = x.shape[-1]
    rows = x.numel() // D
    p, seed, site = dropout
    h.call("vit_layernorm_bwd_fused", dy.data_ptr(), _DT[dy.dtype], x.data_ptr(), gamma.data_ptr(), mean.data_ptr(),
           rstd.data_ptr(), _ptr(dres), dx.data_ptr(), dgamma.data_ptr(), dbeta.data_ptr(), rows, D, dyn.data_ptr(),
           _DT[dyn.dtype], dbias.data_ptr(), p, seed, site, _stream(x))
    return dx, dgamma, dbeta, dyn, dbias


def layernorm_bwd_rows(dy, x, gamma, mean, rstd, dres, dx, dgamma, dbeta, dyn=None, dbias=None, dropout: Dropout = NO_DROP,
                       dres_row_stride: int = 0, row_stride: int = 1, full_rows: Optional[int] = None):
    _chk(x, torch.float32, "layernorm_bwd_rows x")
    _chk(dx, torch.float32, "layernorm_bwd_rows dx")
    h = _h(x)
    D = x.shape[-1]
    rows = x.numel() // D
    if dy.numel() != x.numel() or dx.numel() != x.numel() or mean.numel() < rows or rstd.numel() < rows or \
            (dyn is not None and (dyn.numel() != x.numel() or dbias is None)):
        raise _cabi.VitError("layernorm_bwd_rows: dy / dx / dyn must have x's shape, mean / rstd its rows")
    if dres is not None:
        _chk(dres, torch.float32, "layernorm_bwd_rows dres")
        need = x.numel() if dres_row_stride == 0 else -(-rows // dres_row_stride) * D
        if dres_row_stride < 0 or dres.numel() < need:
            raise _cabi.VitError(f"layernorm_bwd_rows: dres holds {dres.numel()} elements, needs {need}")
    p, seed, site = dropout
    if row_stride > 1:
        full_rows = (rows - 1) * row_stride + 1 if full_rows is None else full_rows
        if dres_row_stride or -(-full_rows // row_stride) != rows:
            raise _cabi.VitError("layernorm_bwd_rows: row_stride needs full_rows = the full tensor's rows and a dres like dx")
        rows = full_rows
    h.call("vit_layernorm_bwd_rows", dy.data_ptr(), _DT[dy.dtype], x.data_ptr(), gamma.data_ptr(), mean.data_ptr(),
           rstd.data_ptr(), _ptr(dres), dres_row_stride, dx.data_ptr(), dgamma.data_ptr(), dbeta.data_ptr(), rows, D,
           _ptr(dyn), _DT[dyn.dtype] if dyn is not None else VIT_BF16, _ptr(dbias), p, seed, site, row_stride, _stream(x))
    return dx


def linear_bwd_dw_rows(dy, x, out, *, row_stride: int, full_rows: int, ldx: Optional[int] = None):
    _chk(out, torch.float32, "linear_bwd_dw_rows out")
    if dy.dtype != x.dtype or dy.dtype not in _DT:
        raise _cabi.VitError("linear_bwd_dw_rows: operands must both be bf16 or both f32")
    h = _h(dy)
    rows, N = dy.shape
    K = out.shape[1]
    if out.shape[0] != N or not out.is_contiguous() or not dy.is_contiguous():
        raise _cabi.VitError("linear_bwd_dw_rows: out must be a contiguous [N, K] tensor, dy contiguous")
    h.call("vit_linear_bwd_dw_rows", dy.data_ptr(), N, x.data_ptr(), ldx if ldx is not None else K, _DT[dy.dtype],
           out.data_ptr(), rows, N, K, row_stride, full_rows, _stream(dy))
    return out


def colsum_rows(a, out, *, row_stride: int, full_rows: int):
    _chk(out, torch.float32, "colsum_rows out")
    h = _h(a)
    rows, cols = a.shape
    h.call("vit_colsum_rows", a.data_ptr(), _DT[a.dtype], a.stride(0), out.data_ptr(), rows, cols, row_stride, full_rows,
           _stream(a))
    return out


def attention_fwd(qkv, B: int, H: int, T: int, dh: int, scale: float, dropout: Dropout = NO_DROP, ctx=None, lse=None,
                  ctx_lo=None):
    h = _h(qkv)
    ctx = ctx if ctx is not None else torch.empty((B * T, H * dh), dtype=qkv.dtype, device=qkv.device)
    lse = lse if lse is not None else torch.empty((B * H, T), dtype=torch.float32, device=qkv.device)
    p, seed, site = dropout
    if ctx_lo is not None:
        _chk(ctx_lo, ctx.dtype, "attention_fwd ctx_lo")
    h.call("vit_attention_fwd", qkv.data_ptr(), ctx.data_ptr(), _ptr(ctx_lo), lse.data_ptr(), _DT[qkv.dtype], B, H, T, dh,
           scale, p, seed, site, _stream(qkv))
    return ctx, lse


def attention_bwd(qkv, ctx, dctx, lse, B: int, H: int, T: int, dh: int, scale: float, dropout: Dropout = NO_DROP,
                  dqkv=None, delta=None, colsum_out=None, ctx_lo=None):
    _chk(dctx, qkv.dtype, "attention_bwd dctx")
    h = _h(qkv)
    dqkv = dqkv if dqkv is not None else torch.empty_like(qkv)
    delta = delta if delta is not None else torch.empty((B * H, T), dtype=torch.float32, device=qkv.device)
    p, seed, site = dropout
    if colsum_out is not None:
        _chk(colsum_out, torch.float32, "attention_bwd colsum_out")
    h.call("vit_attention_bwd", qkv.data_ptr(), ctx.data_ptr(), _ptr(ctx_lo), dctx.data_ptr(), lse.data_ptr(),
           delta.data_ptr(), dqkv.data_ptr(), _DT[qkv.dtype], B, H, T, dh, scale, p, seed, site, _ptr(colsum_out),
           _stream(qkv))
    return dqkv


def attention_probs(qkv, B: int, H: int, T: int, dh: int, scale: float):
    h = _h(qkv)
    probs = torch.empty((B, H, T, T), dtype=torch.float32, device=qkv.device)
    h.call("vit_attention_probs", qkv.data_ptr(), probs.data_ptr(), _DT[qkv.dtype], B, H, T, dh, scale, _stream(qkv))
    return probs


def fold_add(dpatches, B: int, L: int, P: int, S: int, N: int, out=None):
    _chk(dpatches, torch.float32, "fold_add dpatches")
    if dpatches.numel() != B * N * P:
        raise _cabi.VitError("fold_add: dpatches must hold B*N*P elements")
    out = out if out is not None else torch.empty((B, L), dtype=torch.float32, device=dpatches.device)
    h = _h(dpatches)
    h.call("vit_fold_add", dpatches.data_ptr(), out.data_ptr(), B, L, P, S, N, _stream(dpatches))
    return out


def add_noise(flux, error, noise_level: float, seed: int, out=None):
    _chk(flux, torch.float32, "add_noise flux")
    _chk(error, torch.float32, "add_noise error")
    if error.shape != flux.shape or flux.numel() % 4:
        raise _cabi.VitError("add_noise: flux/error must have the same shape and a multiple of 4 elements")
    out = out if out is not None else torch.empty_like(flux)
    h = _h(flux)
    h.call("vit_add_noise", flux.data_ptr(), error.data_ptr(), out.data_ptr(), flux.numel(), float(noise_level),
           int(seed) & 0xFFFFFFFFFFFFFFFF, _stream(flux))
    return out


def rope_qk(qkv, cos_half, sin_half, T: int, H: int, dh: int, inverse: bool = False):
    if qkv.dtype not in _DT or not qkv.is_contiguous() or qkv.dim() != 2 or qkv.shape[1] != 3 * H * dh:
        raise _cabi.VitError(f"rope_qk: qkv must be a contiguous [rows, {3 * H * dh}] bf16/f32 tensor")
    _chk(cos_half, torch.float32, "rope_qk cos")
    _chk(sin_half, torch.float32, "rope_qk sin")
    if cos_half.shape[-1] != dh // 2 or cos_half.shape[0] < T or sin_half.shape != cos_half.shape:
        raise _cabi.VitError("rope_qk: tables must be [>= T, dh/2]")
    h = _h(qkv)
    h.call("vit_rope_qk", qkv.data_ptr(), _DT[qkv.dtype], cos_half.data_ptr(), sin_half.data_ptr(), qkv.shape[0], T, H, dh,
           qkv.shape[1], 1 if inverse else 0, _stream(qkv))
    return qkv


def unfold_cast(x, P: int, S: int, N: int, out=None, out_dtype=torch.bfloat16):
    _chk(x, torch.float32, "unfold_cast x")
    h = _h(x)
    B, L = x.shape
    out = out if out is not None else torch.empty((B * N, P), dtype=out_dtype, device=x.device)
    h.call("vit_unfold_cast", x.data_ptr(), out.data_ptr(), _DT[out.dtype], B, L, P, S, N, _stream(x))
    return out


def embed_finish(tokens, cls, pos=None, dropout: Dropout = NO_DROP):
    _chk(tokens, torch.float32, "embed_finish tokens")
    h = _h(tokens)
    B, T, D = tokens.shape
    p, seed, site = dropout
    h.call("vit_embed_finish", tokens.data_ptr(), cls.data_ptr(), _ptr(pos), B, T, D, p, seed, site, _stream(tokens))
    return tokens


def embed_finish_bwd(dtokens, dcls, dpos=None, dropout: Dropout = NO_DROP, dpatch=None, out_dtype=torch.bfloat16):
    _chk(dtokens, torch.float32, "embed_finish_bwd dtokens")
    h = _h(dtokens)
    B, T, D = dtokens.shape
    dpatch = dpatch if dpatch is not None else torch.empty((B * (T - 1), D), dtype=out_dtype, device=dtokens.device)
    p, seed, site = dropout
    h.call("vit_embed_finish_bwd", dtokens.data_ptr(), dpatch.data_ptr(), _DT[dpatch.dtype], dcls.data_ptr(), _ptr(dpos), B,
           T, D, p, seed, site, 0, _stream(dtokens))
    return dpatch


def dropout_bwd_cast(dx, dropout: Dropout = NO_DROP, out=None, out_dtype=torch.bfloat16):
    _chk(dx, torch.float32, "dropout_bwd_cast dx")
    h = _h(dx)
    cols = dx.shape[-1]
    rows = dx.numel() // cols
    out = out if out is not None else torch.empty(dx.shape, dtype=out_dtype, device=dx.device)
    p, seed, site = dropout
    h.call("vit_dropout_bwd_cast", dx.data_ptr(), out.data_ptr(), _DT[out.dtype], rows, cols, p, seed, site, _stream(dx))
    return out


def colsum(a, out=None, accumulate: bool = False):
    h = _h(a)
    rows, cols = a.shape
    out = out if out is not None else torch.empty(cols, dtype=torch.float32, device=a.device)
    h.call("vit_colsum", a.data_ptr(), _DT[a.dtype], a.stride(0), out.data_ptr(), rows, cols, int(accumulate), _stream(a))
    return out


def cov_accumulate(x, mean, acc, *, rows: Optional[int] = None, cols: Optional[int] = None):
    h = _h(x)
    if x.dtype != torch.float32 or x.dim() != 2 or x.stride(1) != 1:
        raise _cabi.VitError("cov_accumulate: x must be a 2-D f32 tensor with unit column stride")
    _chk(mean, torch.float32, "cov_accumulate mean")
    _chk(acc, torch.float32, "cov_accumulate acc")
    n = x.shape[0] if rows is None else rows
    L = x.shape[1] if cols is None else cols
    if n > x.shape[0] or L > x.shape[1] or mean.numel() < L or tuple(acc.shape) != (L, L):
        raise _cabi.VitError(f"cov_accumulate: x {tuple(x.shape)}, mean {mean.numel()}, acc {tuple(acc.shape)} do not fit n={n} L={L}")
    h.call("vit_cov_accumulate", x.data_ptr(), x.stride(0) if n > 1 else max(L, x.stride(0)), mean.data_ptr(),
           acc.data_ptr(), n, L, _stream(x))
    return acc


def cov_mean_finish(colsum, n_total: int, cols: Optional[int] = None):
    _chk(colsum, torch.float32, "cov_mean_finish colsum")
    h = _h(colsum)
    h.call("vit_cov_mean_finish", colsum.data_ptr(), colsum.numel() if cols is None else cols, int(n_total),
           _stream(colsum))
    return colsum


def cov_finish(acc, n_total: int, out=None):
    _chk(acc, torch.float32, "cov_finish acc")
    h = _h(acc)
    L = acc.shape[0]
    out = out if out is not None else torch.empty((L, L), dtype=torch.float32, device=acc.device)
    _chk(out, torch.float32, "cov_finish out")
    h.call("vit_cov_finish", acc.data_ptr(), out.data_ptr(), L, int(n_total), _stream(acc))
    return out


def cast_f32_bf16(src, out=None):
    _chk(src, torch.float32, "cast_f32_bf16 src")
    h = _h(src)
    out = out if out is not None else torch.empty(src.shape, dtype=torch.bfloat16, device=src.device)
    h.call("vit_cast_f32_bf16", src.data_ptr(), out.data_ptr(), src.numel(), _stream(src))
    return out


def cast_bf16_f32(src, out, scale: float = 1.0):
    _chk(src, torch.bfloat16, "cast_bf16_f32 src")
    _chk(out, torch.float32, "cast_bf16_f32 out")
    h = _h(src)
    h.call("vit_cast_bf16_f32", src.data_ptr(), out.data_ptr(), src.numel(), float(scale), _stream(src))
    return out


def head_loss_fwd(last_hidden, W, b, labels, loss_kind: int):
    _chk(last_hidden, torch.float32, "head_loss_fwd last_hidden")
    h = _h(last_hidden)
    B, T, D = last_hidden.shape
    Cn = W.shape[0]
    logits = torch.empty((B, Cn), dtype=torch.float32, device=last_hidden.device)
    loss = torch.zeros((), dtype=torch.float32, device=last_hidden.device) if labels is not None else None
    h.call("vit_head_loss_fwd", last_hidden.data_ptr(), W.data_ptr(), b.data_ptr(), _ptr(labels), logits.data_ptr(),
           _ptr(loss), B, T, D, Cn, loss_kind, _stream(last_hidden))
    return logits, loss


def head_loss_bwd(last_hidden, W, logits, labels, dloss, loss_kind: int, dlast=None, dW=None, db=None):
    h = _h(last_hidden)
    B, T, D = last_hidden.shape
    Cn = W.shape[0]
    dlast = dlast if dlast is not None else torch.empty_like(last_hidden)
    dW = dW if dW is not None else torch.empty_like(W)
    db = db if db is not None else torch.empty(Cn, dtype=torch.float32, device=W.device)
    h.call("vit_head_loss_bwd", last_hidden.data_ptr(), W.data_ptr(), logits.data_ptr(), labels.data_ptr(),
           dloss.data_ptr(), dlast.data_ptr(), dW.data_ptr(), db.data_ptr(), B, T, D, Cn, loss_kind, 0,
           _stream(last_hidden))
    return dlast, dW, db


def grad_sqnorm(g, out=None, accumulate: bool = False):
    _chk(g, torch.float32, "grad_sqnorm g")
    h = _h(g)
    out = out if out is not None else torch.empty(1, dtype=torch.float32, device=g.device)
    h.call("vit_grad_sqnorm_acc" if accumulate else "vit_grad_sqnorm", g.data_ptr(), g.numel(), out.data_ptr(), _stream(g))
    return out


def adamw_step(p, g, m, v, p_bf16, *, lr, beta1=0.9, beta2=0.999, eps=1e-8, weight_decay=0.0, step=1, sqnorm=None,
               max_norm=0.0, n: Optional[int] = None):
    h = _h(p)
    n = p.numel() if n is None else n
    h.call("vit_adamw_step", p.data_ptr(), g.data_ptr(), m.data_ptr(), v.data_ptr(), _ptr(p_bf16), n, lr, beta1, beta2, eps,
           weight_decay, step, _ptr(sqnorm), max_norm, _stream(p))
```

Before: 7807.

## Fuse residual add into attention-out and fc2 GEMM epilogues

Adds an epilogue mode that rounds the GEMM output to bf16 and then adds the f32 residual in the kernel, writing the f32 residual stream directly. The attention output and fc2 projections now produce x1 and x[i+1] themselves, so the following layernorm runs without the residual-add variant and the intermediate bf16 y buffer is no longer written or read. A dedicated buffer-load epilogue (FAST==9) prefetches residual rows ahead of the stores. This removes memory traffic for the intermediate tensor, at the cost of more epilogue work and a new planning path gated by an environment variable.

```diff
diff --git a/include/vit_amd.h b/include/vit_amd.h
--- a/include/vit_amd.h
+++ b/include/vit_amd.h
@@ -15,7 +15,8 @@
 
 typedef enum { VIT_OK = 0, VIT_ERR_ARG = -1, VIT_ERR_HIP = -2, VIT_ERR_UNSUPPORTED = -3, VIT_ERR_WORKSPACE = -4 } vit_status;
 typedef enum { VIT_F32 = 0, VIT_BF16 = 1 } vit_dtype;
-typedef enum { VIT_ACT_NONE = 0, VIT_ACT_GELU = 1, VIT_ACT_DGELU = 2, VIT_ACT_GELU_GRAD = 3, VIT_ACT_MUL_AUX = 4 } vit_act;
+typedef enum { VIT_ACT_NONE = 0, VIT_ACT_GELU = 1, VIT_ACT_DGELU = 2, VIT_ACT_GELU_GRAD = 3, VIT_ACT_MUL_AUX = 4,
+               VIT_ACT_ROUND_BF16 = 5 } vit_act;
 typedef enum { VIT_LOSS_MSE = 0, VIT_LOSS_L1 = 1, VIT_LOSS_CE = 2 } vit_loss;
 
 int vit_version(void);
@@ -142,5 +143,6 @@
 #endif
 
 #include "vit_amd_cov.h"
+#include "vit_amd_plan.h"
 
 #endif
diff --git a/include/vit_amd_plan.h b/include/vit_amd_plan.h
--- /dev/null
+++ b/include/vit_amd_plan.h
@@ -0,0 +1,14 @@
+#ifndef VIT_AMD_PLAN_H_
+#define VIT_AMD_PLAN_H_
+
+#ifdef __cplusplus
+extern "C" {
+#endif
+
+int vit_gemm_fuses_residual(vit_handle h, const vit_gemm_desc* d);
+
+#ifdef __cplusplus
+}
+#endif
+
+#endif
diff --git a/vit_amd/_cabi.py b/vit_amd/_cabi.py
--- a/vit_amd/_cabi.py
+++ b/vit_amd/_cabi.py
@@ -11,7 +11,7 @@
 
 VIT_OK, VIT_ERR_WORKSPACE = 0, -4
 VIT_F32, VIT_BF16 = 0, 1
-ACT_NONE, ACT_GELU, ACT_DGELU, ACT_GELU_GRAD, ACT_MUL_AUX = 0, 1, 2, 3, 4
+ACT_NONE, ACT_GELU, ACT_DGELU, ACT_GELU_GRAD, ACT_MUL_AUX, ACT_ROUND_BF16 = 0, 1, 2, 3, 4, 5
 LOSS_MSE, LOSS_L1, LOSS_CE = 0, 1, 2
 
 
@@ -60,6 +60,7 @@
     "vit_step_advance": [_P, _U64, _F, _F, _P],
     "vit_adamw_step_dyn": [_P, _P, _P, _P, _P, _P, _I64, _F, _F, _F, _F, _P, _F, _P],
     "vit_gemm": [_P, C.POINTER(GemmDesc), _P],
+    "vit_gemm_fuses_residual": [_P, C.POINTER(GemmDesc)],
     "vit_last_gemm_kernel": [],
     "vit_linear_fwd": [_P, _P, _P, _P, _P, _I, _I, _I, _I, _I, _P, _F, _U64, _U64, _P, _P],
     "vit_linear_bwd_dx": [_P, _P, _P, _P, _I, _I, _I, _I, _P, _P],
diff --git a/vit_amd/build.py b/vit_amd/build.py
--- a/vit_amd/build.py
+++ b/vit_amd/build.py
@@ -16,7 +16,7 @@
 SOURCES = ["api.hip", "gemm.hip", "gemm2.hip", "layernorm.hip", "attention.hip", "attention_tiled.hip", "attention_resident.hip",
            "attention_pipe.hip", "attention_f32.hip", "elementwise.hip", "covariance.hip"]
 HEADERS = [os.path.join(CSRC, "common.h"), os.path.join(CSRC, "attention.h"), os.path.join(ROOT, "include", "vit_amd.h"),
-           os.path.join(ROOT, "include", "vit_amd_cov.h")]
+           os.path.join(ROOT, "include", "vit_amd_cov.h"), os.path.join(ROOT, "include", "vit_amd_plan.h")]
 
 
 def _hipcc() -> str:
diff --git a/vit_amd/csrc/common.h b/vit_amd/csrc/common.h
--- a/vit_amd/csrc/common.h
+++ b/vit_amd/csrc/common.h
@@ -48,6 +48,11 @@
   bf2 r = __builtin_convertvector(v, bf2);
   return __builtin_bit_cast(unsigned, r);
 }
+__device__ __forceinline__ f32x4 round_bf16(f32x4 v) {
+  const unsigned a = pack2bf(v[0], v[1]), b = pack2bf(v[2], v[3]);
+  return (f32x4){__builtin_bit_cast(float, a << 16), __builtin_bit_cast(float, a & 0xFFFF0000u),
+                 __builtin_bit_cast(float, b << 16), __builtin_bit_cast(float, b & 0xFFFF0000u)};
+}
 
 __device__ __forceinline__ unsigned drop_hash(unsigned k0, unsigned k1, unsigned long long idx) {
   unsigned x = (unsigned)idx ^ k0 ^ ((unsigned)(idx >> 32) * 0x9E3779B9u);
diff --git a/vit_amd/csrc/gemm.hip b/vit_amd/csrc/gemm.hip
--- a/vit_amd/csrc/gemm.hip
+++ b/vit_amd/csrc/gemm.hip
@@ -20,6 +20,7 @@
   const float* bias;
   const short* aux_in; short* aux_out; long ldaux;
   const float* residual; long ldres;
+  int rround;
   float alpha;
   int act, c_dtype;
   DropCfg drop;
@@ -107,6 +108,7 @@
         drop_pair(p.drop, krow, (unsigned)n + 2, k2, k3);
         v[0] *= k0; v[1] *= k1; v[2] *= k2; v[3] *= k3;
       }
+      if (p.rround == VIT_BF16) v = round_bf16(v);
       if (p.residual) v += *(const f32x4*)(p.residual + orow * p.ldres + n);
       if (p.c_dtype == VIT_BF16) {
         u32x2 pk = {pack2bf(v[0], v[1]), pack2bf(v[2], v[3])};
@@ -537,7 +539,7 @@
             VIT_ERR_ARG, "vit_gemm: leading dimension smaller than the row length");
   if (d->bias) VIT_CHECK(al16(d->bias), VIT_ERR_ARG, "vit_gemm: bias must be 16-byte aligned");
   if (d->residual) VIT_CHECK(al16(d->residual) && (d->ldres % 4) == 0, VIT_ERR_ARG, "vit_gemm: residual alignment");
-  VIT_CHECK(d->act >= VIT_ACT_NONE && d->act <= VIT_ACT_MUL_AUX, VIT_ERR_ARG, "vit_gemm: bad act %d", d->act);
+  VIT_CHECK(d->act >= VIT_ACT_NONE && d->act <= VIT_ACT_ROUND_BF16, VIT_ERR_ARG, "vit_gemm: bad act %d", d->act);
   if (d->act == VIT_ACT_DGELU || d->act == VIT_ACT_MUL_AUX)
     VIT_CHECK(d->aux_in && (d->ldaux % 4) == 0, VIT_ERR_ARG, "vit_gemm: ACT_DGELU / ACT_MUL_AUX need aux_in");
   if (d->act == VIT_ACT_GELU_GRAD) VIT_CHECK(d->aux_out, VIT_ERR_ARG, "vit_gemm: ACT_GELU_GRAD needs aux_out");
@@ -622,6 +624,7 @@
               "vit_gemm: accumulate needs an f32 C and no residual");
     a.residual = (const float*)d->C; a.ldres = d->ldc;
   }
+  a.rround = (d->residual && d->act == VIT_ACT_ROUND_BF16) ? VIT_BF16 : 0;
   a.alpha = d->alpha;
   a.act = d->act; a.c_dtype = d->c_dtype;
   a.drop = make_drop_h(h, d->dropout_p, d->seed, d->site);
diff --git a/vit_amd/csrc/gemm2.hip b/vit_amd/csrc/gemm2.hip
--- a/vit_amd/csrc/gemm2.hip
+++ b/vit_amd/csrc/gemm2.hip
@@ -17,6 +17,7 @@
   const float* bias;
   const short* aux_in; short* aux_out; long ldaux;
   const float* residual; long ldres;
+  int rround;
   float alpha;
   int act, c_dtype;
   DropCfg drop;
@@ -99,6 +100,7 @@
           drop_pair(p.drop, krow, (unsigned)n + 2, k2, k3);
           v[0] *= k0; v[1] *= k1; v[2] *= k2; v[3] *= k3;
         }
+        if (p.rround == VIT_BF16) v = round_bf16(v);
         if (p.residual) v += *(const f32x4*)(p.residual + orow * p.ldres + n);
         if (p.c_dtype == VIT_BF16) {
           u32x2 pk = {pack2bf(v[0], v[1]), pack2bf(v[2], v[3])};
@@ -118,6 +120,53 @@
 __device__ __forceinline__ void pp_epilogue(f32x4 (&acc)[NI][4], char* scr, const Gemm2Args& p, int m0, int n0, int split,
                                             int lane) {
   const int l15 = lane & 15, lg = lane >> 4;
+  if (FAST == 9) {
+    const int n = n0 + l15 * 4;
+    f32x4 bv = (f32x4){0.f, 0.f, 0.f, 0.f};
+    if (p.bias) bv = *(const f32x4*)(p.bias + n);
+    const __amdgpu_buffer_rsrc_t rr_ = make_rsrc(p.residual, (unsigned long long)p.M * p.ldres * 4);
+    const __amdgpu_buffer_rsrc_t rc_ = make_rsrc(p.C, (unsigned long long)p.M * p.ldc * 4);
+    constexpr int RES_LD = 18, RES_ST = 16;
+    u32x4 rs[NI][4];
+#define RES_LOAD(I_)                                                                                                  \
+  _Pragma("unroll") for (int rr = 0; rr < 4; ++rr) rs[I_][rr] = __builtin_amdgcn_raw_buffer_load_b128(                 \
+      rr_, (unsigned)(((long)(m0 + (I_) * 16 + rr * 4 + lg) * p.ldres + n) * 4), 0, RES_LD);
+    RES_LOAD(0)
+    RES_LOAD(1)
+#pragma unroll
+    for (int i = 0; i < NI; ++i) {
+      if ((i & 1) == 0 && i + 3 < NI) {
+        RES_LOAD(i + 2)
+        RES_LOAD(i + 3)
+      }
+#pragma unroll
+      for (int j = 0; j < 4; ++j) {
+        *(f32x4*)(scr + l15 * 256 + (((j * 4 + lg) ^ l15) << 4)) = acc[i][j];
+        acc[i][j] = (f32x4){0.f, 0.f, 0.f, 0.f};
+      }
+      f32x4 v[4];
+#pragma unroll
+      for (int rr = 0; rr < 4; ++rr) {
+        const int row = rr * 4 + lg;
+        v[rr] = *(const f32x4*)(scr + row * 256 + ((l15 ^ row) << 4));
+      }
+#pragma unroll
+      for (int rr = 0; rr < 4; ++rr) {
+        const long m = m0 + i * 16 + rr * 4 + lg;
+        f32x4 o = v[rr] + bv;
+        if (p.drop.thr) {
+          float k0, k1, k2, k3;
+          drop_pair(p.drop, (unsigned long long)m, (unsigned)n, k0, k1);
+          drop_pair(p.drop, (unsigned long long)m, (unsigned)n + 2, k2, k3);
+          o[0] *= k0; o[1] *= k1; o[2] *= k2; o[3] *= k3;
+        }
+        const f32x4 out = __builtin_bit_cast(f32x4, rs[i][rr]) + round_bf16(o);
+        __builtin_amdgcn_raw_buffer_store_b128(__builtin_bit_cast(u32x4, out), rc_, (unsigned)((m * p.ldc + n) * 4), 0, RES_ST);
+      }
+    }
+#undef RES_LOAD
+    return;
+  }
   if (FAST == 7) {
     float* cf = p.splits > 1 ? p.slab + (long)split * p.M * p.N : (float*)p.C;
     const long ldc = p.splits > 1 ? (long)p.N : p.ldc;
@@ -593,6 +642,7 @@
   if (epi == 5) return launch_stag<0, 1, 5>(a, grid, st);
   if (epi == 6) return launch_stag<0, 1, 6>(a, grid, st);
   if (epi == 8) return launch_stag<0, 0, 8>(a, grid, st);
+  if (epi == 9) return launch_stag<0, 0, 9>(a, grid, st);
   if (epi == 7) return launch_stag<1, 1, 7>(a, grid, st);
   if (!at && !bt) return launch_stag<0, 0, 0>(a, grid, st);
   if (!at && bt) return launch_stag<0, 1, 0>(a, grid, st);
@@ -641,6 +691,14 @@
   if (d->accumulate && splits == 1 && !(d->c_dtype == VIT_F32 && !d->residual && d->rows_per_batch == 0)) return false;
   *epi_out = epi; *splits_out = splits; *kps_out = kps;
   return true;
+}
+static bool pp_residual_fast(vit_handle h, const vit_gemm_desc* d) {
+  int epi, splits, kps;
+  if (d->ab_dtype != VIT_BF16 || !pp_plan(h, d, &epi, &splits, &kps)) return false;
+  return epi == 0 && splits == 1 && d->residual && d->act == VIT_ACT_ROUND_BF16 && d->c_dtype == VIT_F32 && !d->a_trans &&
+         !d->b_trans && !d->accumulate && d->rows_per_batch == 0 && !(d->dropout_p > 0.f && d->drop_row_stride > 1) &&
+         d->alpha == 1.0f && !d->colsum_out && !d->rope_cos &&
+         (unsigned long long)d->M * d->ldc * 4 < 0x7FFFFFF0ull && (unsigned long long)d->M * d->ldres * 4 < 0x7FFFFFF0ull;
 }
 static size_t pp_colsum_bytes(const vit_gemm_desc* d) { return (size_t)(d->M / 256) * 2 * d->N * sizeof(float); }
 
@@ -672,6 +730,7 @@
   a.aux_in = (const short*)d->aux_in; a.aux_out = (short*)d->aux_out; a.ldaux = d->ldaux;
   a.residual = d->residual; a.ldres = d->ldres;
   if (d->accumulate && splits == 1) { a.residual = (const float*)d->C; a.ldres = d->ldc; }
+  a.rround = (d->residual && d->act == VIT_ACT_ROUND_BF16) ? VIT_BF16 : 0;
   a.alpha = d->alpha;
   a.rope_cos = d->rope_cos; a.rope_sin = d->rope_sin; a.rope_T = d->rope_T; a.rope_dh = d->rope_dh; a.rope_cols = d->rope_cols;
   a.act = d->act; a.c_dtype = d->c_dtype;
@@ -694,6 +753,7 @@
   else if (epi == 0 && plain && !a.bias && !a.drop.thr && d->c_dtype == VIT_BF16 && !d->a_trans && d->b_trans &&
            splits == 1) epi5 = 6;
   else if (epi == 0 && plain && !a.bias && !a.drop.thr && d->c_dtype == VIT_F32 && d->a_trans && d->b_trans) epi5 = 7;
+  else if (pp_residual_fast(h, d)) epi5 = 9;
   if (d->rope_cos) {
     if (epi5 == 3 && !a.drop.thr && (d->rope_dh == 16 || d->rope_dh == 32 || d->rope_dh == 64) && (d->rope_cols % 64) == 0 &&
         d->rope_T >= 9)
@@ -837,6 +897,10 @@
 }
 
 extern "C" {
+
+int vit_gemm_fuses_residual(vit_handle h, const vit_gemm_desc* d) {
+  return h && d && d->M > 0 && d->N > 0 && d->K > 0 && vit::pp_residual_fast(h, d) ? 1 : 0;
+}
 
 int vit_linear_bwd_dw_rows(vit_handle h, const void* dy, int64_t ldy, const void* x, int64_t ldx, int dtype, float* dW,
                            int rows, int N, int K, int64_t row_stride, int64_t full_rows, vit_stream stream) {
diff --git a/vit_amd/engine.py b/vit_amd/engine.py
--- a/vit_amd/engine.py
+++ b/vit_amd/engine.py
@@ -146,6 +146,7 @@
         self._side_reads: Dict[str, object] = {}
         self.overlap_dw = "auto"
         self.cls_tail = os.environ.get("VIT_CLS_TAIL", "1") != "0"
+        self.residual_sites = frozenset(filter(None, os.environ.get("VIT_RESIDUAL_SITES", "attn,fc2").split(",")))
         self._accum = False
         self._gen = 0
         self.grad_ready_cb: Optional[Callable[[int, int], None]] = None
@@ -248,12 +249,12 @@
         return self.grads[off:off + 3 * D * D].view(3 * D, D)
 
     def _ensure_arena(self, B: int, train: bool):
-        key = (B, train, self.precision)
+        key = (B, train, self.precision, self.residual_sites)
         if self._arena_key == key:
             return
         slot = self._arenas.get(train)
         if slot is not None and slot[0] == key:
-            self._arena_key, self.act, self.tmp, self._Mp = key, slot[1], slot[2], slot[3]
+            self._arena_key, self.act, self.tmp, self._Mp, self._fuse = key, slot[1], slot[2], slot[3], slot[4]
             return
         self.act, self.tmp = {}, {}
         self._arenas.pop(train, None)
@@ -265,6 +266,10 @@
         Mp = -(-M // 256) * 256 if (D % 256 == 0 and Fd % 256 == 0) else M
         self._Mp = Mp
         nl = L if train else 1
+        fuse = {s: self.precision == "bf16" and s in self.residual_sites and
+                vf.gemm_fuses_residual(self.flat, M=Mp, N=D, K=(D if s == "attn" else Fd), dropout_p=c.hidden_dropout_prob)
+                for s in ("attn", "fc2")}
+        self._fuse = fuse
         f32, b16 = torch.float32, self.adt
 
         def E(shape, dt):
@@ -275,16 +280,16 @@
 
         self.act = dict(
             patches=E((B * N, P), b16),
-            x=[E((B, T, D), f32) for _ in range(L + 1)],
+            x=[G(D, f32).view(B, T, D) for _ in range(L + 1)],
             h1=[G(D, b16) for _ in range(nl)], qkv=[G(3 * D, b16) for _ in range(nl)],
             ctx=[G(D, b16) for _ in range(nl)], lse=[E((B * H, T), f32) for _ in range(nl)],
             ctx_lo=[E((M, D), b16) if (train and self.precision == "bf16") else None for _ in range(nl)],
-            x1=[E((M, D), f32) for _ in range(nl)], h2=[G(D, b16) for _ in range(nl)],
+            x1=[G(D, f32) for _ in range(nl)], h2=[G(D, b16) for _ in range(nl)],
             u=[G(Fd, b16) for _ in range(nl)], g=[G(Fd, b16) for _ in range(nl)],
             mean1=[E((M,), f32) for _ in range(nl)], rstd1=[E((M,), f32) for _ in range(nl)],
             mean2=[E((M,), f32) for _ in range(nl)], rstd2=[E((M,), f32) for _ in range(nl)],
             last=E((B, T, D), f32), meanF=E((M,), f32), rstdF=E((M,), f32),
-            y=G(D, b16),
+            y=None if (fuse["attn"] and fuse["fc2"]) else G(D, b16),
             c_y=E((B, D), b16), c_x1=E((B, D), f32), c_h2=E((B, D), b16), c_u=E((B, Fd), b16), c_g=E((B, Fd), b16),
             c_mean2=E((B,), f32), c_rstd2=E((B,), f32), c_xL=E((B, D), f32), c_last=E((B, 1, D), f32),
             c_meanF=E((B,), f32), c_rstdF=E((B,), f32),
@@ -300,7 +305,7 @@
                 dctx_cls=G(D, b16),
             )
         self._arena_key = key
-        self._arenas[train] = (key, self.act, self.tmp, Mp)
+        self._arenas[train] = (key, self.act, self.tmp, Mp, fuse)
 
     def _drop_arenas(self):
         self._arena_key = None
@@ -364,16 +369,18 @@
 
         atts = [] if output_attentions else None
         rope = self._rope_tables(T) if c.pos_encoding_type == "rope" else None
-        y = a["y"]
+        y, fuse = a["y"], self._fuse
+        bf = torch.bfloat16
+        pend = None
         tail = bool(self.cls_tail) and L > 0 and not output_hidden_states
         for i in range(L):
             j = i if need_grad else 0
             pre = f"vit.encoder.layer.{i}."
             xin = a["x"][i].view(M, D)
-            if i == 0:
+            if pend is None:
                 self._ln(xin, pre + "layernorm_before", a["h1"][j], a["mean1"][j], a["rstd1"][j])
             else:
-                self._ln_res(a["x1"][jprev], y, xin, pre + "layernorm_before", a["h1"][j], a["mean1"][j], a["rstd1"][j])
+                self._ln_res(pend, y, xin, pre + "layernorm_before", a["h1"][j], a["mean1"][j], a["rstd1"][j])
             vf.gemm(a["h1"][j], self._qkv16(i), M=Mp, N=3 * D, K=D, out=a["qkv"][j], bias=self._qkv_bias(i, self.flat),
                     rope=None if rope is None else (rope[0], rope[1], T, dh, 2 * D))
             vf.attention_fwd(a["qkv"][j], B, H, T, dh, scale, dropout=(pa, seed, self._site(i, 0)), ctx=a["ctx"][j],
@@ -384,15 +391,25 @@
                 capture_ctx.append(a["ctx"][j].view(B, T, D).clone())
             if tail and i == L - 1:
                 break
-            vf.gemm(a["ctx"][j], self.w16(pre + "attention.output.dense.weight"), M=Mp, N=D, K=D, out=y,
-                    bias=self.p(pre + "attention.output.dense.bias"), dropout=(ph, seed, self._site(i, 1)))
-            self._ln_res(xin, y, a["x1"][j], pre + "layernorm_after", a["h2"][j], a["mean2"][j], a["rstd2"][j])
+            wo, bo = self.w16(pre + "attention.output.dense.weight"), self.p(pre + "attention.output.dense.bias")
+            if fuse["attn"]:
+                vf.gemm(a["ctx"][j], wo, M=Mp, N=D, K=D, out=a["x1"][j], bias=bo, dropout=(ph, seed, self._site(i, 1)),
+                        residual=xin, pre_residual_dtype=bf)
+                self._ln(a["x1"][j], pre + "layernorm_after", a["h2"][j], a["mean2"][j], a["rstd2"][j])
+            else:
+                vf.gemm(a["ctx"][j], wo, M=Mp, N=D, K=D, out=y, bias=bo, dropout=(ph, seed, self._site(i, 1)))
+                self._ln_res(xin, y, a["x1"][j], pre + "layernorm_after", a["h2"][j], a["mean2"][j], a["rstd2"][j])
             vf.gemm(a["h2"][j], self.w16(pre + "intermediate.dense.weight"), M=Mp, N=Fd, K=D, out=a["g"][j],
                     bias=self.p(pre + "intermediate.dense.bias"), act=vf.ACT_GELU_GRAD if need_grad else ACT_GELU,
                     aux_out=a["u"][j] if need_grad else None)
-            vf.gemm(a["g"][j], self.w16(pre + "output.dense.weight"), M=Mp, N=D, K=Fd, out=y,
-                    bias=self.p(pre + "output.dense.bias"), dropout=(ph, seed, self._site(i, 2)))
-            jprev = j
+            w2, b2 = self.w16(pre + "output.dense.weight"), self.p(pre + "output.dense.bias")
+            if fuse["fc2"]:
+                vf.gemm(a["g"][j], w2, M=Mp, N=D, K=Fd, out=a["x"][i + 1].view(M, D), bias=b2,
+                        dropout=(ph, seed, self._site(i, 2)), residual=a["x1"][j], pre_residual_dtype=bf)
+                pend = None
+            else:
+                vf.gemm(a["g"][j], w2, M=Mp, N=D, K=Fd, out=y, bias=b2, dropout=(ph, seed, self._site(i, 2)))
+                pend = a["x1"][j]
         last = a["last"]
         if tail:
             i, pre = L - 1, f"vit.encoder.layer.{L - 1}."
@@ -408,9 +425,8 @@
             vf.gemm(a["c_g"], self.w16(pre + "output.dense.weight"), M=B, N=D, K=Fd, out=cy,
                     bias=self.p(pre + "output.dense.bias"), dropout=(ph, seed, self._site(i, 2)), drop_row_stride=T)
             self._ln_res(a["c_x1"], cy, a["c_xL"], "vit.layernorm", last.view(B, D), a["c_meanF"], a["c_rstdF"])
-        elif L > 0:
-            self._ln_res(a["x1"][jprev], y, a["x"][L].view(M, D), "vit.layernorm", a["last"].view(M, D), a["meanF"],
-                         a["rstdF"])
+        elif pend is not None:
+            self._ln_res(pend, y, a["x"][L].view(M, D), "vit.layernorm", a["last"].view(M, D), a["meanF"], a["rstdF"])
         else:
             self._ln(a["x"][L].view(M, D), "vit.layernorm", a["last"].view(M, D), a["meanF"], a["rstdF"])
         hn = self.layout.head
diff --git a/vit_amd/functional.py b/vit_amd/functional.py
--- a/vit_amd/functional.py
+++ b/vit_amd/functional.py
@@ -62,10 +62,17 @@
          dropout: Dropout = NO_DROP, residual: Optional[torch.Tensor] = None, row_map: Tuple[int, int, int] = (0, 0, 0),
          out_rows: Optional[int] = None, split_k: int = 0, accumulate: bool = False,
          colsum_out: Optional[torch.Tensor] = None,
-         rope: Optional[Tuple[torch.Tensor, torch.Tensor, int, int, int]] = None, drop_row_stride: int = 0) -> torch.Tensor:
+         rope: Optional[Tuple[torch.Tensor, torch.Tensor, int, int, int]] = None, drop_row_stride: int = 0,
+         pre_residual_dtype: Optional[torch.dtype] = None) -> torch.Tensor:
     h = _h(a)
     if a.dtype != b.dtype or a.dtype not in _DT:
         raise _cabi.VitError(f"gemm: operands must both be bf16 or both f32 (got {a.dtype}, {b.dtype})")
+    if pre_residual_dtype not in (None, torch.bfloat16):
+        raise _cabi.VitError(f"gemm: pre_residual_dtype must be None or torch.bfloat16 (got {pre_residual_dtype})")
+    if pre_residual_dtype is not None:
+        if act != ACT_NONE:
+            raise _cabi.VitError("gemm: pre_residual_dtype cannot be combined with an activation")
+        act = _cabi.ACT_ROUND_BF16
     if out is None:
         out = torch.empty((out_rows if out_rows is not None else M, N), dtype=out_dtype, device=a.device)
     d = GemmDesc()
@@ -101,6 +108,19 @@
     return out
 
 
+def gemm_fuses_residual(like: torch.Tensor, *, M: int, N: int, K: int, dropout_p: float = 0.0) -> bool:
+    h = _h(like)
+    d = GemmDesc()
+    d.M, d.N, d.K = M, N, K
+    d.ab_dtype, d.c_dtype, d.act = VIT_BF16, VIT_F32, _cabi.ACT_ROUND_BF16
+    d.lda = d.ldb = K
+    d.ldc = d.ldres = d.ldaux = N
+    d.alpha = 1.0
+    d.A = d.B = d.C = d.bias = d.residual = like.data_ptr()
+    d.dropout_p = dropout_p
+    return bool(h.lib.vit_gemm_fuses_residual(h.h, C.byref(d)))
+
+
 def linear_fwd(x, W, bias=None, *, out_dtype=torch.bfloat16, act=ACT_NONE, aux_out=None, dropout: Dropout = NO_DROP,
                residual=None, out=None):
     M, K = x.shape
```

New measurement: 7865, median of 6. About the same (+0.7%).
